# LLNL/saamge

Measured on AMD Instinct MI355X. Metric: AMG setup+solve DoF/s (3D Poisson, PCG to 1e-8), higher is better.
Workload: dtype f64; 1 GPU; 3D Poisson 256^3 Q1 hexes, 3-level SAAMGE, theta=0.003, nu_relax=3, 8x8x4-element AEs, 8x8x4-AE coarse blocks; workload_id=poisson256, dofs=16974593, converged=True, parallelism=single GPU

## Files before the change

### saamge_amd/csrc/capi.hip

```cpp
#include <cstdlib>
#include "../../include/saamge_amd.h"

#include <string>

#include "hierarchy.h"
#include "operator.h"
#include "partition.h"
#include "spgemm.h"

using namespace saamge_amd;

struct saamge_amd_hierarchy {
    Hierarchy *H;
};

struct saamge_amd_partitioning {
    int device = 0;
    std::vector<DBuf<int>> part;
    std::vector<std::vector<int>> part_host;
    std::vector<const int *> part_ptr, part_host_ptr;
    std::vector<int> n_elem, nparts;
    std::vector<DBuf<roff_t>> xadj;
    std::vector<DBuf<int>> adj;
    std::vector<int64_t> nnz;
// ... 261 lines not shown
        set_thread_stream(hs);
    }
    delete h->H;
    delete h;
    if (had) {
        dev_pool_close_stream(hs);
        unset_thread_stream();
    }
}

struct VecIn {
    DBuf<double> buf;
    const double *p;
    VecIn(const double *src, size_t n, hipStream_t s) {
        if (is_device_ptr(src)) p = src;
        else { buf.assign(src, n, s); p = buf.p; }
    }
};
struct VecOut {
    DBuf<double> buf;
    double *p, *host = nullptr;
    size_t n;
    hipStream_t s;
    VecOut(double *dst, size_t n_, hipStream_t s_, bool load) : n(n_), s(s_) {
        if (is_device_ptr(dst)) p = dst;
        else {
            host = dst;
            if (load) buf.assign(dst, n, s); else buf.alloc(n);
            p = buf.p;
        }
    }
    void finish() {
        if (host && n) SA_HIP_CHECK(hipMemcpyAsync(host, p, 8 * n, hipMemcpyDeviceToHost, s));
        SA_HIP_CHECK(hipStreamSynchronize(s));
    }
};

int saamge_amd_vcycle_mult(saamge_amd_hierarchy *h, const double *b, double *x) {
    SA_API_BEGIN
    SA_REQUIRE(h && b && x, "null argument");
    Hierarchy &H = *h->H;
    require_device(H);
    const size_t n = (size_t)H.levels[0]->A.nrows;
    VecIn vb(b, n, H.stream);
    VecOut vx(x, n, H.stream, false);
    vcycle_apply(H, 0, vb.p, vx.p);
    vx.finish();
    SA_API_END
}

int saamge_amd_vcycle(saamge_amd_hierarchy *h, const double *b, double *x, int iterative_mode) {
    if (!iterative_mode) return saamge_amd_vcycle_mult(h, b, x);
    SA_API_BEGIN
    SA_REQUIRE(h && b && x, "null argument");
    Hierarchy &H = *h->H;
    require_device(H);
    Level &L0 = *H.levels[0];
    SA_REQUIRE(!L0.dist.on, "iterative_mode is not available on a row-partitioned hierarchy");
    const size_t n = (size_t)L0.A.nrows;
    VecIn vb(b, n, H.stream);
    VecOut vx(x, n, H.stream, true);
    spmv_residual(H.stream, L0.A, vx.p, vb.p, H.pcg_r.p);
    vcycle_apply(H, 0, H.pcg_r.p, H.pcg_z.p);
    vec_axpy(H.stream, (int)n, 1.0, H.pcg_z.p, vx.p);
    vx.finish();
    SA_API_END
}

int saamge_amd_set_coarse_solver(saamge_amd_hierarchy *h, saamge_amd_coarse_solve_fn fn, void *ctx) {
    SA_API_BEGIN
    SA_REQUIRE(h, "null argument");
    h->H->user_coarse_solve = fn;
    h->H->user_coarse_ctx = ctx;
    SA_API_END
}

int saamge_amd_set_smoother(saamge_amd_hierarchy *h, int level, saamge_amd_smoother_fn pre, saamge_amd_smoother_fn post,
                            void *ctx) {
    SA_API_BEGIN
    SA_REQUIRE(h, "null argument");
    Hierarchy &H = *h->H;
    SA_REQUIRE(level >= 0 && level < (int)H.levels.size(), "bad level");
    if (H.user_smoothers.size() < H.levels.size()) H.user_smoothers.resize(H.levels.size());
    H.user_smoothers[(size_t)level].pre = pre;
    H.user_smoothers[(size_t)level].post = post;
    H.user_smoothers[(size_t)level].ctx = ctx;
    SA_API_END
}

int saamge_amd_smoother(saamge_amd_hierarchy *h, int level, const double *b, double *x) {
    SA_API_BEGIN
    SA_REQUIRE(h && b && x, "null argument");
    Hierarchy &H = *h->H;
    require_device(H);
    SA_REQUIRE(level >= 0 && level < (int)H.levels.size(), "bad level");
    const size_t n = (size_t)H.levels[level]->A.nrows;
    VecIn vb(b, n, H.stream);
    VecOut vx(x, n, H.stream, true);
    smoother_apply(H, level, vb.p, vx.p);
    vx.finish();
    SA_API_END
}

int saamge_amd_pcg(saamge_amd_hierarchy *h, const double *b, double *x, double rel_tol,
                   double abs_tol, int max_iter, int squared_tol, int zero_guess, int *iters,
                   int *converged, double *hist) {
    SA_API_BEGIN
    SA_REQUIRE(h && b && x && iters, "null argument");
    Hierarchy &H = *h->H;
    require_device(H);
    const size_t n = (size_t)H.levels[0]->A.nrows;
    VecIn vb(b, n, H.stream);
    VecOut vx(x, n, H.stream, !zero_guess);
    int conv = 0;
    *iters = pcg_solve(H, vb.p, vx.p, rel_tol, abs_tol, max_iter, squared_tol, zero_guess, &conv, hist);
    if (converged) *converged = conv;
    vx.finish();
    SA_API_END
}

int saamge_amd_num_levels(const saamge_amd_hierarchy *h) { return h ? (int)h->H->levels.size() + 1 : 0; }

static const DCsr &level_op(const Hierarchy &H, int level, int which) {
    const int nl = (int)H.levels.size();
    SA_REQUIRE(level >= 0 && level < nl, "bad level");
    const Level &L = *H.levels[level];
    switch (which) {
        case 0: return L.A;
        case 1: return L.P;
        case 2: return L.R;
        case 3: return (level + 1 < nl) ? H.levels[level + 1]->A : L.Ac;
    }
    throw Error(1, "bad operator selector");
}

int saamge_amd_level_info(const saamge_amd_hierarchy *h, int level, long long info[16]) {
    SA_API_BEGIN
    SA_REQUIRE(h && info, "null argument");
    const Hierarchy &H = *h->H;
    for (int i = 0; i < 16; ++i) info[i] = 0;
    const Level &L = *H.levels.at(level);
    info[0] = L.A.nrows;
    info[1] = L.A.nnz;
    info[2] = L.rel.nparts;
    info[3] = L.rel.num_mises;
    info[4] = L.P.ncols;
    info[5] = L.P.nnz;
    info[6] = level_op(H, level, 3).nnz;
    long long tot = 0;
    for (int m : L.ae_m) tot += m;
    info[7] = tot;
    info[8] = H.last_coarse_iters;
    info[9] = L.ae_xoff.empty() ? 0 : L.ae_xoff.back();
    info[10] = L.mis_s_off.empty() ? 0 : L.mis_s_off.back();
    long long usz = 0;
    for (int m = 0; m < L.rel.num_mises; ++m) usz += (long long)L.mis_k[m] * L.rel.mis_to_dof.row_size(m);
    info[11] = usz;
    info[12] = L.dist.on ? 1 : 0;
    info[13] = L.dist.row0;
    info[14] = L.dist.nloc;
    info[15] = L.dist.nrecv;
    SA_API_END
}

int saamge_amd_level_format(const saamge_amd_hierarchy *h, int level, long long info[12]) {
    SA_API_BEGIN
    SA_REQUIRE(h && info, "null argument");
    const Hierarchy &H = *h->H;
    for (int i = 0; i < 12; ++i) info[i] = 0;
    const Sell &S = H.levels.at(level)->A.sell;
    for (int c = 0; c < 3; ++c) { info[c] = S.class_slices[c]; info[3 + c] = S.class_entries[c]; }
    if (S.dict.on) { info[8] = S.dict.ng; info[9] = S.dict.bs3 ? 1 : 0; info[10] = S.dict.bs3 ? S.dict.nirr : 0; }
    info[6] = S.stage.on() ? (long long)div_up(S.nslices, 4) - S.stage.nunstaged : 0;
    info[7] = (long long)S.stream_bytes;
    info[11] = H.levels.at(level)->ae_solved;
    SA_API_END
}

int saamge_amd_coarse_solver_info(const saamge_amd_hierarchy *h, long long info[8]) {
    SA_API_BEGIN
    SA_REQUIRE(h && info, "null argument");
    const Hierarchy &H = *h->H;
    for (int i = 0; i < 8; ++i) info[i] = 0;
    SA_REQUIRE(!H.levels.empty(), "no levels");
    info[0] = H.user_coarse_solve ? 0 : H.coarse_kind;
    info[1] = H.levels.back()->Ac.nrows;
    if (H.coarse_kind == 3) {
        info[2] = H.c_bt.nblk;
        info[3] = H.c_bt.max_block;
        info[4] = (long long)H.c_bt.Sinv.n;
    } else if (H.coarse_kind == 1) {
        info[4] = (long long)H.c_L.n;
    }
    SA_API_END
}

static int get_csr(const saamge_amd_hierarchy *h, int level, int which, void *rowptr, int rowptr_bits, int *col, double *val) {
    SA_API_BEGIN
    SA_REQUIRE(h, "null argument");
    const Hierarchy &H = *h->H;
    require_device(H);
    const DCsr &M = level_op(H, level, which);
    hipStream_t s = H.stream;
    if (rowptr && rowptr_bits == 64)
        SA_HIP_CHECK(hipMemcpyAsync(rowptr, M.rowptr.p, sizeof(roff_t) * ((size_t)M.nrows + 1), hipMemcpyDeviceToHost, s));
    else if (rowptr)
        export_rowptr32((int *)rowptr, M.rowptr, (size_t)M.nrows + 1, s);
    if (col && M.nnz) SA_HIP_CHECK(hipMemcpyAsync(col, M.col.p, 4 * (size_t)M.nnz, hipMemcpyDeviceToHost, s));
    if (val && M.nnz) SA_HIP_CHECK(hipMemcpyAsync(val, M.val.p, 8 * (size_t)M.nnz, hipMemcpyDeviceToHost, s));
    SA_HIP_CHECK(hipStreamSynchronize(s));
    SA_API_END
}
int saamge_amd_get_csr(const saamge_amd_hierarchy *h, int level, int which, int *rowptr, int *col, double *val) {
    return get_csr(h, level, which, rowptr, 32, col, val);
}
int saamge_amd_get_csr64(const saamge_amd_hierarchy *h, int level, int which, long long *rowptr, int *col, double *val) {
    return get_csr(h, level, which, rowptr, 64, col, val);
}

int saamge_amd_get_table(const saamge_amd_hierarchy *h, int level, int which, int *nrows,
                         long long *nconn, int *I, int *J) {
    SA_API_BEGIN
    SA_REQUIRE(h, "null argument");
    require_device(*h->H);
    {
        Level &Lw = *h->H->levels.at(level);
        fetch_relations_ae_host(Lw.rel, Lw.drel, h->H->stream);
    }
    const Relations &r = h->H->levels.at(level)->rel;
    const Table *T = nullptr;
    switch (which) {
        case 0: T = &r.AE_to_dof; break;
        case 1: T = &r.dof_to_AE; break;
        case 2: T = &r.mis_to_dof; break;
        case 3: T = &r.mis_to_AE; break;
        case 4: T = &r.AE_to_mis; break;
        case 5: {
            if (r.elem_to_dof.I.empty()) {
                Level &L = *h->H->levels.at(level);
                Relations &rw = L.rel;
                rw.elem_to_dof.I = L.drel.e2d_I.to_host(h->H->stream);
                rw.elem_to_dof.J = L.drel.e2d_J.to_host(h->H->stream);
                rw.elem_to_dof.ncols = rw.ND;
            }
            T = &r.elem_to_dof;
            break;
        }
        default: throw Error(1, "bad table selector");
    }
    if (nrows) *nrows = T->nrows();
    if (nconn) *nconn = (long long)T->J.size();
    if (I) std::copy(T->I.begin(), T->I.end(), I);
    if (J) std::copy(T->J.begin(), T->J.end(), J);
    SA_API_END
}

int saamge_amd_get_mis(const saamge_amd_hierarchy *h, int level, int *mises, int *mis_k,
                       int *mis_ncols, signed char *agg_flags) {
    SA_API_BEGIN
    SA_REQUIRE(h, "null argument");
    require_device(*h->H);
    {
        Level &Lw = *h->H->levels.at(level);
        fetch_relations_ae_host(Lw.rel, Lw.drel, h->H->stream);
    }
    const Level &L = *h->H->levels.at(level);
    if (mises) std::copy(L.rel.mises.begin(), L.rel.mises.end(), mises);
    if (mis_k) std::copy(L.mis_k.begin(), L.mis_k.end(), mis_k);
    if (mis_ncols) std::copy(L.mis_ncols.begin(), L.mis_ncols.end(), mis_ncols);
    if (agg_flags) std::copy(L.rel.agg_flags.begin(), L.rel.agg_flags.end(), agg_flags);
    SA_API_END
}

int saamge_amd_get_ae_eigens(const saamge_amd_hierarchy *h, int level, int *ae_m, double *evals,
                             double *evecs, double *ae_D) {
    SA_API_BEGIN
    SA_REQUIRE(h, "null argument");
    const Hierarchy &H = *h->H;
    const Level &L = *H.levels.at(level);
    hipStream_t s = H.stream;
    if (ae_m) std::copy(L.ae_m.begin(), L.ae_m.end(), ae_m);
    if (evals || evecs || ae_D) SA_REQUIRE(H.params.keep_debug, "hierarchy was built without keep_debug");
    if (evals && L.evals.n) SA_HIP_CHECK(hipMemcpyAsync(evals, L.evals.p, 8 * L.evals.n, hipMemcpyDeviceToHost, s));
    if (evecs && L.evecs.n) SA_HIP_CHECK(hipMemcpyAsync(evecs, L.evecs.p, 8 * L.evecs.n, hipMemcpyDeviceToHost, s));
    if (ae_D && L.ae_D.n) SA_HIP_CHECK(hipMemcpyAsync(ae_D, L.ae_D.p, 8 * L.ae_D.n, hipMemcpyDeviceToHost, s));
    SA_HIP_CHECK(hipStreamSynchronize(s));
    SA_API_END
}

int saamge_amd_get_mis_svd(const saamge_amd_hierarchy *h, int level, long long *sig_off,
                           double *sig, double *U) {
    SA_API_BEGIN
    SA_REQUIRE(h, "null argument");
    const Hierarchy &H = *h->H;
    const Level &L = *H.levels.at(level);
    hipStream_t s = H.stream;
    const int nm = L.rel.num_mises;
    if (sig_off) for (int m = 0; m <= nm; ++m) sig_off[m] = L.mis_s_off[m];
    if (sig) {
        SA_REQUIRE(H.params.keep_debug, "hierarchy was built without keep_debug");
        if (L.mis_s_off[nm]) SA_HIP_CHECK(hipMemcpyAsync(sig, L.mis_sig.p, 8 * (size_t)L.mis_s_off[nm], hipMemcpyDeviceToHost, s));
    }
    if (U) {
        auto all = L.mis_U.to_host(s);
        size_t o = 0;
        for (int m = 0; m < nm; ++m) {
            const size_t cnt = (size_t)L.mis_k[m] * L.rel.mis_to_dof.row_size(m);
            std::copy(all.begin() + L.mis_u_off[m], all.begin() + L.mis_u_off[m] + cnt, U + o);
            o += cnt;
        }
    }
    SA_HIP_CHECK(hipStreamSynchronize(s));
    SA_API_END
}

static int spmv_entry(int nrows, int ncols, const void *rowptr, int rowptr_bits, const int *col, const double *val,
                      const double *x, double *y) {
    SA_API_BEGIN
    SA_REQUIRE(rowptr && col && val && x && y && nrows >= 0, "bad argument");
    const Options opt = g_default_options;
    validate_options(opt);
    hipStream_t s = 0;
    set_thread_stream(s);
    DCsr A;
    A.nrows = nrows;
    A.ncols = ncols;
    import_rowptr(A.rowptr, rowptr, rowptr_bits, (size_t)nrows + 1, s);
    roff_t nnz = 0;
    SA_HIP_CHECK(hipMemcpyAsync(&nnz, A.rowptr.p + nrows, sizeof(roff_t), hipMemcpyDeviceToHost, s));
    SA_HIP_CHECK(hipStreamSynchronize(s));
    A.nnz = nnz;
    import_array(A.col, col, (size_t)A.nnz, s);
    import_array(A.val, val, (size_t)A.nnz, s);
    A.lanes_per_row = pick_lanes_per_row(A.nnz, nrows > 0 ? nrows : 1);
    if (nrows == ncols && opt.spmv_sell) build_sell(s, A, opt);
    VecIn vx(x, (size_t)ncols, s);
    VecOut vy(y, (size_t)nrows, s, false);
    spmv(s, A, vx.p, vy.p);
    vy.finish();
    SA_API_END
}
int saamge_amd_spmv(int nrows, int ncols, const int *rowptr, const int *col, const double *val,
                    const double *x, double *y) {
    return spmv_entry(nrows, ncols, rowptr, 32, col, val, x, y);
}
int saamge_amd_spmv64(int nrows, int ncols, const long long *rowptr, const int *col, const double *val,
                      const double *x, double *y) {
    return spmv_entry(nrows, ncols, rowptr, 64, col, val, x, y);
}

static void import_host_csr(DCsr &M, const char *name, int nrows, int ncols, const int *rowptr, const int *col,
                            const double *val, hipStream_t s) {
    const std::string who(name);
    SA_REQUIRE(nrows >= 0 && ncols >= 0 && rowptr, who + ": bad dimensions or no row offsets");
    SA_REQUIRE(rowptr[0] == 0, who + ": the row offsets must start at 0");
    for (int i = 0; i < nrows; ++i) SA_REQUIRE(rowptr[i + 1] >= rowptr[i], who + ": the row offsets must ascend");
    const size_t nnz = (size_t)rowptr[nrows];
    SA_REQUIRE(nnz == 0 || (col && val), who + ": entries without their arrays");
    for (size_t k = 0; k < nnz; ++k) SA_REQUIRE(col[k] >= 0 && col[k] < ncols, who + ": a column index out of range");
    M.nrows = nrows;
    M.ncols = ncols;
    M.nnz = (int64_t)nnz;
    import_rowptr(M.rowptr, rowptr, 32, (size_t)nrows + 1, s);
    M.col.assign(col, nnz, s);
    M.val.assign(val, nnz, s);
    SA_HIP_CHECK(hipStreamSynchronize(s));
    M.lanes_per_row = pick_lanes_per_row(M.nnz, nrows > 0 ? nrows : 1);
}
static void export_host_csr(const DCsr &M, int *rowptr, long long *nnz, int *col, double *val, hipStream_t s) {
    if (rowptr) export_rowptr32(rowptr, M.rowptr, (size_t)M.nrows + 1, s);
    if (nnz) *nnz = (long long)M.nnz;
    if (col && val && M.nnz) {
        SA_HIP_CHECK(hipMemcpyAsync(col, M.col.p, 4 * (size_t)M.nnz, hipMemcpyDeviceToHost, s));
        SA_HIP_CHECK(hipMemcpyAsync(val, M.val.p, 8 * (size_t)M.nnz, hipMemcpyDeviceToHost, s));
    }
    SA_HIP_CHECK(hipStreamSynchronize(s));
}

int saamge_amd_spgemm(int nrows, int ninner, int ncols, const int *Arow, const int *Acol, const double *Aval,
                      const int *Brow, const int *Bcol, const double *Bval, const int *Erow, const int *Ecol,
                      const double *Eval, const double *d, double alpha, double beta, int *Crow, long long *Cnnz,
                      int *Ccol, double *Cval, int *route) {
    if (route) *route = SPGEMM_ROUTE_NONE;
    SA_API_BEGIN
    hipStream_t s = 0;
    set_thread_stream(s);
    DCsr A, B, E, Cm;
    import_host_csr(A, "A", nrows, ninner, Arow, Acol, Aval, s);
    import_host_csr(B, "B", ninner, ncols, Brow, Bcol, Bval, s);
    const bool alias = Erow && Erow == Brow && Ecol == Bcol && Eval == Bval && nrows == ninner;
    if (Erow && !alias) import_host_csr(E, "E", nrows, ncols, Erow, Ecol, Eval, s);
    DBuf<double> dd;
    if (d) dd.assign(d, (size_t)nrows, s);
    spgemm(s, A, B, Erow ? (alias ? &B : &E) : nullptr, d ? dd.p : nullptr, alpha, beta, Cm);
    if (route) *route = spgemm_last_route();
    export_host_csr(Cm, Crow, Cnnz, Ccol, Cval, s);
    SA_API_END
}

int saamge_amd_csr_transpose(int nrows, int ncols, const int *rowptr, const int *col, const double *val, int *Rrow,
                             long long *Rnnz, int *Rcol, double *Rval) {
    SA_API_BEGIN
    hipStream_t s = 0;
    set_thread_stream(s);
    DCsr P, R;
    import_host_csr(P, "P", nrows, ncols, rowptr, col, val, s);
    csr_transpose(s, P, R);
    export_host_csr(R, Rrow, Rnnz, Rcol, Rval, s);
    SA_API_END
}

int saamge_amd_csr_threshold(int nrows, int ncols, const int *rowptr, const int *col, const double *val, double tol,
                             int *Crow, long long *Cnnz, int *Ccol, double *Cval) {
    SA_API_BEGIN
    hipStream_t s = 0;
    set_thread_stream(s);
    DCsr A, Cm;
    import_host_csr(A, "A", nrows, ncols, rowptr, col, val, s);
    csr_threshold(s, A, tol, Cm);
    export_host_csr(Cm, Crow, Cnnz, Ccol, Cval, s);
    SA_API_END
}

__global__ void apply_dscale_kernel(int count, const int *ns, const int64_t *moff, const int64_t *voff,
                                    double *W, const double *D, double *dis) {
    const int b = blockIdx.x;
    const int n = ns[b];
    double *Wm = W + moff[b];
    const double *Dm = D + voff[b];
    for (int i = threadIdx.x; i < n; i += blockDim.x) dis[voff[b] + i] = 1.0 / sqrt(Dm[i]);
    __syncthreads();
    for (size_t idx = threadIdx.x; idx < (size_t)n * n; idx += blockDim.x) {
        const int r = (int)(idx % n), c = (int)(idx / n);
        Wm[idx] = dis[voff[b] + r] * Wm[idx] * dis[voff[b] + c];
    }
}

int saamge_amd_lower_eigens_batched(int count, const int *n, const double *A, const double *D,
                                    double vl, double vu, int *m, double *evals, double *evecs) {
    SA_API_BEGIN
    SA_REQUIRE(count >= 0 && n && A && D && m && evals && evecs, "bad argument");
    const Options opt = g_default_options;
    validate_options(opt);
    hipStream_t s = 0;
    set_thread_stream(s);
    std::vector<int> sizes(n, n + count);
    EigBatch b;
    eig_batch_alloc(b, sizes, opt, s);
    b.set_window(vu);
    b.dense_only = opt.eig_dense_only != 0;
// ... 437 lines not shown
```

### saamge_amd/csrc/common.h

```cpp
#pragma once
#include <hip/hip_runtime.h>

#include <cstdint>
#include <cstdio>
#include <cstring>
#include <type_traits>
#include <stdexcept>
#include <string>
#include <vector>

namespace saamge_amd {

struct Error : std::runtime_error {
    int code;
    Error(int c, const std::string &m) : std::runtime_error(m), code(c) {}
};

#define SA_HIP_CHECK(expr)                                                              \
    do {                                                                                \
        hipError_t e_ = (expr);                                                         \
        if (e_ != hipSuccess)                                                           \
            throw ::saamge_amd::Error(2, std::string(__FILE__) + ":" +                  \
                                             std::to_string(__LINE__) + " " + #expr +   \
                                             " -> " + hipGetErrorString(e_));           \
    } while (0)

#define SA_REQUIRE(cond, msg)                                                           \
    do {                                                                                \
        if (!(cond))                                                                    \
            throw ::saamge_amd::Error(1, std::string(__FILE__) + ":" +                  \
                                             std::to_string(__LINE__) + " " + (msg));   \
    } while (0)

inline int current_device() {
    int d = 0;
    SA_HIP_CHECK(hipGetDevice(&d));
    return d;
}
inline void adopt_device(int dev) { SA_HIP_CHECK(hipSetDevice(dev)); }
hipStream_t side_stream(int slot);

void *pinned_alloc(size_t bytes);
void pinned_free(void *p, size_t bytes);
void pinned_pool_release();

template <class T>
struct PinnedAlloc {
    typedef T value_type;
    PinnedAlloc() {}
    template <class U>
    PinnedAlloc(const PinnedAlloc<U> &) {}
    T *allocate(size_t n) { return (T *)pinned_alloc(n * sizeof(T)); }
    void deallocate(T *p, size_t n) { pinned_free((void *)p, n * sizeof(T)); }
    template <class U>
    bool operator==(const PinnedAlloc<U> &) const { return true; }
    template <class U>
    bool operator!=(const PinnedAlloc<U> &) const { return false; }
};
template <class T>
using hvec = std::vector<T, PinnedAlloc<T>>;

inline bool is_device_ptr(const void *p) {
    if (!p) return false;
    hipPointerAttribute_t a;
    hipError_t e = hipPointerGetAttributes(&a, p);
    if (e != hipSuccess) {
        (void)hipGetLastError();
        return false;
    }
    return a.type == hipMemoryTypeDevice || a.type == hipMemoryTypeManaged;
}

void host_heap_policy(int mb);
bool env_timing();
bool env_timing_host();
bool env_serial();

void set_thread_stream(hipStream_t s);
void unset_thread_stream();
hipStream_t thread_stream();
bool thread_stream_is_set();
void *dev_alloc(size_t bytes);
void dev_free(void *p) noexcept;
void dev_pool_release();
size_t dev_pool_idle_bytes();
void dev_memory_stats(size_t *live, size_t *peak, bool reset_peak);
void dev_pool_counts(long *n_malloc, long *n_free, size_t *malloc_bytes, bool reset);
struct ThreadStreamScope {
    hipStream_t prev;
    bool had;
    explicit ThreadStreamScope(hipStream_t s) : prev(thread_stream()), had(thread_stream_is_set()) { set_thread_stream(s); }
    ~ThreadStreamScope() { if (had) set_thread_stream(prev); else unset_thread_stream(); }
};
void dev_pool_close_stream(hipStream_t s);

template <class T>
struct DBuf {
    T *p = nullptr;
    size_t n = 0;
    bool owned = true;
    DBuf() {}
    explicit DBuf(size_t n_) { alloc(n_); }
    DBuf(const DBuf &) = delete;
    DBuf &operator=(const DBuf &) = delete;
    DBuf(DBuf &&o) noexcept : p(o.p), n(o.n), owned(o.owned) { o.p = nullptr; o.n = 0; }
    DBuf &operator=(DBuf &&o) noexcept {
        if (this != &o) {
            release();
            p = o.p; n = o.n; owned = o.owned;
            o.p = nullptr; o.n = 0;
        }
        return *this;
    }
    ~DBuf() { release(); }
    void release() {
        if (p && owned) dev_free(p);
        p = nullptr; n = 0; owned = true;
    }
    void alloc(size_t n_) {
        release();
        n = n_;
        if (n) p = (T *)dev_alloc(n * sizeof(T));
    }
    void zero(hipStream_t s = 0) {
        if (n) SA_HIP_CHECK(hipMemsetAsync(p, 0, n * sizeof(T), s));
    }
    void assign(const T *src, size_t n_, hipStream_t s = 0) {
        alloc(n_);
        if (!n) return;
        SA_HIP_CHECK(hipMemcpyAsync(p, src, n * sizeof(T), hipMemcpyDefault, s));
    }
    template <class V>
    void from_host(const V &v, hipStream_t s = 0) {
        alloc(v.size());
        if (!n) return;
        const size_t bytes = n * sizeof(T);
        const bool pinned = std::is_same<typename V::allocator_type, PinnedAlloc<typename V::value_type>>::value;
        if (!pinned && bytes >= (256u << 10)) {
            void *stage = pinned_alloc(bytes);
            std::memcpy(stage, v.data(), bytes);
            const hipError_t e = hipMemcpyAsync(p, stage, bytes, hipMemcpyHostToDevice, s);
            const hipError_t e2 = hipStreamSynchronize(s);
            pinned_free(stage, bytes);
            SA_HIP_CHECK(e);
            SA_HIP_CHECK(e2);
            return;
        }
        SA_HIP_CHECK(hipMemcpyAsync(p, v.data(), bytes, hipMemcpyHostToDevice, s));
        SA_HIP_CHECK(hipStreamSynchronize(s));
    }
    hvec<T> to_host(hipStream_t s = 0) const {
        hvec<T> v(n);
        if (n) {
            SA_HIP_CHECK(hipMemcpyAsync(v.data(), p, n * sizeof(T), hipMemcpyDeviceToHost, s));
            SA_HIP_CHECK(hipStreamSynchronize(s));
        }
        return v;
    }
    void view(T *ptr, size_t n_) {
        release();
        p = ptr; n = n_; owned = false;
    }
};

template <class T>
inline void import_array(DBuf<T> &dst, const T *src, size_t n, hipStream_t s) {
    if (is_device_ptr(src))
        dst.view(const_cast<T *>(src), n);
    else
        dst.assign(src, n, s);
}

template <class T>
inline hvec<T> fetch_host(const T *src, size_t n, hipStream_t s) {
    hvec<T> v(n);
    if (n) {
        SA_HIP_CHECK(hipMemcpyAsync(v.data(), src, n * sizeof(T), hipMemcpyDefault, s));
        SA_HIP_CHECK(hipStreamSynchronize(s));
    }
    return v;
}
template <class T>
inline T read_one(const T *p, hipStream_t s) {
    T v;
    SA_HIP_CHECK(hipMemcpyAsync(&v, p, sizeof(T), hipMemcpyDeviceToHost, s));
    SA_HIP_CHECK(hipStreamSynchronize(s));
    return v;
}

typedef int64_t roff_t;

}
#include "sell.h"
namespace saamge_amd {
struct DCsr {
    int nrows = 0, ncols = 0;
    int64_t nnz = 0;
    DBuf<roff_t> rowptr;
    DBuf<int> col;
    DBuf<double> val;
    int lanes_per_row = 8;
    mutable int max_row = -1;
    Sell sell;
};

void exclusive_scan_int(hipStream_t s, int n, const int *in, int *out);
void exclusive_scan_int_async(hipStream_t s, int n, const int *in, int *out, int *tile_sums);
void exclusive_scan_off(hipStream_t s, int n, const int *in, roff_t *out);

void import_rowptr(DBuf<roff_t> &dst, const void *src, int bits, size_t n, hipStream_t s);
void export_rowptr32(int *dst_host, const DBuf<roff_t> &src, size_t n, hipStream_t s);

inline int pick_lanes_per_row(int64_t nnz, int nrows) {
    double avg = nrows ? double(nnz) / nrows : 1.0;
    int l = 1;
    while (l < 64 && l * 2 <= avg * 0.75 + 1.0) l *= 2;
    return l;
}

inline int div_up(int64_t a, int64_t b) { return int((a + b - 1) / b); }
__host__ __device__ inline unsigned hash_home(unsigned key, unsigned size) {
    return (key * 2654435761u) >> (__builtin_clz(size) + 1);
}

struct KernelStat {
    std::string name;
    double ms = 0.0;
    int64_t launches = 0;
    double bytes = 0.0;
    double flops = 0.0;
    double fmt_bytes = 0.0;
};

struct Profiler {
    bool enabled = false;
    std::vector<KernelStat> stats;
    hipEvent_t e0 = nullptr, e1 = nullptr;
    int level_tag = 0;
    KernelStat &get(const std::string &name) {
        for (auto &s : stats)
            if (s.name == name) return s;
        stats.push_back(KernelStat());
        stats.back().name = name;
        return stats.back();
    }
    void begin(hipStream_t s) {
        if (!enabled) return;
        if (!e0) {
            SA_HIP_CHECK(hipEventCreate(&e0));
            SA_HIP_CHECK(hipEventCreate(&e1));
        }
        SA_HIP_CHECK(hipEventRecord(e0, s));
    }
    void end(hipStream_t s, const char *name, double bytes, double flops, double fmt_bytes = 0.0) {
        if (!enabled) return;
        SA_HIP_CHECK(hipEventRecord(e1, s));
        SA_HIP_CHECK(hipEventSynchronize(e1));
        float ms = 0.f;
        SA_HIP_CHECK(hipEventElapsedTime(&ms, e0, e1));
        KernelStat &k = level_tag > 0 ? get(std::string(name) + "@L" + std::to_string(level_tag)) : get(name);
        k.ms += ms;
        k.launches += 1;
        k.bytes += bytes;
        k.flops += flops;
        k.fmt_bytes += fmt_bytes > 0.0 ? fmt_bytes : bytes;
    }
};

Profiler &profiler();

}
```

### saamge_amd/csrc/hierarchy.h

```cpp
#pragma once
#include <exception>
#include <memory>
#include <thread>

#include "assemble.h"
#include "blocktri.h"
#include "common.h"
#include "eig.h"
#include "mis.h"
#include "options.h"
#include "sparse.h"
#include "topology.h"

namespace saamge_amd {

constexpr int MAX_LEVELS = 8;

struct Params {
    int num_coarsenings = 1;
    double theta[MAX_LEVELS];
    int nu_relax[MAX_LEVELS];
    int nu_pro[MAX_LEVELS];
    int avoid_ess_bdr_dofs = 1;
    int testmesh = 0;
    int coarse_solver = 0;
    double coarse_rtol = 1e-14;
    int coarse_max_iter = 2000;
    size_t workspace_bytes = (size_t)32 << 30;
    int keep_debug = 0;
    int rank = 0, world = 1;
    int (*allgather)(void *ctx, void *buf_dev, const long long *byte_off) = nullptr;
    void *allgather_ctx = nullptr;
    int (*allreduce_sum)(void *ctx, double *buf_dev, long long count) = nullptr;
    int (*alltoallv)(void *ctx, const void *send_dev, const long long *send_byte_off, void *recv_dev,
                     const long long *recv_byte_off) = nullptr;
    long long dist_min_local_rows = 262144;
    int comm_stream_ordered = 0;
    int correct_nullspace = 0;
    const double *extra_modes = nullptr;
    int num_extra_modes = 0;
    double smooth_drop_tol = 0.0;
    int do_aggregates = 0;
    int algebraic = 0;
    int eigensolver = 0;
    double eig_tol = 1e-12;
    Options opt;
};

struct NextPrep {
    bool ready = false;
    Table e2d;
    std::vector<int> colpos_ptr, colpos;
    DBuf<int> d_colpos_ptr, d_colpos;
    bool on_device = false;
};

struct Level {
    DCsr A;
    DCsr P, R, Ac;
    DCsr Ptent;
    DBuf<double> dinv_neg;
    std::vector<double> roots;
    double theta = 0.0;
    int nu_relax = 3;
    Relations rel;
    bool rel_prebuilt = false;
    NextPrep next_prep;
    DevRelations drel;
    DevElmats elmat;
    std::vector<int> ae_begin;
    std::vector<int> ae_m;
    std::vector<int> ae_class;
    std::vector<int> ae_evclass;
    long long ae_solved = 0;
    std::vector<int64_t> ae_xoff, ae_eoff;
    DBuf<double> evals, evecs;
    DBuf<double> ae_D;
    std::vector<int> mis_k;
    std::vector<int> mis_coloff;
    std::vector<int> mis_ncols;
    std::vector<int64_t> mis_u_off, mis_s_off;
    DBuf<double> mis_U, mis_sig;
    DBuf<int> d_mis_k, d_mis_coloff;
    DBuf<int64_t> d_mis_u_off;
    DBuf<double> x, b, r, t0, t1;
    DBuf<double> extra;
    DBuf<double> cvec_next;
    struct Dist {
        bool on = false;
        int row0 = 0, nloc = 0;
        std::vector<int> row_off;
        std::vector<long long> send_off, recv_off;
        std::vector<long long> own_off;
        DBuf<int> send_idx, recv_idx;
        DBuf<double> send_buf, recv_buf;
        DBuf<double> rs_buf;
        std::vector<long long> rs_off;
        int nsend = 0, nrecv = 0;
        int int_row0 = 0, int_nrows = 0;
    } dist;
};

struct KernelTiming { double setup_ms = 0, solve_ms = 0; };

struct ParCsrIn {
    long long global_rows = 0;
    const long long *row_starts = nullptr;
    int nrows = 0;
    const int *diag_i = nullptr, *diag_j = nullptr;
    const double *diag_a = nullptr;
    const int *offd_i = nullptr, *offd_j = nullptr;
    const double *offd_a = nullptr;
    int num_cols_offd = 0;
    const long long *col_map_offd = nullptr;
};
struct DistIn {
    DBuf<roff_t> rowptr;
    DBuf<int> col, e2d;
    DBuf<double> val;
    DBuf<signed char> bdr;
    std::vector<DBuf<int>> parts;
    std::vector<int> nparts;
    int elem0 = 0, NE_loc = 0;
    std::vector<std::vector<long long>> ae_begin;
};

struct Hierarchy {
    Params params;
    hipStream_t stream = 0;
    int device = 0;
    std::vector<std::unique_ptr<Level>> levels;
    int coarse_kind = 2;
    BlockTri c_bt;
    DBuf<double> c_dinv, c_r, c_z, c_d, c_q, c_t0, c_t1, c_b, c_x;
    DBuf<double> c_L, c_work;
    std::vector<double> c_roots;
    DBuf<double> pcg_r, pcg_z, pcg_d, pcg_q, scal, partials;
    int last_coarse_iters = 0;
    int (*user_coarse_solve)(void *ctx, int n, const double *rc_host, double *xc_host) = nullptr;
    void *user_coarse_ctx = nullptr;
    struct UserSmoother {
        int (*pre)(void *ctx, int level, int n, const double *b_host, double *x_host) = nullptr;
        int (*post)(void *ctx, int level, int n, const double *b_host, double *x_host) = nullptr;
        void *ctx = nullptr;
    };
    std::vector<UserSmoother> user_smoothers;
    DBuf<int> own_e2d;
    DBuf<int> e2d_ptr;
    std::vector<hvec<int>> coarse_parts;
    std::vector<int> nparts_in;
    std::unique_ptr<DistIn> dist_in;
    std::thread galerkin_thread;
    std::exception_ptr galerkin_err;
    int galerkin_lev = -1;
    hipEvent_t ev_fork = nullptr, ev_join = nullptr;
    ~Hierarchy() {
        if (galerkin_thread.joinable()) galerkin_thread.join();
        if (ev_fork) (void)hipEventDestroy(ev_fork);
        if (ev_join) (void)hipEventDestroy(ev_join);
    }
};

Hierarchy *hierarchy_create(int n, const void *Arow, int rowptr_bits, const int *Acol, const double *Aval, int NE,
                            int nde, const int *elem_ptr, const int *elem_to_dof, const double *elmat,
                            const signed char *bdr, const int *const *partitions,
                            const int *nparts, const Params &p, hipStream_t stream, std::unique_ptr<DistIn> din = nullptr);
Hierarchy *hierarchy_create_dist(const ParCsrIn &A, int NE_loc, int nde, const int *elem_to_dof, const double *elmat,
                                 const signed char *bdr_own, const int *const *partitions, const int *nparts_loc,
                                 const Params &p, hipStream_t stream);

void hierarchy_update_operators(Hierarchy &h, const double *new_val);

void vcycle_apply(Hierarchy &h, int level, const double *b, double *x);
void smoother_apply(Hierarchy &h, int level, const double *b, double *x);
int pcg_solve(Hierarchy &h, const double *b, double *x, double rel_tol, double abs_tol,
              int max_iter, int squared_tol, int zero_guess, int *converged, double *hist);

}
```

### saamge_amd/csrc/hierarchy.hip

```cpp
#include "hierarchy.h"
#include "dist.h"
#include "dense.h"
#include "spgemm.h"

#include <algorithm>
#include <cmath>
#include <chrono>
#include <cstdlib>
#include <functional>
#include <thread>

namespace saamge_amd {

static std::vector<double> sas_poly_roots(int nu) {
    SA_REQUIRE(nu > 0, "nu_relax must be positive");
    std::vector<double> r;
    const double denom = (double)(2 * nu + 1);
    for (int i = 0; i <= 2 * nu; ++i) {
        const double v = std::cos(((double)i * M_PI) / denom);
        r.push_back(v * v);
    }
    for (int i = 1; i <= nu; ++i) {
        const double v = std::sin(((double)i * M_PI) / denom);
        r.push_back(v * v);
    }
    return r;
}

struct PhaseTimer {
    bool on, host;
    hipStream_t s;
    std::chrono::steady_clock::time_point t0;
    explicit PhaseTimer(hipStream_t st) : on(env_timing() || env_timing_host()), host(env_timing_host()), s(st) {
        t0 = std::chrono::steady_clock::now();
    }
    void lap(const char *what, int lev) {
        if (!on) return;
        if (!host) (void)hipStreamSynchronize(s);
        auto t1 = std::chrono::steady_clock::now();
        std::fprintf(stderr, "TIMING: level %d %-28s %9.3f ms\n", lev, what,
                     std::chrono::duration<double, std::milli>(t1 - t0).count());
        t0 = std::chrono::steady_clock::now();
    }
};

static DBuf<double> &scratch_pool(int slot) {
    static DBuf<double> *pools = new DBuf<double>[4];
    return pools[slot];
}
static double *scratch_get(int slot, size_t need) {
    DBuf<double> &p = scratch_pool(slot);
    if (p.n < need) p.alloc(need + need / 8 + 64);
    return p.p;
}

static void finish_csr(DCsr &A) { A.lanes_per_row = pick_lanes_per_row(A.nnz, A.nrows > 0 ? A.nrows : 1); }

__global__ void iota_int_kernel(long n, int *p) {
    const long i = (long)blockIdx.x * 256 + threadIdx.x;
    if (i < n) p[i] = (int)i;
}

__global__ void iota64_kernel(long n, int64_t scale, int64_t *p) {
    const long i = (long)blockIdx.x * 256 + threadIdx.x;
    if (i < n) p[i] = i * scale;
}

constexpr int MAX_ELEM_DOFS = 32767;
__global__ __launch_bounds__(256) void elem_ptr_check_kernel(long NE, const int *__restrict__ ptr, int *__restrict__ info) {
    const long e = (long)blockIdx.x * 256 + threadIdx.x;
    if (e == 0 && ptr[0] != 0) atomicOr(&info[0], 1);
    if (e >= NE) return;
    const int nd = ptr[e + 1] - ptr[e];
    if (nd <= 0) atomicOr(&info[0], 2);
    else if (nd > MAX_ELEM_DOFS) atomicOr(&info[0], 4);
    else { atomicMax(&info[1], MAX_ELEM_DOFS - nd); atomicMax(&info[2], nd); }
}
__global__ __launch_bounds__(256) void dof_range_kernel(long nconn, int ND, const int *__restrict__ J, int *__restrict__ err) {
    const long k = (long)blockIdx.x * 256 + threadIdx.x;
    if (k < nconn && (J[k] < 0 || J[k] >= ND)) atomicOr(err, 8);
}
__global__ __launch_bounds__(256) void elem_sq_kernel(long NE, const int *__restrict__ ptr, int *__restrict__ sq) {
    const long e = (long)blockIdx.x * 256 + threadIdx.x;
    if (e < NE) { const int nd = ptr[e + 1] - ptr[e]; sq[e] = nd * nd; }
}

static int check_elem_ptr(int NE, const int *elem_ptr, const int *elem_to_dof, int ND, int &max_nd, hipStream_t s) {
    int bits = 0, mn = 0, mx = 0;
    long nconn = 0;
    if (!is_device_ptr(elem_ptr)) {
        bits |= elem_ptr[0] != 0 ? 1 : 0;
        mn = MAX_ELEM_DOFS;
        for (int e = 0; e < NE && !bits; ++e) {
            const int nd = elem_ptr[e + 1] - elem_ptr[e];
            if (nd <= 0) bits |= 2;
            else if (nd > MAX_ELEM_DOFS) bits |= 4;
            else { mn = std::min(mn, nd); mx = std::max(mx, nd); }
        }
        if (!bits) nconn = elem_ptr[NE];
    } else {
        DBuf<int> info(3);
        info.zero(s);
        hipLaunchKernelGGL(elem_ptr_check_kernel, dim3(div_up((long)NE, 256)), dim3(256), 0, s, (long)NE, elem_ptr, info.p);
        SA_HIP_CHECK(hipGetLastError());
        const auto h = info.to_host(s);
        bits = h[0]; mn = MAX_ELEM_DOFS - h[1]; mx = h[2];
        if (!bits) {
            int last = 0;
            SA_HIP_CHECK(hipMemcpyAsync(&last, elem_ptr + NE, sizeof(int), hipMemcpyDeviceToHost, s));
            SA_HIP_CHECK(hipStreamSynchronize(s));
            nconn = last;
        }
    }
    SA_REQUIRE(!(bits & 1), "elem_ptr[0] must be 0");
    SA_REQUIRE(!(bits & 2), "elem_ptr: an element without dofs or decreasing offsets");
    SA_REQUIRE(!(bits & 4), "elem_ptr: an element with more than 32767 dofs");
    if (!is_device_ptr(elem_to_dof)) {
        for (long k = 0; k < nconn; ++k)
            SA_REQUIRE(elem_to_dof[k] >= 0 && elem_to_dof[k] < ND, "elem_to_dof entry out of range");
    } else {
        DBuf<int> err(1);
        err.zero(s);
        hipLaunchKernelGGL(dof_range_kernel, dim3(div_up(nconn, 256)), dim3(256), 0, s, nconn, ND, elem_to_dof, err.p);
        SA_HIP_CHECK(hipGetLastError());
        SA_REQUIRE(!err.to_host(s)[0], "elem_to_dof entry out of range");
    }
    max_nd = mx;
    return mn == mx ? mx : 0;
}

__global__ void gather_kernel(long n, const int *__restrict__ idx, const double *__restrict__ src, double *__restrict__ dst) {
    const long i = (long)blockIdx.x * blockDim.x + threadIdx.x;
    if (i < n) dst[i] = src[idx[i]];
}
__global__ void fill_kernel(long n, double *p, double v) {
    const long i = (long)blockIdx.x * 256 + threadIdx.x;
    if (i < n) p[i] = v;
}

static void level_galerkin(Hierarchy &H, int lev, bool first, hipStream_t s) {
    Level &L = *H.levels[lev];
    const Params &P = H.params;
    const Relations &rel = L.rel;
    const int world = P.world > 1 ? P.world : 1;
    if (P.nu_pro[lev] == 0) {
        std::vector<long long> nnz_off;
        rap_mis(s, L.drel, rel, L.A, L.mis_k, L.mis_coloff, L.d_mis_k.p, L.d_mis_coloff.p,
                L.d_mis_u_off.p, L.mis_U.p, L.Ac, P.rank, world, world > 1 ? &nnz_off : nullptr);
        if (world > 1 && L.Ac.nnz > 0) {
            std::vector<long long> off((size_t)world + 1);
            for (int r = 0; r <= world; ++r) off[r] = 4ll * nnz_off[r];
            SA_REQUIRE(P.allgather(P.allgather_ctx, L.Ac.col.p, off.data()) == 0, "all-gather (Ac columns) failed");
            for (int r = 0; r <= world; ++r) off[r] = 8ll * nnz_off[r];
            SA_REQUIRE(P.allgather(P.allgather_ctx, L.Ac.val.p, off.data()) == 0, "all-gather (Ac values) failed");
        }
    } else {
        const int nu = P.nu_pro[lev];
        if (first) L.Ptent = std::move(L.P);
        DCsr tmp[2];
        const DCsr *cur = &L.Ptent;
        for (int k = 1; k <= nu; ++k) {
            const double sn = std::sin((double)k * M_PI / (double)(2 * nu + 1));
            DCsr &dst = tmp[k & 1];
            dst = DCsr();
            spgemm(s, L.A, *cur, cur, L.dinv_neg.p, 1.0 / (sn * sn), 1.0, dst);
            cur = &dst;
        }
        if (P.smooth_drop_tol != 0.0)
            csr_threshold(s, tmp[nu & 1], P.smooth_drop_tol, L.P);
        else
            L.P = std::move(tmp[nu & 1]);
        csr_transpose(s, L.P, L.R);
        DCsr AP;
        spgemm(s, L.A, L.P, nullptr, nullptr, 1.0, 0.0, AP);
        spgemm(s, L.R, AP, nullptr, nullptr, 1.0, 0.0, L.Ac);
    }
}

static void level_galerkin(Hierarchy &H, int lev, bool first) { level_galerkin(H, lev, first, H.stream); }

static void join_galerkin(Hierarchy &H) {
    if (H.galerkin_lev < 0) return;
    if (H.galerkin_thread.joinable()) H.galerkin_thread.join();
    const int lev = H.galerkin_lev;
    H.galerkin_lev = -1;
    if (H.galerkin_err) {
        std::exception_ptr e = H.galerkin_err;
        H.galerkin_err = nullptr;
        std::rethrow_exception(e);
    }
    H.levels[lev + 1]->A = std::move(H.levels[lev]->Ac);
}

struct DeviceInputs {
    const int *e2d = nullptr, *part = nullptr;
    const int *e2d_I = nullptr;
    const signed char *bdr = nullptr;
    int NE = 0, nde = 0;
};

static void prepare_next_host(const Level &L, const roff_t *p_rowptr_dev, const double *p_val_dev, int p_nrows,
                              int64_t p_nnz, hipStream_t s, NextPrep &out);

static void build_level(Hierarchy &H, int lev, Table &&e2d, const hvec<int> &part, int nparts,
                        const signed char *bdr_host, const DeviceInputs *din = nullptr) {
    Level &L = *H.levels[lev];
    hipStream_t s = H.stream;
    const Params &P = H.params;
    L.theta = P.theta[lev];
    L.nu_relax = P.nu_relax[lev];
    SA_REQUIRE(P.nu_pro[lev] >= 0 && P.nu_pro[lev] <= 8, "bad prolongator smoothing degree");
    PhaseTimer tm(s);
    std::thread op_thread;
    std::exception_ptr op_err;
    struct OpJoiner { std::thread &t; ~OpJoiner() { if (t.joinable()) t.join(); } } op_joiner{op_thread};
    const bool op_early = lev == 0 && din && !env_serial() && !profiler().enabled && H.galerkin_lev < 0 && (P.opt.overlap & 8);
    if (op_early) {
        hipStream_t os = side_stream(6);
        const int dev0 = current_device();
        SA_HIP_CHECK(hipStreamSynchronize(s));
        op_thread = std::thread([&L, &P, &op_err, os, dev0]() {
            try {
                adopt_device(dev0);
                set_thread_stream(os);
                build_sell(os, L.A, P.opt);
                L.dinv_neg.alloc((size_t)L.A.nrows);
                DBuf<double> tmp((size_t)L.A.nrows);
                build_dinv_neg(os, L.A, tmp.p, L.dinv_neg.p);
                build_dinv_codes(os, L.A, L.dinv_neg.p, P.opt);
                SA_HIP_CHECK(hipStreamSynchronize(os));
            } catch (...) { op_err = std::current_exception(); }
        });
    }
    bool on_device = false;
    if (din) {
        on_device = build_relations_ae_device(L.rel, L.drel, din->e2d, din->NE, din->nde, din->e2d_I, din->part, nparts,
                                              L.A.nrows, din->bdr, s);
        tm.lap("device topology (AE tables)", lev);
    }
    if (!on_device) {
        hvec<int> part_h;
        hvec<signed char> bdr_h;
        if (din) {
            if (din->e2d_I) {
                e2d.I = fetch_host(din->e2d_I, (size_t)din->NE + 1, s);
            } else {
                e2d.I.resize((size_t)din->NE + 1);
                for (int e = 0; e <= din->NE; ++e) e2d.I[e] = e * din->nde;
            }
            e2d.J = fetch_host(din->e2d, (size_t)e2d.I[din->NE], s);
            e2d.ncols = L.A.nrows;
            part_h = fetch_host(din->part, (size_t)din->NE, s);
            if (din->bdr) bdr_h = fetch_host(din->bdr, (size_t)L.A.nrows, s);
        }
        if (!L.rel_prebuilt)
            build_relations_ae(L.rel, std::move(e2d), din ? part_h : part, nparts, L.A.nrows,
                               din ? (din->bdr ? bdr_h.data() : nullptr) : bdr_host);
        tm.lap(L.rel_prebuilt ? "host topology (built beside the element matrices)" : "host topology (AE tables)", lev);
        upload_relations_ae(L.drel, L.rel, s);
        tm.lap("upload topology", lev);
    }
    HostCsr aggA;
    const bool aggregates = P.do_aggregates && lev == P.num_coarsenings - 1;
    if (aggregates) {
        join_galerkin(H);
        aggA.nrows = L.A.nrows;
        aggA.rowptr.resize((size_t)L.A.nrows + 1);
        aggA.col.resize((size_t)L.A.nnz);
        aggA.val.resize((size_t)L.A.nnz);
        SA_HIP_CHECK(hipMemcpyAsync(aggA.rowptr.data(), L.A.rowptr.p, sizeof(roff_t) * ((size_t)L.A.nrows + 1), hipMemcpyDeviceToHost, s));
        SA_HIP_CHECK(hipMemcpyAsync(aggA.col.data(), L.A.col.p, sizeof(int) * (size_t)L.A.nnz, hipMemcpyDeviceToHost, s));
        SA_HIP_CHECK(hipMemcpyAsync(aggA.val.data(), L.A.val.p, sizeof(double) * (size_t)L.A.nnz, hipMemcpyDeviceToHost, s));
        SA_HIP_CHECK(hipStreamSynchronize(s));
    }
    hipStream_t mis_stream = side_stream(0);
    const int dev = current_device();
    std::exception_ptr mis_err;
    const bool serial = env_serial();
    auto mis_work = [&]() {
        try {
            adopt_device(dev);
            set_thread_stream(mis_stream);
            constexpr bool host_mis = false;
            PhaseTimer tmis(mis_stream);
            bool on_dev = false;
            if (!aggregates && !host_mis) on_dev = build_relations_mis_device(L.rel, L.drel, mis_stream);
            if (on_dev) tmis.lap("    device MIS tables", lev);
            if (!on_dev) {
                fetch_relations_ae_host(L.rel, L.drel, mis_stream);
                build_relations_mis(L.rel, aggregates ? &aggA : nullptr);
                upload_relations_mis(L.drel, L.rel, mis_stream);
            }
            SA_HIP_CHECK(hipStreamSynchronize(mis_stream));
        } catch (...) { mis_err = std::current_exception(); }
    };
    std::thread mis_thread;
    if (serial) {
        mis_work();
        set_thread_stream(s);
    } else {
// ... 300 lines not shown
        solve_cls[slot].clear();
        if (dedupe && dedupe_level && !batch.dense_only) {
            DdSource src = classes.src;
            bool found = classes.early;
            if (!found && !classes.searched && batch.has_bw) {
                src = eig_dedupe_source(batch);
                found = eig_dedupe_find(qa, src, cnt, batch.max_n, classes.cls, P.opt.debug);
            }
            if (!found && lvl_classes.empty()) dedupe_level = false;
            if (found) {
                const DdClasses &cl = classes.cls;
                const int nl = (int)cl.reps.size();
                std::vector<int> l2g((size_t)nl, -1);
                std::vector<int> list, qidx, cand;
                std::vector<const unsigned long long *> blobs;
                std::vector<long> bwords;
                for (int q = 0; q < nl; ++q) {
                    auto it = lvl_by_hash.find(DdKey{cl.rep_hash[2 * (size_t)q], cl.rep_hash[2 * (size_t)q + 1]});
                    if (it == lvl_by_hash.end()) continue;
                    for (int id : it->second)
                        if (lvl_classes[id].kind == src.kind) {
                            list.push_back(cl.reps[q]); qidx.push_back(q); cand.push_back(id);
                            blobs.push_back(lvl_classes[id].blob.p); bwords.push_back(lvl_classes[id].words);
                        }
                }
                std::vector<char> same;
                eig_dedupe_compare(qa, src, batch.max_n, list, blobs, bwords, same);
                for (size_t t = 0; t < list.size(); ++t)
                    if (same[t] && l2g[qidx[t]] < 0) l2g[qidx[t]] = cand[t];
                std::vector<int> newq, newlist;
                for (int q = 0; q < nl; ++q)
                    if (l2g[q] < 0) { newq.push_back(q); newlist.push_back(cl.reps[q]); }
                const std::vector<long> nwords = eig_dedupe_words(qa, src, batch.h_n, newlist);
                std::vector<DBuf<unsigned long long>> nblobs;
                eig_dedupe_pack(qa, src, batch.max_n, newlist, nwords, nblobs);
                std::vector<int> alias(newq.size(), -1);
                {
                    std::unordered_map<DdKey, int, DdKeyHash> firstc;
                    std::vector<int> clist, cwho;
                    std::vector<const unsigned long long *> cblobs;
                    std::vector<long> cwords;
                    for (size_t t = 0; t < newq.size(); ++t) {
                        auto it = firstc.emplace(DdKey{cl.rep_hash[2 * (size_t)newq[t]], cl.rep_hash[2 * (size_t)newq[t] + 1]}, (int)t);
                        if (it.second) continue;
                        clist.push_back(newlist[t]); cwho.push_back((int)t);
                        cblobs.push_back(nblobs[it.first->second].p); cwords.push_back(nwords[it.first->second]);
                    }
                    std::vector<char> csame;
                    eig_dedupe_compare(qa, src, batch.max_n, clist, cblobs, cwords, csame);
                    for (size_t u = 0; u < clist.size(); ++u)
                        if (csame[u]) alias[cwho[u]] = firstc[DdKey{cl.rep_hash[2 * (size_t)newq[cwho[u]]], cl.rep_hash[2 * (size_t)newq[cwho[u]] + 1]}];
                }
                std::vector<int> solve_list;
                std::vector<int> id_of(newq.size(), -1);
                for (size_t t = 0; t < newq.size(); ++t) {
                    if (alias[t] >= 0) { id_of[t] = id_of[alias[t]]; l2g[newq[t]] = id_of[t]; continue; }
                    solve_list.push_back(newlist[t]);
                    const int id = (int)lvl_classes.size();
                    id_of[t] = id;
                    lvl_classes.emplace_back();
                    SolvedClass &sc = lvl_classes.back();
                    sc.n = batch.h_n[newlist[t]];
                    sc.kind = src.kind;
                    sc.words = nwords[t];
                    sc.blob = std::move(nblobs[t]);
                    lvl_by_hash[DdKey{cl.rep_hash[2 * (size_t)newq[t]], cl.rep_hash[2 * (size_t)newq[t] + 1]}].push_back(id);
                    l2g[newq[t]] = id;
                    solve_cls[slot].push_back(id);
                }
                cls_of[slot].resize((size_t)cnt);
                for (int i = 0; i < cnt; ++i) cls_of[slot][i] = l2g[cl.rep_of[i]];
                assembled[slot] = std::move(batch);
                eig_batch_compact(qa, batch, assembled[slot], solve_list);
            }
        }
        if (batch.count) eig_tridiagonalize(qa, batch, 1);
        L.ae_solved += batch.count;
        pend_ae0[slot] = ae0;
        pend_cnt[slot] = cnt;
        pend_row0[slot] = row0;
        if (prev >= 0) { join_iterate(); post(prev); }
        start_iterate(slot);
        prev = slot;
        row0 += rows_chunk;
        ae0 += cnt;
    }
    if (prev >= 0) { join_iterate(); post(prev); }
    tm.lap("local eigenproblems", lev);
    if (operator_pending) {
        operator_data();
        tm.lap("operator (deferred Galerkin product) + SELL + D", lev);
    }
    if (world > 1) {
        DBuf<int> d_m;
        d_m.from_host(L.ae_m, s);
        std::vector<long long> off((size_t)world + 1);
        for (int r = 0; r <= world; ++r) off[r] = 4ll * ae_begin[r];
        SA_REQUIRE(P.allgather(P.allgather_ctx, d_m.p, off.data()) == 0, "all-gather (counts) failed");
        auto t_ = d_m.to_host(s);
        L.ae_m.assign(t_.begin(), t_.end());
    }
    const bool extra = (P.testmesh && lev == 0);
    L.ae_xoff.assign((size_t)nparts + 1, 0);
    L.ae_eoff.assign((size_t)nparts + 1, 0);
    std::vector<int> m_tot = L.ae_m;
    if (extra) m_tot[0] += 1;
    for (int p = 0; p < nparts; ++p) {
        L.ae_xoff[p + 1] = L.ae_xoff[p] + (int64_t)m_tot[p] * sizes[p];
        L.ae_eoff[p + 1] = L.ae_eoff[p] + L.ae_m[p];
    }
    L.evals.alloc((size_t)L.ae_eoff[nparts]);
    L.evecs.alloc((size_t)L.ae_xoff[nparts]);
    for (Chunk &c : chunks) {
        if (c.evals.n)
            SA_HIP_CHECK(hipMemcpyAsync(L.evals.p + L.ae_eoff[c.ae0], c.evals.p, 8 * c.evals.n,
                                        hipMemcpyDeviceToDevice, s));
        if (extra && c.ae0 == 0) {
            const int64_t first = (int64_t)L.ae_m[0] * sizes[0];
            SA_HIP_CHECK(hipMemcpyAsync(L.evecs.p, c.evecs.p, 8 * first, hipMemcpyDeviceToDevice, s));
            hipLaunchKernelGGL(fill_kernel, dim3(div_up(sizes[0], 256)), dim3(256), 0, s, (long)sizes[0],
                               L.evecs.p + first, 1.0);
            if (c.evecs.n > (size_t)first)
                SA_HIP_CHECK(hipMemcpyAsync(L.evecs.p + L.ae_xoff[1], c.evecs.p + first,
                                            8 * (c.evecs.n - first), hipMemcpyDeviceToDevice, s));
        } else if (c.evecs.n) {
            SA_HIP_CHECK(hipMemcpyAsync(L.evecs.p + L.ae_xoff[c.ae0], c.evecs.p, 8 * c.evecs.n,
                                        hipMemcpyDeviceToDevice, s));
        }
    }
    SA_HIP_CHECK(hipStreamSynchronize(s));
    chunks.clear();
    L.ae_m = m_tot;
    if (world > 1) {
        std::vector<long long> off((size_t)world + 1);
        for (int r = 0; r <= world; ++r) off[r] = 8ll * L.ae_xoff[ae_begin[r]];
        SA_REQUIRE(P.allgather(P.allgather_ctx, L.evecs.p, off.data()) == 0, "all-gather (eigenvectors) failed");
        if (P.keep_debug) {
            for (int r = 0; r <= world; ++r) off[r] = 8ll * L.ae_eoff[ae_begin[r]];
            SA_REQUIRE(P.allgather(P.allgather_ctx, L.evals.p, off.data()) == 0, "all-gather (eigenvalues) failed");
            int64_t rows = 0;
            std::vector<int64_t> rowoff((size_t)nparts + 1, 0);
            for (int p = 0; p < nparts; ++p) rowoff[p + 1] = rowoff[p] + sizes[p];
            (void)rows;
            for (int r = 0; r <= world; ++r) off[r] = 8ll * rowoff[ae_begin[r]];
            SA_REQUIRE(P.allgather(P.allgather_ctx, L.ae_D.p, off.data()) == 0, "all-gather (D) failed");
        }
        tm.lap("all-gather eigenvectors", lev);
    }

    if (mis_thread.joinable()) mis_thread.join();
    if (mis_err) std::rethrow_exception(mis_err);
    tm.lap("MIS tables (join)", lev);
    const int nm = rel.num_mises;
    std::vector<int64_t> g_off((size_t)nm + 1, 0);
    L.mis_u_off.assign((size_t)nm + 1, 0);
    L.mis_s_off.assign((size_t)nm + 1, 0);
    int max_ctot = 0;
    const int nextra = (lev == 0 && P.extra_modes) ? P.num_extra_modes : 0;
    if (nextra) import_array(L.extra, P.extra_modes, (size_t)nextra * L.A.nrows, s);
    for (int m = 0; m < nm; ++m) {
        int ctot = nextra;
        for (int q = rel.mis_to_AE.I[m]; q < rel.mis_to_AE.I[m + 1]; ++q) ctot += L.ae_m[rel.mis_to_AE.J[q]];
        const int r = rel.mis_to_dof.row_size(m);
        g_off[m + 1] = g_off[m] + (int64_t)r * ctot;
        L.mis_u_off[m + 1] = L.mis_u_off[m] + (int64_t)r * std::max(1, std::min(r, ctot));
        L.mis_s_off[m + 1] = L.mis_s_off[m] + ctot;
        max_ctot = std::max(max_ctot, ctot);
    }
    L.mis_U.alloc((size_t)L.mis_u_off[nm]);
    L.mis_sig.alloc((size_t)L.mis_s_off[nm] + 1);
    L.mis_sig.zero(s);
    L.d_mis_k.alloc((size_t)nm);
    {
        double *gather = scratch_get(1, (size_t)g_off[nm] + 1);
        DBuf<int64_t> d_goff, d_soff, d_xoff;
        DBuf<int> d_aem, d_ncols((size_t)nm);
        d_goff.from_host(g_off, s);
        d_soff.from_host(L.mis_s_off, s);
        L.d_mis_u_off.from_host(L.mis_u_off, s);
        d_xoff.from_host(L.ae_xoff, s);
        d_aem.from_host(L.ae_m, s);
        MisSvdIO io;
        io.ae_m = d_aem.p;
        io.ae_xoff = d_xoff.p;
        io.evecs = L.evecs.p;
        io.g_off = d_goff.p;
        io.gather = gather;
        io.u_off = L.d_mis_u_off.p;
        io.s_off = d_soff.p;
        io.U = L.mis_U.p;
        io.sig = L.mis_sig.p;
        io.k = L.d_mis_k.p;
        io.ncols = d_ncols.p;
        io.avoid_ess = P.avoid_ess_bdr_dofs;
        io.extra = nextra ? L.extra.p : nullptr;
        io.nextra = nextra;
        io.ND = L.A.nrows;
        io.debug = P.opt.debug;
        if (world > 1) {
            std::vector<int> mb((size_t)world + 1, nm);
            double total = 0.0;
            auto cost = [&](int m) {
                const double r = rel.mis_to_dof.row_size(m), c = (double)(L.mis_s_off[m + 1] - L.mis_s_off[m]);
                return r * std::min(r, c) * std::max(r, c) + 64.0;
            };
            for (int m = 0; m < nm; ++m) total += cost(m);
            double run = 0.0;
            int rk = 0;
            mb[0] = 0;
            for (int m = 0; m < nm && rk + 1 < world; ++m) {
                run += cost(m);
                while (rk + 1 < world && run >= total * (rk + 1) / world) mb[++rk] = m + 1;
            }
            mb[world] = nm;
            L.d_mis_k.zero(s);
            d_ncols.zero(s);
            mis_svd(s, L.drel, mb[P.rank + 1] - mb[P.rank], max_ctot, io, mb[P.rank]);
            std::vector<long long> off((size_t)world + 1);
            for (int r = 0; r <= world; ++r) off[r] = 8ll * L.mis_u_off[mb[r]];
            SA_REQUIRE(P.allgather(P.allgather_ctx, L.mis_U.p, off.data()) == 0, "all-gather (MIS bases) failed");
            for (int r = 0; r <= world; ++r) off[r] = 8ll * L.mis_s_off[mb[r]];
            SA_REQUIRE(P.allgather(P.allgather_ctx, L.mis_sig.p, off.data()) == 0, "all-gather (singular values) failed");
            for (int r = 0; r <= world; ++r) off[r] = 4ll * mb[r];
            SA_REQUIRE(P.allgather(P.allgather_ctx, L.d_mis_k.p, off.data()) == 0, "all-gather (MIS counts) failed");
            SA_REQUIRE(P.allgather(P.allgather_ctx, d_ncols.p, off.data()) == 0, "all-gather (MIS columns) failed");
        } else {
            DBuf<int> d_ev;
            bool any = false;
            for (int v_ : L.ae_evclass) any = any || v_ >= 0;
            if (any && P.opt.eig_dedupe != 0 && !(P.testmesh && lev == 0)) d_ev.from_host(L.ae_evclass, s);
            mis_svd(s, L.drel, nm, max_ctot, io, 0, d_ev.n ? d_ev.p : nullptr);
        }
        { auto t_ = L.d_mis_k.to_host(s); L.mis_k.assign(t_.begin(), t_.end()); }
        { auto t_ = d_ncols.to_host(s); L.mis_ncols.assign(t_.begin(), t_.end()); }
    }
    tm.lap("MIS gather + SVD", lev);
    L.mis_coloff.assign((size_t)nm + 1, 0);
    for (int m = 0; m < nm; ++m) L.mis_coloff[m + 1] = L.mis_coloff[m] + L.mis_k[m];
    L.d_mis_coloff.from_host(L.mis_coloff, s);
    build_P_R(s, L.drel, rel, L.mis_k, L.mis_u_off, L.d_mis_k.p, L.d_mis_coloff.p, L.d_mis_u_off.p,
              L.mis_U.p, L.P, L.R);
    if (lev + 1 < P.num_coarsenings) {
        L.cvec_next.alloc((size_t)L.R.nrows);
        const double *cv = nullptr;
        DBuf<double> ones;
        if (lev > 0 && H.levels[lev - 1]->cvec_next.n == (size_t)L.A.nrows) cv = H.levels[lev - 1]->cvec_next.p;
        else {
            ones.alloc((size_t)L.A.nrows);
            hipLaunchKernelGGL(fill_kernel, dim3(div_up((long)L.A.nrows, 256)), dim3(256), 0, s, (long)L.A.nrows, ones.p, 1.0);
            cv = ones.p;
        }
        spmv(s, L.R, cv, L.cvec_next.p);
        SA_HIP_CHECK(hipStreamSynchronize(s));
    }
    std::exception_ptr prep_err;
    std::thread prep_thread;
    struct PrepJoiner { std::thread &t; ~PrepJoiner() { if (t.joinable()) t.join(); } } prep_joiner{prep_thread};
    constexpr bool host_e2d = false;
    if (lev + 1 < P.num_coarsenings && P.nu_pro[lev] == 0 && !host_e2d) {
        NextPrep &np = L.next_prep;
        np.on_device = coarse_e2d_device(s, L.drel, rel, L.d_mis_k.p, L.d_mis_coloff.p, L.mis_coloff.back(),
                                         L.P.rowptr.p, L.P.val.p, np.d_colpos_ptr, np.d_colpos, np.e2d);
        np.ready = np.on_device;
    }
    if (lev + 1 < P.num_coarsenings && P.nu_pro[lev] == 0 && !L.next_prep.ready) {
        hipStream_t side = side_stream(1);
        SA_HIP_CHECK(hipStreamSynchronize(s));
        const roff_t *prp = L.P.rowptr.p;
        const double *pvl = L.P.val.p;
        const int pnr = L.P.nrows;
        const int64_t pnz = L.P.nnz;
        hipStream_t sd = side;
        prep_thread = std::thread([&L, &prep_err, prp, pvl, pnr, pnz, sd, dev]() {
            try {
                adopt_device(dev);
                set_thread_stream(sd);
                prepare_next_host(L, prp, pvl, pnr, pnz, sd, L.next_prep);
                SA_HIP_CHECK(hipStreamSynchronize(sd));
            } catch (...) { prep_err = std::current_exception(); }
        });
    }
    const bool no_overlap = !(P.opt.overlap & 4) || env_serial();
    const bool defer = lev + 1 < P.num_coarsenings && P.nu_pro[lev] == 0 && world == 1 && !no_overlap &&
                       !profiler().enabled;
    if (defer) {
        SA_HIP_CHECK(hipStreamSynchronize(s));
        hipStream_t gs = side_stream(2);
        H.galerkin_lev = lev;
        H.galerkin_thread = std::thread([&H, lev, gs, dev]() {
            try {
                adopt_device(dev);
                set_thread_stream(gs);
                level_galerkin(H, lev, true, gs);
                SA_HIP_CHECK(hipStreamSynchronize(gs));
            } catch (...) { H.galerkin_err = std::current_exception(); }
        });
    } else {
        level_galerkin(H, lev, true);
    }
    if (prep_thread.joinable()) prep_thread.join();
    if (prep_err) std::rethrow_exception(prep_err);
    tm.lap(defer ? "P, R (RAP deferred)" : "P, R, RAP", lev);
    if (!P.keep_debug) {
        L.evals.release();
        L.evecs.release();
        L.mis_sig.release();
    }
    const size_t n = (size_t)L.A.nrows;
    L.x.alloc(n); L.b.alloc(n); L.r.alloc(n); L.t0.alloc(n);
}

static void prepare_next_host(const Level &L, const roff_t *p_rowptr_dev, const double *p_val_dev, int p_nrows,
                              int64_t p_nnz, hipStream_t s, NextPrep &out) {
    fetch_relations_ae_host(const_cast<Relations &>(L.rel), L.drel, s);
    const Relations &rel = L.rel;
    const int nparts = rel.nparts;
    Table &e2d = out.e2d;
    e2d.ncols = L.mis_coloff.back();
    e2d.I.assign((size_t)nparts + 1, 0);
    hvec<roff_t> p_rowptr((size_t)p_nrows + 1);
    hvec<double> p_val((size_t)p_nnz + 1);
    SA_HIP_CHECK(hipMemcpyAsync(p_rowptr.data(), p_rowptr_dev, sizeof(roff_t) * ((size_t)p_nrows + 1), hipMemcpyDeviceToHost, s));
    if (p_nnz) SA_HIP_CHECK(hipMemcpyAsync(p_val.data(), p_val_dev, sizeof(double) * (size_t)p_nnz, hipMemcpyDeviceToHost, s));
    SA_HIP_CHECK(hipStreamSynchronize(s));
    std::vector<int> &colpos_ptr = out.colpos_ptr;
    colpos_ptr.assign(rel.AE_to_mis.J.size() + 1, 0);
    for (int e = 0; e < nparts; ++e)
        for (int t = rel.AE_to_mis.I[e]; t < rel.AE_to_mis.I[e + 1]; ++t)
            colpos_ptr[(size_t)t + 1] = colpos_ptr[t] + L.mis_k[rel.AE_to_mis.J[t]];
    std::vector<int> &colpos = out.colpos;
    colpos.assign((size_t)colpos_ptr.back(), -1);
    {
        int T = (int)std::thread::hardware_concurrency();
        if (T < 1) T = 1;
        if (T > 16) T = 16;
        if (nparts < 64) T = 1;
        auto walk = [&](int e, std::vector<int> &stamp, int *dst, bool fill) -> int {
            int run = 0;
            const int *misrow = rel.AE_to_mis.row(e);
            const int nmis = rel.AE_to_mis.row_size(e);
            for (int k = rel.AE_to_dof.I[e]; k < rel.AE_to_dof.I[e + 1]; ++k) {
                const int dof = rel.AE_to_dof.J[k];
                const int m = rel.mises[dof];
                const int km = L.mis_k[m];
                if (km == 0) continue;
                const int t = rel.AE_to_mis.I[e] + (int)(std::lower_bound(misrow, misrow + nmis, m) - misrow);
                for (int v = 0; v < km; ++v) {
                    const int cd = L.mis_coloff[m] + v;
                    if (stamp[cd] == e) continue;
                    if (p_val[(size_t)p_rowptr[dof] + v] == 0.0) continue;
                    stamp[cd] = e;
                    if (fill) {
                        colpos[(size_t)colpos_ptr[t] + v] = run;
                        dst[run] = cd;
                    }
                    ++run;
                }
            }
            return run;
        };
        const int dev = current_device();
        for (int pass = 0; pass < 2; ++pass) {
            std::vector<std::thread> th;
            for (int t = 0; t < T; ++t)
                th.emplace_back([&, t, pass]() {
                    (void)hipSetDevice(dev);
                    std::vector<int> stamp((size_t)e2d.ncols, -1);
                    const int eb = (int)((int64_t)nparts * t / T), ee = (int)((int64_t)nparts * (t + 1) / T);
                    for (int e = eb; e < ee; ++e) {
                        if (pass == 0) e2d.I[e + 1] = walk(e, stamp, nullptr, false);
                        else walk(e, stamp, e2d.J.data() + e2d.I[e], true);
                    }
                });
            for (auto &x : th) x.join();
            if (pass == 0) {
                for (int e = 0; e < nparts; ++e) e2d.I[e + 1] += e2d.I[e];
                e2d.J.resize((size_t)e2d.I[nparts]);
            }
        }
    }
    out.ready = true;
}

static Table prepare_next_level(Hierarchy &H, int lev) {
    Level &L = *H.levels[lev];
    hipStream_t s = H.stream;
    const Relations &rel = L.rel;
    const int nparts = rel.nparts;
    if (!L.next_prep.ready) {
        const DCsr &PT = L.Ptent.nrows ? L.Ptent : L.P;
        NextPrep &np = L.next_prep;
        constexpr bool host_e2d = false;
        if (!host_e2d)
            np.on_device = coarse_e2d_device(s, L.drel, rel, L.d_mis_k.p, L.d_mis_coloff.p, L.mis_coloff.back(),
                                             PT.rowptr.p, PT.val.p, np.d_colpos_ptr, np.d_colpos, np.e2d);
        if (!np.on_device) prepare_next_host(L, PT.rowptr.p, PT.val.p, PT.nrows, PT.nnz, s, L.next_prep);
    }
    Table e2d = std::move(L.next_prep.e2d);
    DBuf<int> d_colpos_ptr, d_colpos;
    if (L.next_prep.on_device) {
        d_colpos_ptr = std::move(L.next_prep.d_colpos_ptr);
        d_colpos = std::move(L.next_prep.d_colpos);
    } else {
        for (int v : L.next_prep.colpos) SA_REQUIRE(v >= 0, "coarse dof with an all-zero prolongator column in an AE");
        d_colpos_ptr.from_host(L.next_prep.colpos_ptr, s);
        d_colpos.from_host(L.next_prep.colpos, s);
    }
    L.next_prep = NextPrep();
    Level &N = *H.levels[lev + 1];
    std::vector<int64_t> out_off((size_t)nparts + 1, 0);
    for (int e = 0; e < nparts; ++e) {
        const int64_t ke = e2d.row_size(e);
        out_off[e + 1] = out_off[e] + ke * ke;
    }
    N.elmat.off.from_host(out_off, s);
    N.elmat.val.alloc((size_t)out_off[nparts] + 1);
    std::exception_ptr topo_err;
    std::thread topo_thread;
    struct TopoJoiner { std::thread &t; ~TopoJoiner() { if (t.joinable()) t.join(); } } topo_joiner{topo_thread};
    if (lev + 1 < H.params.num_coarsenings && lev + 1 < (int)H.coarse_parts.size() && !H.coarse_parts[(size_t)lev + 1].empty() &&
        !env_serial()) {
        const int dev = current_device();
        const int nd_next = L.mis_coloff.back(), np_next = H.nparts_in[(size_t)lev + 1];
        Table *e2d_copy = new Table(e2d);
        const hvec<int> *part_next = &H.coarse_parts[(size_t)lev + 1];
        topo_thread = std::thread([&N, &topo_err, e2d_copy, part_next, nd_next, np_next, dev]() {
            std::unique_ptr<Table> own(e2d_copy);
            try {
                adopt_device(dev);
                build_relations_ae(N.rel, std::move(*own), *part_next, np_next, nd_next, nullptr);
                N.rel_prebuilt = true;
            } catch (...) { topo_err = std::current_exception(); }
        });
    }
    std::vector<int> sizes((size_t)nparts);
    for (int p = 0; p < nparts; ++p) sizes[p] = rel.AE_to_dof.row_size(p);
    const int world = H.params.world > 1 ? H.params.world : 1;
    const int ae_lo = world > 1 ? L.ae_begin[H.params.rank] : 0;
    const int ae_hi = world > 1 ? L.ae_begin[H.params.rank + 1] : nparts;
    DBuf<int> d_ae_class;
    for (int ae0 = ae_lo; ae0 < ae_hi;) {
        size_t bytes = 0;
        int cnt = 0;
        while (ae0 + cnt < ae_hi) {
            const size_t n = (size_t)sizes[ae0 + cnt];
            const size_t add = 8 * (n * n + n * (EIG_NB + 8) + n * (size_t)e2d.row_size(ae0 + cnt));
            if (cnt > 0 && bytes + add > H.params.workspace_bytes) break;
            bytes += add;
            ++cnt;
        }
        EigBatch batch;
        eig_batch_alloc(batch, std::vector<int>(sizes.begin() + ae0, sizes.begin() + ae0 + cnt), H.params.opt, s);
        std::vector<int64_t> soff((size_t)cnt + 1, 0);
        for (int i = 0; i < cnt; ++i) soff[i + 1] = soff[i] + (int64_t)sizes[ae0 + i] * e2d.row_size(ae0 + i);
        DBuf<int64_t> d_soff;
        d_soff.from_host(soff, s);
        double *scratch = scratch_get(0, (size_t)soff[cnt] + 1);
        int RW = 0;
        const double *rv = nullptr;
        const short *rc = nullptr;
        constexpr bool dense_only = false;
        const RowsSpan span{(int64_t)rel.AE_to_dof.I[ae0] - (int64_t)rel.AE_to_dof.I[ae_lo], (int64_t)rel.AE_to_dof.I[ae_hi] - (int64_t)rel.AE_to_dof.I[ae_lo]};
        if (lev == 0 && !dense_only && ae_sparse_rows(s, L.drel, L.A, L.elmat, ae0, batch, RW, rv, rc, &span)) {
            int kmax = 0;
            for (int km : L.mis_k) kmax = std::max(kmax, km);
            bool have_classes = H.params.opt.eig_dedupe != 0 && (int)L.ae_class.size() == nparts;
            for (int i = ae0; have_classes && i < ae0 + cnt; ++i) have_classes = L.ae_class[i] >= 0;
            if (have_classes && !d_ae_class.n) d_ae_class.from_host(L.ae_class, s);
            coarse_elmats_sparse(s, L.drel, ae0, batch, RW, rv, rc, L.d_mis_k.p, L.d_mis_u_off.p, L.mis_U.p,
                                 d_colpos_ptr.p, d_colpos.p, N.elmat.off.p, N.elmat.val.p, scratch, d_soff.p, kmax,
                                 have_classes ? d_ae_class.p : nullptr);
        } else {
            ae_build(s, L.drel, lev == 0 ? &L.A : nullptr, L.elmat, ae0, batch, false, nullptr);
            coarse_elmats(s, L.drel, ae0, batch, L.d_mis_k.p, L.d_mis_u_off.p, L.mis_U.p, d_colpos_ptr.p,
                          d_colpos.p, N.elmat.off.p, N.elmat.val.p, scratch, d_soff.p);
        }
        if (world > 1 || ae0 + cnt < ae_hi) SA_HIP_CHECK(hipStreamSynchronize(s));
        ae0 += cnt;
    }
    if (world > 1) {
        std::vector<long long> off((size_t)world + 1);
        for (int r = 0; r <= world; ++r) off[r] = 8ll * out_off[L.ae_begin[r]];
        SA_REQUIRE(H.params.allgather(H.params.allgather_ctx, N.elmat.val.p, off.data()) == 0,
                   "all-gather (coarse element matrices) failed");
    }
    if (topo_thread.joinable()) topo_thread.join();
    if (topo_err) std::rethrow_exception(topo_err);
    return e2d;
}

static const DCsr &coarsest_op(const Hierarchy &H) { return H.levels.back()->Ac; }

static void setup_coarse_solver(Hierarchy &H) {
    DCsr &Ac = H.levels.back()->Ac;
    hipStream_t s = H.stream;
    const size_t n = (size_t)Ac.nrows;
    build_sell(s, Ac, H.params.opt);
    H.coarse_kind = 2;
    H.c_dinv.alloc(n);
    H.c_r.alloc(n); H.c_z.alloc(n); H.c_d.alloc(n); H.c_q.alloc(n); H.c_t0.alloc(n); H.c_t1.alloc(n);
    if (n) {
        DBuf<double> tmp(n);
        build_dinv_neg(s, Ac, tmp.p, H.c_dinv.p);
        SA_HIP_CHECK(hipStreamSynchronize(s));
    }
    H.c_roots = sas_poly_roots(H.levels.back()->nu_relax);
    const int want = H.params.coarse_solver;
    constexpr long dense_max = 8192;
    H.c_bt = BlockTri();
    if (n && (want == 1 || (want == 0 && (long)n <= dense_max)) && n <= 16384) {
        if (dense_inverse_spd(s, Ac, H.c_L)) H.coarse_kind = 1;
        else H.c_L.release();
    } else if (n && (want == 1 || want == 3)) {
        if (blocktri_factor(s, Ac, H.c_bt)) H.coarse_kind = 3;
    }
}

static inline RowRange rows_of(const Level::Dist *D) {
    RowRange rr;
    if (D) { rr.row0 = D->row0; rr.nrows = D->nloc; }
    return rr;
}

static void smooth_from_zero(Hierarchy &H, const DCsr &A, const double *dinv,
                             const std::vector<double> &roots, const double *b, double *x, double *tmp,
                             Level::Dist *D = nullptr) {
    hipStream_t s = H.stream;
    const int deg = (int)roots.size();
    const int off = D ? D->row0 : 0, nl = D ? D->nloc : A.nrows;
    double *cur = ((deg - 1) % 2 == 0) ? x : tmp;
    double *oth = (cur == x) ? tmp : x;
    smooth_first(s, nl, dinv + off, b + off, cur + off, 1.0 / roots[0]);
    for (int i = 1; i < deg; ++i) {
        const double scale = 1.0 / roots[i];
        halo_then(H, D, cur, [&](hipStream_t q, RowRange rr) { smooth_step(q, A, dinv, b, cur, oth, scale, rr); });
        std::swap(cur, oth);
    }
}

static void smooth_inplace(Hierarchy &H, const DCsr &A, const double *dinv,
                           const std::vector<double> &roots, const double *b, double *x, double *tmp,
                           Level::Dist *D = nullptr) {
    hipStream_t s = H.stream;
    const int deg = (int)roots.size();
    const int off = D ? D->row0 : 0, nl = D ? D->nloc : A.nrows;
    double *cur = x, *oth = tmp;
    for (int i = 0; i < deg; ++i) {
        const double scale = 1.0 / roots[i];
        halo_then(H, D, cur, [&](hipStream_t q, RowRange rr) { smooth_step(q, A, dinv, b, cur, oth, scale, rr); });
        std::swap(cur, oth);
    }
    if (cur != x) vec_copy(s, nl, cur + off, x + off);
}

static double read_scalar(hipStream_t s, const double *dptr) {
    double v;
    SA_HIP_CHECK(hipMemcpyAsync(&v, dptr, sizeof(double), hipMemcpyDeviceToHost, s));
    SA_HIP_CHECK(hipStreamSynchronize(s));
    return v;
}

static int pcg_loop(Hierarchy &H, const DCsr &A, const std::function<void(const double *, double *)> &prec,
                    const double *b, double *x, double *r, double *z, double *d, double *q,
                    double rel_tol, double abs_tol, int max_iter, bool squared, bool zero_guess,
                    int *converged, double *hist, double *sc, Level::Dist *D = nullptr) {
    hipStream_t s = H.stream;
    const int off = D ? D->row0 : 0, n = D ? D->nloc : A.nrows;
    auto pdot = [&](const double *u, const double *v, double *out) {
        dot(s, n, u + off, v + off, H.partials.p, out);
        if (D) dist_allreduce(H, out, 1);
    };
    if (zero_guess) {
        vec_zero(s, n, x + off);
        vec_copy(s, n, b + off, r + off);
    } else {
        halo_then(H, D, x, [&](hipStream_t q, RowRange rq) { spmv_residual(q, A, x, b, r, rq); });
    }
    prec(r, z);
    vec_copy(s, n, z + off, d + off);
    pdot(d, r, sc + 0);
    const double nom0 = read_scalar(s, sc + 0);
    if (hist) hist[0] = nom0;
    const double r0 = squared ? std::max(nom0 * rel_tol * rel_tol, abs_tol * abs_tol)
                              : std::max(nom0 * rel_tol, abs_tol);
    if (converged) *converged = 0;
    if (nom0 <= r0) {
        if (converged) *converged = 1;
        return 0;
    }
    halo_then(H, D, d, [&](hipStream_t st, RowRange rq) { spmv(st, A, d, q, rq); });
    pdot(q, d, sc + 1);
    if (read_scalar(s, sc + 1) == 0.0) return 0;
    int i = 1;
    int final_iter = max_iter;
    for (;;) {
        pcg_update_xr(s, n, sc, x + off, r + off, d + off, q + off);
        prec(r, z);
        pdot(r, z, sc + 2);
        const double betanom = read_scalar(s, sc + 2);
        if (hist) hist[i] = betanom;
        if (betanom < r0) {
            if (converged) *converged = 1;
            final_iter = i;
            break;
        }
        if (++i > max_iter) break;
        pcg_update_d(s, n, sc, d + off, z + off);
        halo_then(H, D, d, [&](hipStream_t st, RowRange rq) { spmv(st, A, d, q, rq); });
        pdot(d, q, sc + 1);
        SA_HIP_CHECK(hipMemcpyAsync(sc + 0, sc + 2, sizeof(double), hipMemcpyDeviceToDevice, s));
    }
    return final_iter;
}

static void coarse_solve(Hierarchy &H, const double *rc, double *xc) {
    const DCsr &Ac = coarsest_op(H);
    if (Ac.nrows == 0) return;
    if (H.user_coarse_solve) {
        const size_t n = (size_t)Ac.nrows;
        hvec<double> hr(n), hx(n, 0.0);
        SA_HIP_CHECK(hipMemcpyAsync(hr.data(), rc, 8 * n, hipMemcpyDeviceToHost, H.stream));
        SA_HIP_CHECK(hipStreamSynchronize(H.stream));
        SA_REQUIRE(H.user_coarse_solve(H.user_coarse_ctx, (int)n, hr.data(), hx.data()) == 0, "user coarse solver failed");
        SA_HIP_CHECK(hipMemcpyAsync(xc, hx.data(), 8 * n, hipMemcpyHostToDevice, H.stream));
        SA_HIP_CHECK(hipStreamSynchronize(H.stream));
        H.last_coarse_iters = 0;
        return;
    }
    if (H.coarse_kind == 1) {
        const int n = Ac.nrows;
        dense_symv(H.stream, n, H.c_L.p, rc, xc, false);
        spmv_residual(H.stream, Ac, xc, rc, H.c_r.p);
        dense_symv(H.stream, n, H.c_L.p, H.c_r.p, xc, true);
        H.last_coarse_iters = 0;
        return;
    }
    if (H.coarse_kind == 3) {
        blocktri_solve(H.stream, Ac, H.c_bt, rc, xc);
        H.last_coarse_iters = 0;
        return;
    }
    auto prec = [&](const double *r, double *z) {
        smooth_from_zero(H, Ac, H.c_dinv.p, H.c_roots, r, z, H.c_t0.p);
    };
    int conv = 0;
    H.last_coarse_iters = pcg_loop(H, Ac, prec, rc, xc, H.c_r.p, H.c_z.p, H.c_d.p, H.c_q.p,
                                   H.params.coarse_rtol, 0.0, H.params.coarse_max_iter, false, true,
                                   &conv, nullptr, H.scal.p + 4);
}

static Level::Dist *dist_of(Level &L) { return L.dist.on ? &L.dist : nullptr; }

static void user_smooth(Hierarchy &H, int level, int (*fn)(void *, int, int, const double *, double *), void *ctx,
                        const double *b, double *x, bool zero_start) {
    Level &L = *H.levels[level];
    SA_REQUIRE(!L.dist.on, "a caller's smoother cannot run on a level that is row-partitioned over several ranks");
    const size_t n = (size_t)L.A.nrows;
    hvec<double> hb(n), hx(n, 0.0);
    SA_HIP_CHECK(hipMemcpyAsync(hb.data(), b, 8 * n, hipMemcpyDeviceToHost, H.stream));
    if (!zero_start) SA_HIP_CHECK(hipMemcpyAsync(hx.data(), x, 8 * n, hipMemcpyDeviceToHost, H.stream));
    SA_HIP_CHECK(hipStreamSynchronize(H.stream));
    SA_REQUIRE(fn(ctx, level, (int)n, hb.data(), hx.data()) == 0, "the caller's smoother failed");
    SA_HIP_CHECK(hipMemcpyAsync(x, hx.data(), 8 * n, hipMemcpyHostToDevice, H.stream));
    SA_HIP_CHECK(hipStreamSynchronize(H.stream));
}

static void vcycle_rec(Hierarchy &H, int level, const double *b, double *x) {
    Level &L = *H.levels[level];
    hipStream_t s = H.stream;
    Level::Dist *D = dist_of(L);
    const bool last = (level + 1 == (int)H.levels.size());
    const Hierarchy::UserSmoother us = level < (int)H.user_smoothers.size() ? H.user_smoothers[level] : Hierarchy::UserSmoother();
    if (us.pre) user_smooth(H, level, us.pre, us.ctx, b, x, true);
    else smooth_from_zero(H, L.A, L.dinv_neg.p, L.roots, b, x, L.t0.p, D);
    halo_then(H, D, x, [&](hipStream_t q, RowRange rr) { spmv_residual(q, L.A, x, b, L.r.p, rr); });
    double *rc = last ? H.c_b.p : H.levels[level + 1]->b.p;
    double *xc = last ? H.c_x.p : H.levels[level + 1]->x.p;
    spmv(s, L.R, L.r.p, rc);
    if (D) {
        constexpr bool no_rs = false;
        if (!last && !no_rs && H.levels[level + 1]->dist.on) dist_reduce_scatter_rows(H, H.levels[level + 1]->dist, rc);
        else dist_allreduce(H, rc, L.R.nrows);
    }
    if (last) {
        coarse_solve(H, rc, xc);
    } else {
        vcycle_rec(H, level + 1, rc, xc);
        Level &N = *H.levels[level + 1];
        if (N.dist.on) dist_allgather_rows(H, N.dist, xc);
    }
    spmv_add(s, L.P, xc, x, rows_of(D));
    if (us.post) user_smooth(H, level, us.post, us.ctx, b, x, false);
    else smooth_inplace(H, L.A, L.dinv_neg.p, L.roots, b, x, L.t0.p, D);
}

void smoother_apply(Hierarchy &H, int level, const double *b, double *x) {
    Level &L = *H.levels[level];
    Level::Dist *D = dist_of(L);
    smooth_inplace(H, L.A, L.dinv_neg.p, L.roots, b, x, L.t0.p, D);
    if (D) dist_allgather_rows(H, *D, x);
}

void vcycle_apply(Hierarchy &H, int level, const double *b, double *x) {
    vcycle_rec(H, level, b, x);
    Level &L = *H.levels[level];
    if (L.dist.on) dist_allgather_rows(H, L.dist, x);
}

int pcg_solve(Hierarchy &H, const double *b, double *x, double rel_tol, double abs_tol,
              int max_iter, int squared_tol, int zero_guess, int *converged, double *hist) {
    Level &L0 = *H.levels[0];
    Level::Dist *D = dist_of(L0);
    auto prec = [&](const double *r, double *z) { vcycle_rec(H, 0, r, z); };
    PhaseTimer tm(H.stream);
    struct Lap { PhaseTimer &t; ~Lap() { t.lap("TOTAL pcg_solve", 0); } } lap{tm};
    const int it = pcg_loop(H, L0.A, prec, b, x, H.pcg_r.p, H.pcg_z.p, H.pcg_d.p, H.pcg_q.p, rel_tol,
                            abs_tol, max_iter, squared_tol != 0, zero_guess != 0, converged, hist,
                            H.scal.p, D);
    if (D) dist_allgather_rows(H, *D, x);
    return it;
}

__global__ __launch_bounds__(64) void scaling_p_kernel(const int *__restrict__ mis2d_I, const int *__restrict__ k,
                                                       const int *__restrict__ coloff,
                                                       const int64_t *__restrict__ u_off,
                                                       const double *__restrict__ U,
                                                       const int *__restrict__ active, roff_t *__restrict__ prow,
                                                       int *__restrict__ pcol, double *__restrict__ pval) {
    extern __shared__ double xs[];
    const int m = blockIdx.x, lane = threadIdx.x;
    const int km = k[m];
    if (km == 0) return;
    const int r = mis2d_I[m + 1] - mis2d_I[m];
    const double *Um = U + u_off[m];
    double nn = 0.0;
    for (int v = 0; v < km; ++v) {
        double sum = 0.0;
        for (int i = lane; i < r; i += 64) sum += Um[(size_t)v * r + i];
#pragma unroll
        for (int o = 32; o > 0; o >>= 1) sum += __shfl_xor(sum, o, 64);
        if (lane == 0) xs[v] = sum;
        nn = fma(sum, sum, nn);
    }
    __syncthreads();
    const double inv = 1.0 / sqrt(nn);
    for (int v = lane; v < km; v += 64) {
        const int row = coloff[m] + v;
        prow[row] = row;
        pcol[row] = active[m];
        pval[row] = xs[v] * inv;
    }
}

static void add_nullspace_level(Hierarchy &H) {
    hipStream_t s = H.stream;
    Level &L = *H.levels.back();
    const int nm = L.rel.num_mises;
    const int nc = L.Ac.nrows;
    SA_REQUIRE(!H.params.testmesh, "the corrected null-space level is not available with the mltest fixture vectors");
    std::vector<int> active((size_t)nm, -1);
    int nact = 0, kmax = 1;
    for (int m = 0; m < nm; ++m)
        if (L.mis_k[m] > 0) { active[m] = nact++; kmax = std::max(kmax, L.mis_k[m]); }
    H.levels.emplace_back(new Level);
    Level &N = *H.levels.back();
    N.A = std::move(L.Ac);
    N.theta = 0.0;
    N.nu_relax = 3;
    N.roots = sas_poly_roots(3);
    build_sell(s, N.A, H.params.opt);
    N.dinv_neg.alloc((size_t)nc);
    {
        DBuf<double> tmp((size_t)nc);
        build_dinv_neg(s, N.A, tmp.p, N.dinv_neg.p);
        SA_HIP_CHECK(hipStreamSynchronize(s));
    }
    N.P.nrows = nc;
    N.P.ncols = nact;
    N.P.nnz = nc;
    N.P.rowptr.alloc((size_t)nc + 1);
    N.P.col.alloc((size_t)nc + 1);
    N.P.val.alloc((size_t)nc + 1);
    DBuf<int> d_active;
    d_active.from_host(active, s);
    hipLaunchKernelGGL(scaling_p_kernel, dim3(nm), dim3(64), sizeof(double) * (size_t)kmax, s, L.drel.mis2d_I.p,
                       L.d_mis_k.p, L.d_mis_coloff.p, L.d_mis_u_off.p, L.mis_U.p, d_active.p, N.P.rowptr.p,
                       N.P.col.p, N.P.val.p);
    SA_HIP_CHECK(hipGetLastError());
    const roff_t nc_off = nc;
    SA_HIP_CHECK(hipMemcpyAsync(N.P.rowptr.p + nc, &nc_off, sizeof(roff_t), hipMemcpyHostToDevice, s));
    SA_HIP_CHECK(hipStreamSynchronize(s));
    N.P.lanes_per_row = 1;
    csr_transpose(s, N.P, N.R);
    DCsr AP;
    spgemm(s, N.A, N.P, nullptr, nullptr, 1.0, 0.0, AP);
    spgemm(s, N.R, AP, nullptr, nullptr, 1.0, 0.0, N.Ac);
    N.rel.ND = nc;
    N.rel.nparts = nact;
    N.x.alloc((size_t)nc); N.b.alloc((size_t)nc); N.r.alloc((size_t)nc); N.t0.alloc((size_t)nc);
}

Hierarchy *hierarchy_create(int n, const void *Arow, int rowptr_bits, const int *Acol, const double *Aval, int NE,
                            int nde, const int *elem_ptr, const int *elem_to_dof, const double *elmat,
                            const signed char *bdr, const int *const *partitions,
                            const int *nparts, const Params &p, hipStream_t stream, std::unique_ptr<DistIn> dist_inputs) {
    SA_REQUIRE(p.num_coarsenings >= 1 && p.num_coarsenings < MAX_LEVELS, "bad number of coarsenings");
    ae_rows_new_build();
    DBuf<int> iota_e2d;
    if (p.algebraic) {
        NE = n;
        nde = 1;
        iota_e2d.alloc((size_t)n);
        hipLaunchKernelGGL(iota_int_kernel, dim3(div_up(n, 256)), dim3(256), 0, stream, (long)n, iota_e2d.p);
        SA_HIP_CHECK(hipGetLastError());
        elem_to_dof = iota_e2d.p;
        elmat = nullptr;
        bdr = nullptr;
    }
    int max_nd = 0;
    if (elem_ptr) {
        SA_REQUIRE(!p.algebraic && !dist_inputs && elem_to_dof && elmat, "elem_ptr needs element arrays");
        SA_REQUIRE(n > 0 && NE > 0, "empty problem");
        nde = check_elem_ptr(NE, elem_ptr, elem_to_dof, n, max_nd, stream);
        if (nde) elem_ptr = nullptr;
    }
    SA_REQUIRE(n > 0 && NE > 0 && (nde > 0 || elem_ptr), "empty problem");
    PhaseTimer tm_all(stream), tm0(stream);
    std::unique_ptr<Hierarchy> Hp(new Hierarchy);
    Hierarchy &H = *Hp;
    H.params = p;
    H.stream = stream;
    H.device = current_device();
    H.own_e2d = std::move(iota_e2d);
    H.dist_in = std::move(dist_inputs);
    hipStream_t s = stream;
    H.scal.alloc(8);
    H.partials.alloc(1024);
    for (int l = 0; l < p.num_coarsenings; ++l) H.levels.emplace_back(new Level);
    Level &L0 = *H.levels[0];
    {
        import_rowptr(L0.A.rowptr, Arow, rowptr_bits, (size_t)n + 1, s);
        roff_t nnz = 0;
        SA_HIP_CHECK(hipMemcpyAsync(&nnz, L0.A.rowptr.p + n, sizeof(roff_t), hipMemcpyDeviceToHost, s));
        SA_HIP_CHECK(hipStreamSynchronize(s));
        L0.A.nrows = L0.A.ncols = n;
        L0.A.nnz = nnz;
        import_array(L0.A.col, Acol, (size_t)nnz, s);
        import_array(L0.A.val, Aval, (size_t)nnz, s);
        finish_csr(L0.A);
    }
    {
        L0.elmat.off.alloc((size_t)NE + 1);
        if (H.dist_in) {
            L0.elmat.off.zero(s);
            hipLaunchKernelGGL(iota64_kernel, dim3(div_up((long)H.dist_in->NE_loc + 1, 256)), dim3(256), 0, s, (long)H.dist_in->NE_loc + 1,
                               (int64_t)nde * nde, L0.elmat.off.p + H.dist_in->elem0);
            SA_HIP_CHECK(hipGetLastError());
            import_array(L0.elmat.val, elmat, (size_t)H.dist_in->NE_loc * nde * nde, s);
            L0.elmat.first = H.dist_in->elem0;
        } else if (elem_ptr) {
            import_array(H.e2d_ptr, elem_ptr, (size_t)NE + 1, s);
            DBuf<int> sq((size_t)NE);
            hipLaunchKernelGGL(elem_sq_kernel, dim3(div_up((long)NE, 256)), dim3(256), 0, s, (long)NE, H.e2d_ptr.p, sq.p);
            SA_HIP_CHECK(hipGetLastError());
            exclusive_scan_off(s, NE, sq.p, L0.elmat.off.p);
            int64_t total = 0;
            SA_HIP_CHECK(hipMemcpyAsync(&total, L0.elmat.off.p + NE, sizeof(int64_t), hipMemcpyDeviceToHost, s));
            SA_HIP_CHECK(hipStreamSynchronize(s));
            import_array(L0.elmat.val, elmat, (size_t)total, s);
            L0.elmat.max_nd = max_nd;
        } else {
        hipLaunchKernelGGL(iota64_kernel, dim3(div_up((long)NE + 1, 256)), dim3(256), 0, s, (long)NE + 1,
                           (int64_t)nde * nde, L0.elmat.off.p);
        SA_HIP_CHECK(hipGetLastError());
        if (!p.algebraic) import_array(L0.elmat.val, elmat, (size_t)NE * nde * nde, s);
        }
        L0.elmat.nde = nde;
        L0.elmat.algebraic = p.algebraic;
    }
    constexpr bool host_topo = false;
    DeviceInputs din;
    const bool dev_inputs = !host_topo && is_device_ptr(elem_to_dof) && is_device_ptr(partitions[0]) &&
                            (!bdr || is_device_ptr(bdr));
    Table e2d;
    hvec<signed char> bdr_h;
    if (dev_inputs) {
        din.e2d = elem_to_dof;
        din.part = partitions[0];
        din.bdr = bdr;
        din.NE = NE;
        din.nde = nde;
        din.e2d_I = elem_ptr ? H.e2d_ptr.p : nullptr;
    } else if (elem_ptr) {
        e2d.I = fetch_host(H.e2d_ptr.p, (size_t)NE + 1, s);
        e2d.J = fetch_host(elem_to_dof, (size_t)e2d.I[NE], s);
        e2d.ncols = n;
        if (bdr) bdr_h = fetch_host(bdr, (size_t)n, s);
    } else {
        auto J = fetch_host(elem_to_dof, (size_t)NE * nde, s);
        e2d.J = std::move(J);
        e2d.I.resize((size_t)NE + 1);
        for (int e = 0; e <= NE; ++e) e2d.I[e] = e * nde;
        e2d.ncols = n;
        if (bdr) bdr_h = fetch_host(bdr, (size_t)n, s);
    }
    H.coarse_parts.resize((size_t)p.num_coarsenings);
    H.nparts_in.assign(nparts, nparts + p.num_coarsenings);
    {
        int ne = nparts[0];
        for (int lev = 1; lev < p.num_coarsenings; ++lev) {
            H.coarse_parts[(size_t)lev] = fetch_host(partitions[lev], (size_t)ne, s);
            ne = nparts[lev];
        }
    }
    tm0.lap("inputs fetched/imported", 0);
    int n_elem = NE;
    for (int lev = 0; lev < p.num_coarsenings; ++lev) {
        hvec<int> part;
        if (lev > 0) part = H.coarse_parts[(size_t)lev];
        else if (!dev_inputs) part = fetch_host(partitions[lev], (size_t)n_elem, s);
        const bool tag_levels = (H.params.opt.debug & 4) != 0;
        profiler().level_tag = tag_levels ? lev : 0;
        build_level(H, lev, std::move(e2d), part, nparts[lev], (lev == 0 && bdr && !dev_inputs) ? bdr_h.data() : nullptr,
                    (lev == 0 && dev_inputs) ? &din : nullptr);
        Level &L = *H.levels[lev];
        if (lev + 1 < p.num_coarsenings) {
            PhaseTimer tm(s);
            e2d = prepare_next_level(H, lev);
            tm.lap("next-level elements", lev);
            Level &N = *H.levels[lev + 1];
            if (H.galerkin_lev == lev) {
                N.A = DCsr();
                N.A.nrows = N.A.ncols = L.mis_coloff.back();
            } else {
                N.A = std::move(L.Ac);
            }
            n_elem = L.rel.nparts;
        }
    }
    profiler().level_tag = 0;
    join_galerkin(H);
    tm0 = PhaseTimer(s);
    if (p.correct_nullspace) {
        add_nullspace_level(H);
        tm0.lap("corrected null-space level", 0);
    }
    setup_coarse_solver(H);
    const size_t nc = (size_t)coarsest_op(H).nrows;
    H.c_b.alloc(nc);
    H.c_x.alloc(nc);
    H.pcg_r.alloc((size_t)n); H.pcg_z.alloc((size_t)n); H.pcg_d.alloc((size_t)n); H.pcg_q.alloc((size_t)n);
    SA_HIP_CHECK(hipStreamSynchronize(s));
    tm0.lap("coarse solver + vectors", 0);
    if (p.world > 1 && p.alltoallv) {
        for (int lev = 0; lev < p.num_coarsenings; ++lev)
            if (!dist_setup_level(H, lev)) break;
        tm0.lap("row-partitioned solve: halo lists", 0);
    }
    tm_all.lap("TOTAL ml_produce_data", 0);
    if (env_timing()) {
        long nm_ = 0, nf_ = 0;
        size_t mb_ = 0;
        dev_pool_counts(&nm_, &nf_, &mb_, true);
        std::fprintf(stderr, "TIMING: device pool: %ld hipMalloc (%.1f MB), %ld hipFree of cached blocks, %.1f GB idle\n", nm_, mb_ / 1048576.0, nf_,
                     dev_pool_idle_bytes() / 1073741824.0);
    }
    return Hp.release();
}

void hierarchy_update_operators(Hierarchy &H, const double *new_val) {
    hipStream_t s = H.stream;
    const int nspec = H.params.num_coarsenings;
    Level &L0 = *H.levels[0];
    if (new_val && new_val != L0.A.val.p) {
        if (is_device_ptr(new_val)) {
            L0.A.val.view(const_cast<double *>(new_val), (size_t)L0.A.nnz);
        } else {
            if (!L0.A.val.owned) L0.A.val.alloc((size_t)L0.A.nnz);
            SA_HIP_CHECK(hipMemcpyAsync(L0.A.val.p, new_val, sizeof(double) * (size_t)L0.A.nnz,
                                        hipMemcpyHostToDevice, s));
            SA_HIP_CHECK(hipStreamSynchronize(s));
        }
    }
    for (int lev = 0; lev < nspec; ++lev) {
        Level &L = *H.levels[lev];
        build_sell(s, L.A, H.params.opt);
        {
            DBuf<double> tmp((size_t)L.A.nrows);
            build_dinv_neg(s, L.A, tmp.p, L.dinv_neg.p);
            build_dinv_codes(s, L.A, L.dinv_neg.p, H.params.opt);
            SA_HIP_CHECK(hipStreamSynchronize(s));
        }
        L.Ac = DCsr();
        level_galerkin(H, lev, false);
        if (lev + 1 < (int)H.levels.size()) H.levels[lev + 1]->A = std::move(L.Ac);
    }
    if (H.params.correct_nullspace) {
        Level &N = *H.levels.back();
        build_sell(s, N.A, H.params.opt);
        DBuf<double> tmp((size_t)N.A.nrows);
        build_dinv_neg(s, N.A, tmp.p, N.dinv_neg.p);
        SA_HIP_CHECK(hipStreamSynchronize(s));
        DCsr AP;
        spgemm(s, N.A, N.P, nullptr, nullptr, 1.0, 0.0, AP);
        N.Ac = DCsr();
        spgemm(s, N.R, AP, nullptr, nullptr, 1.0, 0.0, N.Ac);
    }
    H.c_L.release();
    setup_coarse_solver(H);
    SA_HIP_CHECK(hipStreamSynchronize(s));
}

}
```

### saamge_amd/csrc/mis.h

```cpp
#pragma once
#include "common.h"
#include "topology.h"

namespace saamge_amd {

struct MisSvdIO {
    const int *ae_m = nullptr;
    const int64_t *ae_xoff = nullptr;
    const double *evecs = nullptr;
    const int64_t *g_off = nullptr;
    double *gather = nullptr;
    const int64_t *u_off = nullptr;
    const int64_t *s_off = nullptr;
    double *U = nullptr;
    double *sig = nullptr;
    int *k = nullptr;
    int *ncols = nullptr;
    int avoid_ess = 1;
    int debug = 0;
    const double *extra = nullptr;
    int nextra = 0, ND = 0;
};

void mis_svd(hipStream_t s, const DevRelations &rel, int num_mises, int max_ctot, const MisSvdIO &io, int m0 = 0,
             const int *ae_ev = nullptr);

void build_P_R(hipStream_t s, const DevRelations &rel, const Relations &hrel,
               const std::vector<int> &h_k, const std::vector<int64_t> &h_u_off, const int *d_k,
               const int *d_coloff, const int64_t *d_u_off, const double *U, DCsr &P, DCsr &R);

bool coarse_e2d_device(hipStream_t s, const DevRelations &rel, const Relations &hrel, const int *d_mis_k,
                       const int *d_mis_coloff, int ncoarse, const roff_t *p_rowptr, const double *p_val,
                       DBuf<int> &colpos_ptr, DBuf<int> &colpos, Table &e2d);

void rap_mis(hipStream_t s, const DevRelations &rel, const Relations &hrel, const DCsr &A,
             const std::vector<int> &h_k, const std::vector<int> &h_coloff, const int *d_k,
             const int *d_coloff, const int64_t *d_u_off, const double *U, DCsr &Ac, int rank = 0,
             int world = 1, std::vector<long long> *nnz_off = nullptr);

}
```

### saamge_amd/csrc/mis.hip

```cpp
#include "mis.h"
#include "assemble.h"

#include <cfloat>

namespace saamge_amd {

__device__ inline double wsum(double v) {
#pragma unroll
    for (int o = 32; o > 0; o >>= 1) v += __shfl_xor(v, o, 64);
    return v;
}

__global__ __launch_bounds__(64) void mis_svd_kernel(
    const int *__restrict__ mis2d_I, const int *__restrict__ mis2d_J,
    const int *__restrict__ mis2ae_I, const int *__restrict__ mis2ae_J,
    const int *__restrict__ ae2d_I, const int64_t *__restrict__ pair_loc_off,
    const int *__restrict__ pair_loc, const signed char *__restrict__ flags, MisSvdIO io, int m0,
    const int *__restrict__ list = nullptr) {
    extern __shared__ __align__(16) double lds[];
    const int m = list ? list[blockIdx.x] : m0 + (int)blockIdx.x;
    const int lane = threadIdx.x;
    const int r = mis2d_I[m + 1] - mis2d_I[m];
    const int *dofs = mis2d_J + mis2d_I[m];
    double *M = io.gather + io.g_off[m];
// ... 158 lines not shown
    const signed char *flags;
    MisSvdIO io;
    const int *ae_ev;
};
__device__ inline unsigned long long mi_mix(unsigned long long x) {
    x += 0x9E3779B97F4A7C15ull;
    x = (x ^ (x >> 30)) * 0xBF58476D1CE4E5B9ull;
    x = (x ^ (x >> 27)) * 0x94D049BB133111EBull;
    return x ^ (x >> 31);
}
template <bool PAIR, class F>
__device__ inline bool mis_walk(const MisIn &v, int m, int m2, int lane, F &&f) {
    const int r = v.mis2d_I[m + 1] - v.mis2d_I[m], qb = v.mis2ae_I[m], nq = v.mis2ae_I[m + 1] - qb;
    const int ctot = (int)(v.io.s_off[m + 1] - v.io.s_off[m]);
    const int *dofs = v.mis2d_J + v.mis2d_I[m];
    const int qb2 = PAIR ? v.mis2ae_I[m2] : 0;
    const int *dofs2 = PAIR ? v.mis2d_J + v.mis2d_I[m2] : nullptr;
    if (PAIR && (r != v.mis2d_I[m2 + 1] - v.mis2d_I[m2] || nq != v.mis2ae_I[m2 + 1] - qb2 ||
                 ctot != (int)(v.io.s_off[m2 + 1] - v.io.s_off[m2]))) return false;
    bool ok = true;
    if (!PAIR && lane == 0) { f(((unsigned long long)(unsigned)r << 32) | (unsigned)nq, 1ull); f((unsigned long long)(unsigned)ctot, 2ull); }
    if (v.io.avoid_ess || v.io.nextra) {
        for (int i = lane; i < r; i += 64) {
            const unsigned long long w = v.io.avoid_ess ? (unsigned long long)(v.flags[dofs[i]] & FLAG_ON_ESS_BORDER) : 0ull;
            if (PAIR) ok = ok && w == (v.io.avoid_ess ? (unsigned long long)(v.flags[dofs2[i]] & FLAG_ON_ESS_BORDER) : 0ull);
            else f(w, (1ull << 40) + (unsigned long long)i);
            for (int q = 0; q < v.io.nextra; ++q) {
                const unsigned long long x = (unsigned long long)__double_as_longlong(v.io.extra[(size_t)q * v.io.ND + dofs[i]]);
                if (PAIR) ok = ok && x == (unsigned long long)__double_as_longlong(v.io.extra[(size_t)q * v.io.ND + dofs2[i]]);
                else f(x, (2ull << 40) + ((unsigned long long)q << 24) + (unsigned long long)i);
            }
        }
    }
    for (int t = 0; t < nq; ++t) {
        const int ae = v.mis2ae_J[qb + t], na = v.ae2d_I[ae + 1] - v.ae2d_I[ae], ma = v.io.ae_m[ae];
        const int id = v.ae_ev[ae];
        const int *loc = v.pair_loc + v.pair_loc_off[qb + t];
        const unsigned long long tag = (unsigned long long)(t + 3) << 40;
        if (PAIR) {
            const int ae2 = v.mis2ae_J[qb2 + t];
            if (!(ae == ae2 || (id >= 0 && id == v.ae_ev[ae2])) || na != v.ae2d_I[ae2 + 1] - v.ae2d_I[ae2] || ma != v.io.ae_m[ae2]) return false;
            const int *loc2 = v.pair_loc + v.pair_loc_off[qb2 + t];
            for (int i = lane; i < r; i += 64) ok = ok && loc[i] == loc2[i];
        } else {
            if (lane == 0) {
                f(id >= 0 ? (unsigned long long)(unsigned)id : 0x8000000000000000ull + (unsigned long long)(unsigned)ae, tag);
                f(((unsigned long long)(unsigned)na << 32) | (unsigned)ma, tag + 1);
            }
            for (int i = lane; i < r; i += 64) f((unsigned long long)(unsigned)loc[i], tag + 2 + (unsigned long long)i);
        }
    }
    return ok;
}
__global__ __launch_bounds__(256) void mis_hash_kernel(MisIn v, int nm, unsigned long long *__restrict__ h) {
    const int m = blockIdx.x * 4 + (threadIdx.x >> 6), lane = threadIdx.x & 63;
    if (m >= nm) return;
    unsigned long long h1 = 0, h2 = 0;
    mis_walk<false>(v, m, 0, lane, [&](unsigned long long w, unsigned long long pos) {
        const unsigned long long k = mi_mix(w + 0x9E3779B97F4A7C15ull * (pos + 1));
        h1 += k;
        h2 += (k >> 32) * (k & 0xffffffffull);
    });
#pragma unroll
    for (int o = 32; o > 0; o >>= 1) { h1 += __shfl_xor(h1, o, 64); h2 += __shfl_xor(h2, o, 64); }
    if (lane == 0) { h[2 * (size_t)m] = h1; h[2 * (size_t)m + 1] = h2; }
}
constexpr unsigned long long MI_EMPTY = ~0ull;
__global__ __launch_bounds__(256) void mis_group_kernel(int nm, const unsigned long long *__restrict__ h, unsigned long long *__restrict__ keys,
                                                        int *__restrict__ first, unsigned mask, int *__restrict__ slot) {
    const int m = blockIdx.x * 256 + threadIdx.x;
    if (m >= nm) return;
    unsigned long long key = h[2 * (size_t)m];
    if (key == MI_EMPTY) key = 0;
    unsigned pos = (unsigned)(key ^ (key >> 32)) & mask;
    for (;;) {
        const unsigned long long cur = atomicCAS(keys + pos, MI_EMPTY, key);
        if (cur == MI_EMPTY || cur == key) break;
        pos = (pos + 1) & mask;
    }
    atomicMin(first + pos, m);
    slot[m] = (int)pos;
}
__global__ __launch_bounds__(256) void mis_rep_kernel2(int nm, const int *__restrict__ slot, const int *__restrict__ first, int *__restrict__ rep) {
    const int m = blockIdx.x * 256 + threadIdx.x;
    if (m < nm) rep[m] = first[slot[m]];
}
__global__ __launch_bounds__(256) void mis_verify_kernel(MisIn v, int nm, const unsigned long long *__restrict__ h, int *__restrict__ rep,
                                                         int *__restrict__ isrep) {
    const int m = blockIdx.x * 4 + (threadIdx.x >> 6), lane = threadIdx.x & 63;
    if (m >= nm) return;
    const int r0 = rep[m];
    bool same = true;
    if (r0 != m) {
        same = h[2 * (size_t)m + 1] == h[2 * (size_t)r0 + 1];
        if (same) same = mis_walk<true>(v, m, r0, lane, [](unsigned long long, unsigned long long) {});
        same = __ballot(!same) == 0ull;
    }
    if (lane == 0) {
        if (!same) rep[m] = m;
        isrep[m] = (r0 == m || !same) ? 1 : 0;
    }
}
__global__ __launch_bounds__(256) void mis_list_kernel(int nm, const int *__restrict__ isrep, const int *__restrict__ pos, int *__restrict__ list) {
    const int m = blockIdx.x * 256 + threadIdx.x;
    if (m < nm && isrep[m]) list[pos[m]] = m;
}
__global__ __launch_bounds__(256) void mis_copy_kernel(MisIn v, int nm, const int *__restrict__ rep) {
    const int m = blockIdx.x * 4 + (threadIdx.x >> 6), lane = threadIdx.x & 63;
    if (m >= nm) return;
    const int r0 = rep[m];
    if (r0 == m) return;
    const int r = v.mis2d_I[m + 1] - v.mis2d_I[m], k = v.io.k[r0], ctot = (int)(v.io.s_off[m + 1] - v.io.s_off[m]);
    if (lane == 0) { v.io.k[m] = k; v.io.ncols[m] = v.io.ncols[r0]; }
    const double *su = v.io.U + v.io.u_off[r0], *ss = v.io.sig + v.io.s_off[r0];
    double *du = v.io.U + v.io.u_off[m], *ds = v.io.sig + v.io.s_off[m];
    for (int i = lane; i < r * k; i += 64) du[i] = su[i];
    for (int i = lane; i < ctot; i += 64) ds[i] = ss[i];
}

void mis_svd(hipStream_t s, const DevRelations &rel, int num_mises, int max_ctot, const MisSvdIO &io, int m0, const int *ae_ev) {
    if (!num_mises) return;
    const size_t lds = (sizeof(double) + sizeof(int)) * (size_t)(max_ctot + 2);
    if (ae_ev && m0 == 0 && num_mises >= 4096) {
        const int nm = num_mises;
        profiler().begin(s);
        MisIn v{rel.mis2d_I.p, rel.mis2d_J.p, rel.mis2ae_I.p, rel.mis2ae_J.p, rel.ae2d_I.p, rel.pair_loc_off.p, rel.pair_loc.p, rel.flags.p, io, ae_ev};
        unsigned tsize = 1024;
        while (tsize < 4u * (unsigned)nm) tsize <<= 1;
        DBuf<unsigned long long> h(2 * (size_t)nm), keys((size_t)tsize);
        DBuf<int> first((size_t)tsize), slot((size_t)nm), rep((size_t)nm), isrep((size_t)nm), pos((size_t)nm + 1), list((size_t)nm);
        SA_HIP_CHECK(hipMemsetAsync(keys.p, 0xff, sizeof(unsigned long long) * (size_t)tsize, s));
        SA_HIP_CHECK(hipMemsetAsync(first.p, 0x7f, sizeof(int) * (size_t)tsize, s));
        hipLaunchKernelGGL(mis_hash_kernel, dim3(div_up(nm, 4)), dim3(256), 0, s, v, nm, h.p);
        hipLaunchKernelGGL(mis_group_kernel, dim3(div_up(nm, 256)), dim3(256), 0, s, nm, h.p, keys.p, first.p, tsize - 1, slot.p);
        hipLaunchKernelGGL(mis_rep_kernel2, dim3(div_up(nm, 256)), dim3(256), 0, s, nm, slot.p, first.p, rep.p);
        hipLaunchKernelGGL(mis_verify_kernel, dim3(div_up(nm, 4)), dim3(256), 0, s, v, nm, h.p, rep.p, isrep.p);
        SA_HIP_CHECK(hipGetLastError());
        exclusive_scan_int(s, nm, isrep.p, pos.p);
        hipLaunchKernelGGL(mis_list_kernel, dim3(div_up(nm, 256)), dim3(256), 0, s, nm, isrep.p, pos.p, list.p);
        SA_HIP_CHECK(hipGetLastError());
        int last[2] = {0, 0};
        SA_HIP_CHECK(hipMemcpyAsync(&last[0], pos.p + (nm - 1), sizeof(int), hipMemcpyDeviceToHost, s));
        SA_HIP_CHECK(hipMemcpyAsync(&last[1], isrep.p + (nm - 1), sizeof(int), hipMemcpyDeviceToHost, s));
        SA_HIP_CHECK(hipStreamSynchronize(s));
        const int nrep = last[0] + last[1];
        profiler().end(s, "eig_dedupe", 0.0, 0.0);
        if (io.debug & 1) std::fprintf(stderr, "MISes: %d distinct of %d\n", nrep, nm);
        profiler().begin(s);
        hipLaunchKernelGGL(mis_svd_kernel, dim3(nrep), dim3(64), lds, s, rel.mis2d_I.p,
                           rel.mis2d_J.p, rel.mis2ae_I.p, rel.mis2ae_J.p, rel.ae2d_I.p,
                           rel.pair_loc_off.p, rel.pair_loc.p, rel.flags.p, io, 0, list.p);
        hipLaunchKernelGGL(mis_copy_kernel, dim3(div_up(nm, 4)), dim3(256), 0, s, v, nm, rep.p);
        SA_HIP_CHECK(hipGetLastError());
        SA_HIP_CHECK(hipStreamSynchronize(s));
        profiler().end(s, "mis_svd", 0.0, 0.0);
        return;
    }
    profiler().begin(s);
    hipLaunchKernelGGL(mis_svd_kernel, dim3(num_mises), dim3(64), lds, s, rel.mis2d_I.p,
                       rel.mis2d_J.p, rel.mis2ae_I.p, rel.mis2ae_J.p, rel.ae2d_I.p,
                       rel.pair_loc_off.p, rel.pair_loc.p, rel.flags.p, io, m0);
    SA_HIP_CHECK(hipGetLastError());
    profiler().end(s, "mis_svd", 0.0, 0.0);
}

__global__ __launch_bounds__(256) void p_count_kernel(int ND, const int *__restrict__ mises,
                                                      const int *__restrict__ k, int *__restrict__ cnt) {
    const long i = (long)blockIdx.x * 256 + threadIdx.x;
    if (i < ND) cnt[i] = k[mises[i]];
}

__global__ __launch_bounds__(256) void r_len_kernel(int nm, const int *__restrict__ mis2d_I, const int *__restrict__ k,
                                                    const int *__restrict__ coloff, int *__restrict__ len) {
    const int m = blockIdx.x * 256 + threadIdx.x;
    if (m >= nm) return;
    const int r = mis2d_I[m + 1] - mis2d_I[m], c0 = coloff[m];
    for (int v = 0; v < k[m]; ++v) len[c0 + v] = r;
}

template <class OUT>
__global__ __launch_bounds__(256) void scan_tile_kernel(int n, const int *__restrict__ in,
                                                        OUT *__restrict__ out, OUT *__restrict__ tsum) {
    __shared__ OUT sh[256];
    const long base = (long)blockIdx.x * 1024;
    int v[4];
    OUT run = 0;
    for (int q = 0; q < 4; ++q) {
        const long i = base + threadIdx.x * 4 + q;
        v[q] = (i < n) ? in[i] : 0;
        run += v[q];
    }
    sh[threadIdx.x] = run;
    __syncthreads();
    for (int o = 1; o < 256; o <<= 1) {
        const OUT t = (threadIdx.x >= o) ? sh[threadIdx.x - o] : 0;
        __syncthreads();
        sh[threadIdx.x] += t;
        __syncthreads();
    }
    OUT excl = sh[threadIdx.x] - run;
    for (int q = 0; q < 4; ++q) {
        const long i = base + threadIdx.x * 4 + q;
        if (i < n) out[i] = excl;
        excl += v[q];
    }
    if (threadIdx.x == 255) tsum[blockIdx.x] = sh[255];
}
template <class OUT>
__global__ __launch_bounds__(256) void scan_sums_kernel(int nt, OUT *__restrict__ tsum, OUT *__restrict__ total) {
    __shared__ OUT sh[256];
    __shared__ OUT carry;
    if (threadIdx.x == 0) carry = 0;
    __syncthreads();
    for (int base = 0; base < nt; base += 256) {
        const int i = base + threadIdx.x;
        const OUT x = (i < nt) ? tsum[i] : 0;
        sh[threadIdx.x] = x;
        __syncthreads();
        for (int o = 1; o < 256; o <<= 1) {
            const OUT t = (threadIdx.x >= o) ? sh[threadIdx.x - o] : 0;
            __syncthreads();
            sh[threadIdx.x] += t;
            __syncthreads();
        }
        if (i < nt) tsum[i] = carry + sh[threadIdx.x] - x;
        __syncthreads();
        if (threadIdx.x == 255) carry += sh[255];
        __syncthreads();
    }
    if (threadIdx.x == 0) *total = carry;
}
template <class OUT>
__global__ __launch_bounds__(256) void scan_add_kernel(int n, OUT *__restrict__ out,
                                                       const OUT *__restrict__ tsum,
                                                       const OUT *__restrict__ total) {
    const long i = (long)blockIdx.x * 256 + threadIdx.x;
    if (i < n) out[i] += tsum[i >> 10];
    if (i == 0) out[n] = *total;
}

template <class OUT>
static void exclusive_scan_t(hipStream_t s, int n, const int *in, OUT *out) {
    const int nt = div_up(n, 1024);
    DBuf<OUT> tsum((size_t)nt + 1);
    hipLaunchKernelGGL(scan_tile_kernel<OUT>, dim3(nt), dim3(256), 0, s, n, in, out, tsum.p);
    hipLaunchKernelGGL(scan_sums_kernel<OUT>, dim3(1), dim3(256), 0, s, nt, tsum.p, tsum.p + nt);
    hipLaunchKernelGGL(scan_add_kernel<OUT>, dim3(div_up(n, 256)), dim3(256), 0, s, n, out, (const OUT *)tsum.p, (const OUT *)(tsum.p + nt));
    SA_HIP_CHECK(hipGetLastError());
    SA_HIP_CHECK(hipStreamSynchronize(s));
}
void exclusive_scan_int(hipStream_t s, int n, const int *in, int *out) { exclusive_scan_t<int>(s, n, in, out); }
void exclusive_scan_int_async(hipStream_t s, int n, const int *in, int *out, int *tsum) {
    const int nt = div_up(n, 1024);
    hipLaunchKernelGGL(scan_tile_kernel<int>, dim3(nt), dim3(256), 0, s, n, in, out, tsum);
    hipLaunchKernelGGL(scan_sums_kernel<int>, dim3(1), dim3(256), 0, s, nt, tsum, tsum + nt);
    hipLaunchKernelGGL(scan_add_kernel<int>, dim3(div_up(n, 256)), dim3(256), 0, s, n, out, (const int *)tsum, (const int *)(tsum + nt));
    SA_HIP_CHECK(hipGetLastError());
}
void exclusive_scan_off(hipStream_t s, int n, const int *in, roff_t *out) { exclusive_scan_t<roff_t>(s, n, in, out); }

__global__ __launch_bounds__(256) void p_fill_kernel(int ND, const int *__restrict__ mises,
                                                     const int *__restrict__ row_in_mis,
                                                     const int *__restrict__ mis2d_I,
                                                     const int *__restrict__ k,
                                                     const int *__restrict__ coloff,
                                                     const int64_t *__restrict__ u_off,
                                                     const double *__restrict__ U,
                                                     const roff_t *__restrict__ rowptr,
                                                     int *__restrict__ col, double *__restrict__ val) {
    const long i = (long)blockIdx.x * 256 + threadIdx.x;
    if (i >= ND) return;
    const int m = mises[i], km = k[m];
    const int r = mis2d_I[m + 1] - mis2d_I[m];
    const double *Um = U + u_off[m] + row_in_mis[i];
    const roff_t base = rowptr[i];
    const int c0 = coloff[m];
    for (int v = 0; v < km; ++v) {
        col[base + v] = c0 + v;
        val[base + v] = Um[(size_t)v * r];
    }
}

__global__ __launch_bounds__(256) void r_fill_kernel(int num_mises, const int *__restrict__ mis2d_I,
                                                     const int *__restrict__ mis2d_J,
                                                     const int *__restrict__ k,
                                                     const int *__restrict__ coloff,
                                                     const int64_t *__restrict__ u_off,
                                                     const double *__restrict__ U,
                                                     const roff_t *__restrict__ rowptr,
                                                     int *__restrict__ col, double *__restrict__ val) {
    const int m = blockIdx.x;
    const int km = k[m];
    if (km == 0) return;
    const int r = mis2d_I[m + 1] - mis2d_I[m];
    const int *dofs = mis2d_J + mis2d_I[m];
    const double *Um = U + u_off[m];
    for (int idx = threadIdx.x; idx < km * r; idx += 256) {
        const int v = idx / r, i = idx % r;
        const roff_t base = rowptr[coloff[m] + v];
        col[base + i] = dofs[i];
        val[base + i] = Um[(size_t)v * r + i];
    }
}

void build_P_R(hipStream_t s, const DevRelations &rel, const Relations &hrel,
               const std::vector<int> &h_k, const std::vector<int64_t> &h_u_off, const int *d_k,
               const int *d_coloff, const int64_t *d_u_off, const double *U, DCsr &P, DCsr &R) {
    (void)h_u_off;
    const int ND = hrel.ND;
    int nc = 0;
    int64_t nnz = 0;
    for (int m = 0; m < hrel.num_mises; ++m) {
        nc += h_k[m];
        nnz += (int64_t)h_k[m] * hrel.mis_to_dof.row_size(m);
    }
    P.nrows = ND; P.ncols = nc; P.nnz = nnz;
    P.rowptr.alloc((size_t)ND + 1);
    P.col.alloc((size_t)nnz);
    P.val.alloc((size_t)nnz);
    {
        DBuf<int> cnt((size_t)ND);
        hipLaunchKernelGGL(p_count_kernel, dim3(div_up(ND, 256)), dim3(256), 0, s, ND, rel.mises.p, d_k, cnt.p);
        exclusive_scan_off(s, ND, cnt.p, P.rowptr.p);
    }
    hipLaunchKernelGGL(p_fill_kernel, dim3(div_up(ND, 256)), dim3(256), 0, s, ND, rel.mises.p,
                       rel.dof_row_in_mis.p, rel.mis2d_I.p, d_k, d_coloff, d_u_off, U, P.rowptr.p,
                       P.col.p, P.val.p);
    P.lanes_per_row = pick_lanes_per_row(nnz, ND);
    R.nrows = nc; R.ncols = ND; R.nnz = nnz;
    {
        DBuf<int> len((size_t)std::max(nc, 1));
        R.rowptr.alloc((size_t)nc + 1);
        if (hrel.num_mises)
            hipLaunchKernelGGL(r_len_kernel, dim3(div_up(hrel.num_mises, 256)), dim3(256), 0, s, hrel.num_mises, rel.mis2d_I.p, d_k,
                               d_coloff, len.p);
        if (nc > 0) exclusive_scan_off(s, nc, len.p, R.rowptr.p);
        else SA_HIP_CHECK(hipMemsetAsync(R.rowptr.p, 0, sizeof(roff_t), s));
    }
    R.col.alloc((size_t)nnz);
    R.val.alloc((size_t)nnz);
    if (hrel.num_mises)
        hipLaunchKernelGGL(r_fill_kernel, dim3(hrel.num_mises), dim3(256), 0, s, hrel.num_mises,
                           rel.mis2d_I.p, rel.mis2d_J.p, d_k, d_coloff, d_u_off, U, R.rowptr.p,
                           R.col.p, R.val.p);
    SA_HIP_CHECK(hipGetLastError());
    R.lanes_per_row = pick_lanes_per_row(nnz, nc > 0 ? nc : 1);
}

__global__ __launch_bounds__(256) void ae_mis_k_kernel(long n, const int *__restrict__ ae2mis_J,
                                                       const int *__restrict__ k, int *__restrict__ out) {
    const long i = (long)blockIdx.x * 256 + threadIdx.x;
    if (i < n) out[i] = k[ae2mis_J[i]];
}

__global__ __launch_bounds__(256) void ae_ke_max_kernel(int nparts, const int *__restrict__ ae2mis_I,
                                                        const int *__restrict__ colpos_ptr, int *__restrict__ out) {
    const int e = blockIdx.x * 256 + threadIdx.x;
    int ke = 0;
    if (e < nparts) ke = colpos_ptr[ae2mis_I[e + 1]] - colpos_ptr[ae2mis_I[e]];
#pragma unroll
    for (int o = 32; o > 0; o >>= 1) ke = max(ke, __shfl_xor(ke, o, 64));
    if ((threadIdx.x & 63) == 0) atomicMax(out, ke);
}

__global__ __launch_bounds__(256) void coarse_e2d_kernel(
    const int *__restrict__ ae2d_I, const int *__restrict__ ae2d_J, const int *__restrict__ ae2mis_I,
    const int *__restrict__ ae2mis_J, const int *__restrict__ mises, const int *__restrict__ mis_k,
    const int *__restrict__ mis_coloff, const int *__restrict__ colpos_ptr, const roff_t *__restrict__ prow,
    const double *__restrict__ pval, int cap, int *__restrict__ colpos, int *__restrict__ e2d_J,
    int *__restrict__ err) {
    extern __shared__ unsigned long long ce_keys[];
    int *cd = (int *)(ce_keys + cap);
    const int e = blockIdx.x, tid = threadIdx.x;
    const int tb = ae2mis_I[e], te = ae2mis_I[e + 1];
    const int c0 = colpos_ptr[tb], KE = colpos_ptr[te] - c0;
    for (int t = tb + tid; t < te; t += 256) {
        const int m = ae2mis_J[t], km = mis_k[m], base = colpos_ptr[t] - c0, co = mis_coloff[m];
        for (int v = 0; v < km; ++v) {
            ce_keys[base + v] = ~0ull;
            cd[base + v] = co + v;
        }
    }
    __syncthreads();
    const int d0 = ae2d_I[e], d1 = ae2d_I[e + 1];
    for (int k = d0 + tid; k < d1; k += 256) {
        const int dof = ae2d_J[k], m = mises[dof], km = mis_k[m];
        if (km == 0) continue;
        int lo = tb, hi = te;
        while (lo < hi) {
            const int mid = (lo + hi) >> 1;
            if (ae2mis_J[mid] < m) lo = mid + 1; else hi = mid;
        }
        const int base = colpos_ptr[lo] - c0;
        const roff_t pr = prow[dof];
        for (int v = 0; v < km; ++v)
            if (pval[pr + v] != 0.0)
                atomicMin(&ce_keys[base + v], ((unsigned long long)(unsigned)(k - d0) << 32) | (unsigned)(base + v));
    }
    __syncthreads();
    for (int idx = tid; idx < KE; idx += 256) {
        const unsigned long long key = ce_keys[idx];
        if (key == ~0ull) {
            colpos[c0 + idx] = -1;
            atomicExch(err, 1);
            continue;
        }
        int rank = 0;
        for (int j = 0; j < KE; ++j) rank += (ce_keys[j] < key) ? 1 : 0;
        colpos[c0 + idx] = rank;
        e2d_J[c0 + rank] = cd[idx];
    }
}

bool coarse_e2d_device(hipStream_t s, const DevRelations &rel, const Relations &hrel, const int *d_mis_k,
                       const int *d_mis_coloff, int ncoarse, const roff_t *p_rowptr, const double *p_val,
                       DBuf<int> &colpos_ptr, DBuf<int> &colpos, Table &e2d) {
    const int nparts = hrel.nparts;
    const long npairs = (long)hrel.AE_to_mis.J.size();
    if (nparts == 0 || npairs == 0) return false;
    DBuf<int> kk((size_t)npairs), info(2);
    info.zero(s);
    hipLaunchKernelGGL(ae_mis_k_kernel, dim3(div_up(npairs, 256)), dim3(256), 0, s, npairs, rel.ae2mis_J.p, d_mis_k, kk.p);
    colpos_ptr.alloc((size_t)npairs + 1);
    exclusive_scan_int(s, (int)npairs, kk.p, colpos_ptr.p);
    hipLaunchKernelGGL(ae_ke_max_kernel, dim3(div_up(nparts, 256)), dim3(256), 0, s, nparts, rel.ae2mis_I.p, colpos_ptr.p, info.p);
    SA_HIP_CHECK(hipGetLastError());
    const int cap = info.to_host(s)[0];
    const size_t lds = (size_t)cap * 12 + 16;
    if (lds > 60 * 1024) return false;
    auto h_ptr = colpos_ptr.to_host(s);
    const int total = h_ptr[(size_t)npairs];
    colpos.alloc((size_t)total + 1);
    DBuf<int> d_J((size_t)total + 1);
    if (total) {
        hipLaunchKernelGGL(coarse_e2d_kernel, dim3(nparts), dim3(256), lds, s, rel.ae2d_I.p, rel.ae2d_J.p, rel.ae2mis_I.p,
                           rel.ae2mis_J.p, rel.mises.p, d_mis_k, d_mis_coloff, colpos_ptr.p, p_rowptr, p_val, cap, colpos.p,
                           d_J.p, info.p + 1);
        SA_HIP_CHECK(hipGetLastError());
    }
    SA_REQUIRE(info.to_host(s)[1] == 0, "coarse dof with an all-zero prolongator column in an AE");
    e2d.ncols = ncoarse;
    e2d.I.resize((size_t)nparts + 1);
    for (int e = 0; e <= nparts; ++e) e2d.I[e] = h_ptr[(size_t)hrel.AE_to_mis.I[e]];
    e2d.J.resize((size_t)total);
    if (total) {
        SA_HIP_CHECK(hipMemcpyAsync(e2d.J.data(), d_J.p, sizeof(int) * (size_t)total, hipMemcpyDeviceToHost, s));
        SA_HIP_CHECK(hipStreamSynchronize(s));
    }
    return true;
}

constexpr int RAP_NT = 256;
constexpr int RAP_HASH = 2048;
constexpr int RAP_SMALL_ROWS = 64;
constexpr int RAP_SUB = 64;
constexpr int RAP_ROW_CLAMP = 1 << 24;

typedef unsigned long long rap_word_t;
constexpr rap_word_t RAP_K0 = 1ull << 63;
__global__ __launch_bounds__(256) void rap_pack_kernel(int n, const int *__restrict__ mises, const int *__restrict__ row_in_mis,
                                                       const int *__restrict__ k, rap_word_t *__restrict__ pack) {
    const long i = (long)blockIdx.x * 256 + threadIdx.x;
    if (i >= n) return;
    const int m = mises[i];
    pack[i] = (rap_word_t)(unsigned)m | ((rap_word_t)(unsigned)row_in_mis[i] << 32) | (k[m] == 0 ? RAP_K0 : 0ull);
}

__device__ inline void rap_row_prefix(int nr, const int *__restrict__ dofs, const roff_t *__restrict__ Arow, int clamp,
                                      int *pre, roff_t *qs) {
    if (threadIdx.x >= 64) return;
    const int l = threadIdx.x;
    int len = 0;
    if (l < nr) {
        const int g = dofs[l];
        const roff_t q0 = Arow[g], n = Arow[g + 1] - q0;
        len = n < (roff_t)clamp ? (int)n : clamp;
        qs[l] = q0;
    }
    int inc = len;
#pragma unroll
    for (int o = 1; o < 64; o <<= 1) {
        const int t = __shfl_up(inc, o, 64);
        if (l >= o) inc += t;
    }
    if (l < nr) pre[l + 1] = inc;
    if (l == 0) pre[0] = 0;
}

__device__ inline int rap_entry_row(const int *pre, int ra, int rb, int base, int e) {
    int lo = ra, hi = rb;
    while (hi - lo > 1) {
        const int mid = (lo + hi) >> 1;
        if (pre[mid] - base <= e) lo = mid; else hi = mid;
    }
    return lo;
}

template <int NT, int CAP>
__global__ __launch_bounds__(NT) void rap_symbolic_kernel(
    const int *__restrict__ mlist, int pass, const int *__restrict__ mis2d_I, const int *__restrict__ mis2d_J,
    const roff_t *__restrict__ Arow, const int *__restrict__ Acol, const rap_word_t *__restrict__ pack,
    const int *__restrict__ k, int *__restrict__ cnt, const int *__restrict__ nbr_ptr,
    int *__restrict__ nbr, int *__restrict__ err, int *__restrict__ stage = nullptr, int stage_cap = 0,
    int maxrow = 0) {
    __shared__ int table[CAP];
    __shared__ int nfound;
    __shared__ roff_t qs[RAP_SUB];
    __shared__ int pre[RAP_SUB + 1];
    const int m1 = mlist ? mlist[blockIdx.x] : (int)blockIdx.x;
    if (k[m1] == 0) {
        if (pass == 0 && threadIdx.x == 0) cnt[m1] = 0;
        return;
    }
    const int r1 = mis2d_I[m1 + 1] - mis2d_I[m1];
    const int *dofs = mis2d_J + mis2d_I[m1];
    __shared__ int overflow;
    int HS = CAP;
    if (maxrow > 0) {
        const long bound = 2l * r1 * maxrow;
        HS = 64;
        while (HS < 256 && HS < bound) HS <<= 1;
    }
    const bool certain = maxrow > 0 && 2l * r1 * maxrow <= HS;
    for (;;) {
        for (int i = threadIdx.x; i < HS; i += NT) table[i] = -1;
        if (threadIdx.x == 0) { nfound = 0; overflow = 0; }
        __syncthreads();
        for (int s0 = 0; s0 < r1; s0 += RAP_SUB) {
            const int nr = min(RAP_SUB, r1 - s0);
            rap_row_prefix(nr, dofs + s0, Arow, RAP_ROW_CLAMP, pre, qs);
            __syncthreads();
            const int ne = pre[nr];
            for (int e = threadIdx.x; e < ne; e += NT) {
                const int row = rap_entry_row(pre, 0, nr, 0, e);
                const rap_word_t w = pack[Acol[qs[row] + (e - pre[row])]];
                if (w & RAP_K0) continue;
                const int m2 = (int)(unsigned)w;
                unsigned h = hash_home((unsigned)m2, (unsigned)HS);
                for (int probe = 0; probe < HS; ++probe) {
                    const int old = atomicCAS(&table[h], -1, m2);
                    if (old == -1) { atomicAdd(&nfound, 1); break; }
                    if (old == m2) break;
                    h = (h + 1) & (HS - 1);
                    if (probe == HS - 1) { if (HS == RAP_HASH) atomicExch(err, 1); else overflow = 1; }
                }
            }
            __syncthreads();
        }
        const bool full = !certain && (overflow || 2 * nfound > HS);
        const bool again = HS < CAP && full;
        __syncthreads();
        if (CAP < RAP_HASH && full && !again) {
            if (threadIdx.x == 0) cnt[m1] = -1;
            return;
        }
        if (!again) break;
        HS = CAP;
    }
    if (pass == 0) {
        if (threadIdx.x == 0) cnt[m1] = nfound;
        if (!stage || nfound > stage_cap) return;
    }
    __shared__ int list[CAP];
    __shared__ int nlist;
    if (threadIdx.x == 0) nlist = 0;
    __syncthreads();
    for (int i = threadIdx.x; i < HS; i += NT) {
        const int v = table[i];
        if (v >= 0) list[atomicAdd(&nlist, 1)] = v;
    }
    __syncthreads();
    const int nl = nlist;
    int *out = (pass == 0) ? stage + (size_t)m1 * stage_cap : nbr + nbr_ptr[m1];
    for (int i = threadIdx.x; i < nl; i += NT) {
        const int v = list[i];
        int rank = 0;
        for (int j = 0; j < nl; ++j) rank += (list[j] < v);
        out[rank] = v;
    }
}

__global__ __launch_bounds__(256) void rap_unstage_kernel(int nm, int cap, const int *__restrict__ stage,
                                                          const int *__restrict__ nbr_ptr, int *__restrict__ nbr) {
    const long i = (long)blockIdx.x * 256 + threadIdx.x;
    const int m = (int)(i / cap), t = (int)(i % cap);
    if (m < nm && t < nbr_ptr[m + 1] - nbr_ptr[m]) nbr[nbr_ptr[m] + t] = stage[i];
}

__device__ inline void rap_walk_row(roff_t qb, roff_t qe, const int *__restrict__ Acol, const double *__restrict__ Aval,
                                    const rap_word_t *__restrict__ pack, const double *__restrict__ U, int nn,
                                    const int *nbl, const long long *uo, const int *kk, const int *rr, const int *pos,
                                    double *Trow) {
    for (roff_t q0 = qb; q0 < qe; q0 += 4) {
        int jj4[4], lo4[4], rim4[4];
        double a4[4], u4[4];
        bool on4[4];
        rap_word_t w4[4];
#pragma unroll
        for (int t = 0; t < 4; ++t) {
            const roff_t q = min(q0 + t, qe - 1);
            jj4[t] = Acol[q];
            a4[t] = Aval[q];
// ... 53 lines not shown
        nbl[t] = m2;
        kk[t] = k[m2];
        rr[t] = mis2d_I[m2 + 1] - mis2d_I[m2];
        uo[t] = u_off[m2];
    }
    __syncthreads();
    if (tid == 0) {
        int run = 0;
        for (int t = 0; t < nn; ++t) { pos[t] = run; run += kk[t]; }
        pos[nn] = run;
    }
    __syncthreads();
    const int ncol = pos[nn];
    double *acc = lds + pos_d;
    const int rows_total = (lds_doubles - pos_d) / ncol;
    const int KC = (k1 + 1 <= rows_total) ? k1 : rows_total / 2;
    const int RC = rows_total - KC;
    double *T = acc + (size_t)KC * ncol;
    for (int idx = tid; idx < k1 * ncol; idx += NT) {
        const int v1 = idx / ncol, cc = idx % ncol;
        int lo = 0, hi = nn;
        while (hi - lo > 1) { const int mid = (lo + hi) >> 1; if (pos[mid] <= cc) lo = mid; else hi = mid; }
        ccol[crowptr[coloff[m1] + v1] + cc] = coloff[nbl[lo]] + (cc - pos[lo]);
    }
    for (int v0 = 0; v0 < k1; v0 += KC) {
        const int kc = min(KC, k1 - v0);
        __syncthreads();
        for (int i = tid; i < kc * ncol; i += NT) acc[i] = 0.0;
        for (int c0 = 0; c0 < r1; c0 += RC) {
            const int rc = min(RC, r1 - c0);
            __syncthreads();
            for (int i = tid; i < rc * ncol; i += NT) T[i] = 0.0;
            __syncthreads();
            for (int il = tid; il < rc; il += NT) {
                const int g = dofs[c0 + il];
                rap_walk_row(Arow[g], Arow[g + 1], Acol, Aval, pack, U, nn, nbl, uo, kk, rr, pos, T + (size_t)il * ncol);
            }
            __syncthreads();
            for (int idx = tid; idx < kc * ncol; idx += NT) {
                const int v1 = idx / ncol, cc = idx % ncol;
                double sum = acc[idx];
                const double *u = U1 + (size_t)(v0 + v1) * r1 + c0;
                for (int il = 0; il < rc; ++il) sum = fma(u[il], T[(size_t)il * ncol + cc], sum);
                acc[idx] = sum;
            }
        }
        __syncthreads();
        for (int idx = tid; idx < kc * ncol; idx += NT) {
            const int v1 = idx / ncol, cc = idx % ncol;
            cval[crowptr[coloff[m1] + v0 + v1] + cc] = acc[idx];
        }
    }
}

enum { RAP_SC_AGAIN = 0, RAP_SC_CNT_MAX, RAP_SC_NEED_MAX, RAP_SC_SMALL_MAX, RAP_SC_SMALL_LDS, RAP_NSC };

__global__ __launch_bounds__(256) void rap_sym_class_kernel(int nm, const int *__restrict__ mis2d_I, int *__restrict__ fa,
                                                            int *__restrict__ fb) {
    const int m = blockIdx.x * 256 + threadIdx.x;
    if (m >= nm) return;
    const int small = mis2d_I[m + 1] - mis2d_I[m] <= RAP_SMALL_ROWS;
    fa[m] = small;
    fb[m] = !small;
}

__global__ __launch_bounds__(256) void rap_cnt_stats_kernel(int nm, const int *__restrict__ cnt, int *__restrict__ fa,
                                                            unsigned long long *__restrict__ sc) {
    const int m = blockIdx.x * 256 + threadIdx.x;
    const int c = m < nm ? cnt[m] : 0;
    int neg = c < 0, mx = max(c, 0);
    if (m < nm) fa[m] = neg;
#pragma unroll
    for (int o = 32; o > 0; o >>= 1) {
        neg += __shfl_xor(neg, o, 64);
        mx = max(mx, __shfl_xor(mx, o, 64));
    }
    if ((threadIdx.x & 63) == 0) {
        if (neg) atomicAdd(&sc[RAP_SC_AGAIN], (unsigned long long)neg);
        if (mx) atomicMax(&sc[RAP_SC_CNT_MAX], (unsigned long long)mx);
    }
}

__global__ __launch_bounds__(256) void rap_size_kernel(int nm, const int *__restrict__ k, const int *__restrict__ coloff,
                                                       const int *__restrict__ mis2d_I, const int *__restrict__ nbr_ptr,
                                                       const int *__restrict__ nbr, unsigned long long cap,
                                                       int *__restrict__ rowlen, int *__restrict__ small_need,
                                                       unsigned long long *__restrict__ sc) {
    typedef unsigned long long u64;
    const int m = blockIdx.x * 256 + threadIdx.x;
    u64 need = 0, small = 0;
    if (m < nm) {
        const int km = k[m];
        int sn = 0;
        if (km > 0) {
            const int t0 = nbr_ptr[m], t1 = nbr_ptr[m + 1];
            int ncol = 0;
            for (int t = t0; t < t1; ++t) ncol += k[nbr[t]];
            for (int v = 0; v < km; ++v) rowlen[coloff[m] + v] = ncol;
            const u64 tables = (u64)(3 * (t1 - t0) + 2);
            need = tables + (u64)(km + 1) * ncol;
            if (need > cap) need = max(tables + 2ull * ncol, min(need, cap));
            small = tables + (u64)(km + 8) * ncol;
            const u64 all = tables + (u64)(km + (mis2d_I[m + 1] - mis2d_I[m])) * ncol;
            sn = (int)min(min(all, max((u64)1024, small)), (u64)(1u << 30));
        }
        small_need[m] = sn;
    }
#pragma unroll
    for (int o = 32; o > 0; o >>= 1) {
        need = max(need, (u64)__shfl_xor((long long)need, o, 64));
        small = max(small, (u64)__shfl_xor((long long)small, o, 64));
    }
    if ((threadIdx.x & 63) == 0) {
        if (need) atomicMax(&sc[RAP_SC_NEED_MAX], need);
        if (small) atomicMax(&sc[RAP_SC_SMALL_MAX], small);
    }
}

__global__ __launch_bounds__(256) void rap_num_class_kernel(int nm, int m_lo, int m_hi, const int *__restrict__ k,
                                                            const int *__restrict__ mis2d_I, const int *__restrict__ small_need,
                                                            int *__restrict__ fa, int *__restrict__ fb,
                                                            unsigned long long *__restrict__ sc) {
    const int m = blockIdx.x * 256 + threadIdx.x;
    int lds = 0;
    if (m < nm) {
        const bool on = m >= m_lo && m < m_hi && k[m] > 0;
        const bool small = on && mis2d_I[m + 1] - mis2d_I[m] <= RAP_SMALL_ROWS && small_need[m] <= 2048;
        fa[m] = small;
        fb[m] = on && !small;
        if (small) lds = small_need[m];
    }
#pragma unroll
    for (int o = 32; o > 0; o >>= 1) lds = max(lds, __shfl_xor(lds, o, 64));
    if ((threadIdx.x & 63) == 0 && lds) atomicMax(&sc[RAP_SC_SMALL_LDS], (unsigned long long)lds);
}

__global__ __launch_bounds__(256) void rap_scatter_kernel(int nm, const int *__restrict__ flag, const int *__restrict__ pos,
                                                          int *__restrict__ list) {
    const int m = blockIdx.x * 256 + threadIdx.x;
    if (m < nm && flag[m]) list[pos[m]] = m;
}

static int rap_compact(hipStream_t s, int nm, const int *flag, int *pos, DBuf<int> &list) {
    exclusive_scan_int(s, nm, flag, pos);
    int n = 0;
    SA_HIP_CHECK(hipMemcpyAsync(&n, pos + nm, sizeof(int), hipMemcpyDeviceToHost, s));
    SA_HIP_CHECK(hipStreamSynchronize(s));
    list.alloc((size_t)n);
    if (n) hipLaunchKernelGGL(rap_scatter_kernel, dim3(div_up(nm, 256)), dim3(256), 0, s, nm, flag, (const int *)pos, list.p);
    return n;
}

void rap_mis(hipStream_t s, const DevRelations &rel, const Relations &hrel, const DCsr &A,
             const std::vector<int> &h_k, const std::vector<int> &h_coloff, const int *d_k,
             const int *d_coloff, const int64_t *d_u_off, const double *U, DCsr &Ac, int rank, int world,
             std::vector<long long> *nnz_off) {
    const int nm = hrel.num_mises;
    int nc = 0;
    for (int m = 0; m < nm; ++m) nc += h_k[m];
    Ac.nrows = Ac.ncols = nc;
    Ac.nnz = 0;
    if (nm == 0 || nc == 0) {
        Ac.rowptr.from_host(std::vector<roff_t>(1, 0), s);
        return;
    }
    DBuf<int> cnt((size_t)nm), err(1);
    err.zero(s);
    if (A.max_row < 0) A.max_row = csr_max_row(s, A);
    const int maxrow = A.max_row;
    SA_REQUIRE(maxrow <= RAP_ROW_CLAMP, "RAP: a row of A is too long");
    profiler().begin(s);
    DBuf<rap_word_t> pack((size_t)A.nrows);
    hipLaunchKernelGGL(rap_pack_kernel, dim3(div_up(A.nrows, 256)), dim3(256), 0, s, A.nrows, rel.mises.p, rel.dof_row_in_mis.p, d_k, pack.p);
    constexpr int STAGE_CAP = 64;
    DBuf<int> stage((size_t)nm * STAGE_CAP);
    DBuf<int> fa((size_t)nm), fb((size_t)nm), pos((size_t)nm + 1);
    DBuf<unsigned long long> sc(RAP_NSC);
    const dim3 gm(div_up(nm, 256));
    {
        hipLaunchKernelGGL(rap_sym_class_kernel, gm, dim3(256), 0, s, nm, rel.mis2d_I.p, fa.p, fb.p);
        DBuf<int> d_sym_small, d_sym_big;
        const int n_small = rap_compact(s, nm, fa.p, pos.p, d_sym_small), n_big = rap_compact(s, nm, fb.p, pos.p, d_sym_big);
        if (n_big)
            hipLaunchKernelGGL((rap_symbolic_kernel<RAP_NT, RAP_HASH>), dim3((unsigned)n_big), dim3(RAP_NT), 0, s, d_sym_big.p, 0,
                               rel.mis2d_I.p, rel.mis2d_J.p, A.rowptr.p, A.col.p, pack.p, d_k, cnt.p, nullptr, nullptr, err.p, stage.p,
                               STAGE_CAP, maxrow);
        if (n_small)
            hipLaunchKernelGGL((rap_symbolic_kernel<64, 256>), dim3((unsigned)n_small), dim3(64), 0, s, d_sym_small.p, 0,
                               rel.mis2d_I.p, rel.mis2d_J.p, A.rowptr.p, A.col.p, pack.p, d_k, cnt.p, nullptr, nullptr, err.p, stage.p,
                               STAGE_CAP, maxrow);
        SA_HIP_CHECK(hipGetLastError());
        SA_HIP_CHECK(hipStreamSynchronize(s));
    }
    sc.zero(s);
    hipLaunchKernelGGL(rap_cnt_stats_kernel, gm, dim3(256), 0, s, nm, cnt.p, fa.p, sc.p);
    SA_HIP_CHECK(hipGetLastError());
    auto h_sc = sc.to_host(s);
    if (h_sc[RAP_SC_AGAIN]) {
        DBuf<int> d_again;
        const int n_again = rap_compact(s, nm, fa.p, pos.p, d_again);
        hipLaunchKernelGGL((rap_symbolic_kernel<RAP_NT, RAP_HASH>), dim3((unsigned)n_again), dim3(RAP_NT), 0, s, d_again.p, 0,
                           rel.mis2d_I.p, rel.mis2d_J.p, A.rowptr.p, A.col.p, pack.p, d_k, cnt.p, nullptr, nullptr, err.p, stage.p,
                           STAGE_CAP, maxrow);
        sc.zero(s);
        hipLaunchKernelGGL(rap_cnt_stats_kernel, gm, dim3(256), 0, s, nm, cnt.p, fa.p, sc.p);
        SA_HIP_CHECK(hipGetLastError());
        h_sc = sc.to_host(s);
    }
    SA_REQUIRE(err.to_host(s)[0] == 0 && h_sc[RAP_SC_AGAIN] == 0, "RAP: MIS neighbour table overflow");
    const int cnt_max = (int)h_sc[RAP_SC_CNT_MAX];
    DBuf<int> nbr_ptr((size_t)nm + 1);
    exclusive_scan_int(s, nm, cnt.p, nbr_ptr.p);
    int nbr_total = 0;
    SA_HIP_CHECK(hipMemcpyAsync(&nbr_total, nbr_ptr.p + nm, sizeof(int), hipMemcpyDeviceToHost, s));
    SA_HIP_CHECK(hipStreamSynchronize(s));
    DBuf<int> nbr((size_t)nbr_total + 1);
    if (cnt_max <= STAGE_CAP)
        hipLaunchKernelGGL(rap_unstage_kernel, dim3(div_up((long)nm * STAGE_CAP, 256)), dim3(256), 0, s, nm, STAGE_CAP, stage.p,
                           nbr_ptr.p, nbr.p);
    else
        hipLaunchKernelGGL((rap_symbolic_kernel<RAP_NT, RAP_HASH>), dim3(nm), dim3(RAP_NT), 0, s, (const int *)nullptr, 1, rel.mis2d_I.p,
                           rel.mis2d_J.p, A.rowptr.p, A.col.p, pack.p, d_k, cnt.p, nbr_ptr.p, nbr.p, err.p, (int *)nullptr, 0,
                           maxrow);
    DBuf<int> rowlen((size_t)nc), small_need((size_t)nm);
    sc.zero(s);
    hipLaunchKernelGGL(rap_size_kernel, gm, dim3(256), 0, s, nm, d_k, d_coloff, rel.mis2d_I.p, nbr_ptr.p, nbr.p,
                       (unsigned long long)(160 * 1024 / 8), rowlen.p, small_need.p, sc.p);
    SA_HIP_CHECK(hipGetLastError());
    Ac.rowptr.alloc((size_t)nc + 1);
    exclusive_scan_off(s, nc, rowlen.p, Ac.rowptr.p);
    roff_t nnz = 0;
    SA_HIP_CHECK(hipMemcpyAsync(&nnz, Ac.rowptr.p + nc, sizeof(roff_t), hipMemcpyDeviceToHost, s));
    h_sc = sc.to_host(s);
    const size_t need_max = (size_t)h_sc[RAP_SC_NEED_MAX], small_max = (size_t)h_sc[RAP_SC_SMALL_MAX];
    size_t lds_doubles = std::max((size_t)2048, small_max);
    if (need_max > 8192) lds_doubles = need_max;
    SA_REQUIRE(lds_doubles * 8 <= 160 * 1024, "RAP: MIS block too wide for LDS");
    SA_HIP_CHECK(hipFuncSetAttribute((const void *)rap_numeric_kernel<RAP_NT>, hipFuncAttributeMaxDynamicSharedMemorySize, 160 * 1024));
    SA_HIP_CHECK(hipFuncSetAttribute((const void *)rap_numeric_kernel<64>, hipFuncAttributeMaxDynamicSharedMemorySize, 160 * 1024));
    Ac.nnz = nnz;
    Ac.col.alloc((size_t)nnz);
    Ac.val.alloc((size_t)nnz);
    int m_lo = 0, m_hi = nm;
    if (world > 1 && nnz_off) {
        const auto crow = Ac.rowptr.to_host(s);
        std::vector<int> mb((size_t)world + 1, nm);
        mb[0] = 0;
        int r = 0;
        for (int m = 0; m < nm && r + 1 < world; ++m) {
            const int64_t done = crow[(size_t)h_coloff[m + 1]];
            while (r + 1 < world && done >= nnz * (r + 1) / world) mb[++r] = m + 1;
        }
        mb[world] = nm;
        nnz_off->assign((size_t)world + 1, 0);
        for (int q = 0; q <= world; ++q) (*nnz_off)[q] = crow[(size_t)h_coloff[mb[q]]];
        m_lo = mb[rank];
        m_hi = mb[rank + 1];
    }
    hipLaunchKernelGGL(rap_num_class_kernel, gm, dim3(256), 0, s, nm, m_lo, m_hi, d_k, rel.mis2d_I.p, small_need.p, fa.p, fb.p, sc.p);
    DBuf<int> d_small, d_big;
    const int n_small = rap_compact(s, nm, fa.p, pos.p, d_small), n_big = rap_compact(s, nm, fb.p, pos.p, d_big);
    const size_t small_lds = (size_t)sc.to_host(s)[RAP_SC_SMALL_LDS];
    if (n_big)
        hipLaunchKernelGGL(rap_numeric_kernel<RAP_NT>, dim3((unsigned)n_big), dim3(RAP_NT), lds_doubles * 8, s,
                           d_big.p, 0, rel.mis2d_I.p, rel.mis2d_J.p, A.rowptr.p, A.col.p, A.val.p, pack.p,
                           d_k, d_coloff, d_u_off, U, nbr_ptr.p, nbr.p, Ac.rowptr.p,
                           Ac.col.p, Ac.val.p, (int)lds_doubles);
    if (n_small) {
        const size_t sl = std::max((size_t)256, small_lds);
        hipLaunchKernelGGL(rap_numeric_kernel<64>, dim3((unsigned)n_small), dim3(64), sl * 8, s,
                           d_small.p, 0, rel.mis2d_I.p, rel.mis2d_J.p, A.rowptr.p, A.col.p, A.val.p, pack.p,
                           d_k, d_coloff, d_u_off, U, nbr_ptr.p, nbr.p, Ac.rowptr.p,
                           Ac.col.p, Ac.val.p, (int)sl);
    }
    SA_HIP_CHECK(hipGetLastError());
    SA_HIP_CHECK(hipStreamSynchronize(s));
    profiler().end(s, "rap", 12.0 * (double)(A.nnz + nnz) + 4.0 * A.nrows, 0.0);
    Ac.lanes_per_row = pick_lanes_per_row(nnz, nc);
}

}
```

Baseline: 70.04 million DoF/s.

## Compute MIS offsets and counts on device and defer coarse e2d readback

Moves the per-MIS size and offset computation (goff/u_off/s_off, column offsets, nnz, kmax) from host loops to device kernels with scans, so only a few scalars are read back and host MIS mirrors are fetched lazily when needed. The coarse element-to-dof table readback now runs asynchronously on a side stream behind an event, and its error check is deferred until the table is consumed. This cuts host-device synchronisations and host serial loops during setup, in exchange for more kernel launches, lazy-mirror mutex logic, and delayed error reporting.

```diff
diff --git a/saamge_amd/csrc/capi.hip b/saamge_amd/csrc/capi.hip
--- a/saamge_amd/csrc/capi.hip
+++ b/saamge_amd/csrc/capi.hip
@@ -437,10 +437,8 @@
     info[7] = tot;
     info[8] = H.last_coarse_iters;
     info[9] = L.ae_xoff.empty() ? 0 : L.ae_xoff.back();
-    info[10] = L.mis_s_off.empty() ? 0 : L.mis_s_off.back();
-    long long usz = 0;
-    for (int m = 0; m < L.rel.num_mises; ++m) usz += (long long)L.mis_k[m] * L.rel.mis_to_dof.row_size(m);
-    info[11] = usz;
+    info[10] = L.mis_s_total;
+    info[11] = L.mis_nnz;
     info[12] = L.dist.on ? 1 : 0;
     info[13] = L.dist.row0;
     info[14] = L.dist.nloc;
@@ -550,6 +548,7 @@
         fetch_relations_ae_host(Lw.rel, Lw.drel, h->H->stream);
     }
     const Level &L = *h->H->levels.at(level);
+    L.mis_mirrors(h->H->stream);
     if (mises) std::copy(L.rel.mises.begin(), L.rel.mises.end(), mises);
     if (mis_k) std::copy(L.mis_k.begin(), L.mis_k.end(), mis_k);
     if (mis_ncols) std::copy(L.mis_ncols.begin(), L.mis_ncols.end(), mis_ncols);
@@ -581,6 +580,7 @@
     const Level &L = *H.levels.at(level);
     hipStream_t s = H.stream;
     const int nm = L.rel.num_mises;
+    L.mis_mirrors(s);
     if (sig_off) for (int m = 0; m <= nm; ++m) sig_off[m] = L.mis_s_off[m];
     if (sig) {
         SA_REQUIRE(H.params.keep_debug, "hierarchy was built without keep_debug");
diff --git a/saamge_amd/csrc/common.h b/saamge_amd/csrc/common.h
--- a/saamge_amd/csrc/common.h
+++ b/saamge_amd/csrc/common.h
@@ -4,6 +4,7 @@
 #include <cstdint>
 #include <cstdio>
 #include <cstring>
+#include <mutex>
 #include <type_traits>
 #include <stdexcept>
 #include <string>
@@ -163,6 +164,52 @@
     }
 };
 
+struct PendingCopy {
+    mutable std::mutex mu;
+    mutable hipEvent_t ev = nullptr;
+    PendingCopy() {}
+    PendingCopy(PendingCopy &&o) noexcept : ev(o.ev) { o.ev = nullptr; }
+    PendingCopy &operator=(PendingCopy &&o) noexcept {
+        if (this != &o) { drop(); ev = o.ev; o.ev = nullptr; }
+        return *this;
+    }
+    ~PendingCopy() { drop(); }
+    bool pending() const { std::lock_guard<std::mutex> lk(mu); return ev != nullptr; }
+    void record(hipStream_t s) {
+        wait();
+        std::lock_guard<std::mutex> lk(mu);
+        SA_HIP_CHECK(hipEventCreateWithFlags(&ev, hipEventDisableTiming));
+        SA_HIP_CHECK(hipEventRecord(ev, s));
+    }
+    void wait() const {
+        std::lock_guard<std::mutex> lk(mu);
+        if (!ev) return;
+        const hipError_t e = hipEventSynchronize(ev);
+        (void)hipEventDestroy(ev);
+        ev = nullptr;
+        SA_HIP_CHECK(e);
+    }
+private:
+    void drop() noexcept {
+        if (!ev) return;
+        (void)hipEventSynchronize(ev);
+        (void)hipEventDestroy(ev);
+        ev = nullptr;
+    }
+};
+
+inline hipStream_t readback_stream_behind(hipStream_t s) {
+    hipStream_t rs = side_stream(8);
+    hipEvent_t ready = nullptr;
+    SA_HIP_CHECK(hipEventCreateWithFlags(&ready, hipEventDisableTiming));
+    const hipError_t e1 = hipEventRecord(ready, s);
+    const hipError_t e2 = e1 == hipSuccess ? hipStreamWaitEvent(rs, ready, 0) : e1;
+    (void)hipEventDestroy(ready);
+    SA_HIP_CHECK(e1);
+    SA_HIP_CHECK(e2);
+    return rs;
+}
+
 template <class T>
 inline void import_array(DBuf<T> &dst, const T *src, size_t n, hipStream_t s) {
     if (is_device_ptr(src))
diff --git a/saamge_amd/csrc/hierarchy.h b/saamge_amd/csrc/hierarchy.h
--- a/saamge_amd/csrc/hierarchy.h
+++ b/saamge_amd/csrc/hierarchy.h
@@ -1,6 +1,7 @@
 #pragma once
 #include <exception>
 #include <memory>
+#include <mutex>
 #include <thread>
 
 #include "assemble.h"
@@ -53,6 +54,7 @@
     std::vector<int> colpos_ptr, colpos;
     DBuf<int> d_colpos_ptr, d_colpos;
     bool on_device = false;
+    CoarseE2dPending pending;
 };
 
 struct Level {
@@ -76,13 +78,19 @@
     std::vector<int64_t> ae_xoff, ae_eoff;
     DBuf<double> evals, evecs;
     DBuf<double> ae_D;
-    std::vector<int> mis_k;
-    std::vector<int> mis_coloff;
-    std::vector<int> mis_ncols;
-    std::vector<int64_t> mis_u_off, mis_s_off;
+    mutable hvec<int> mis_k;
+    mutable hvec<int> mis_coloff;
+    mutable hvec<int> mis_ncols;
+    mutable hvec<int64_t> mis_u_off, mis_s_off;
+    mutable std::mutex mis_mx;
+    mutable bool mis_host = false;
+    bool mis_off_host = false;
+    void mis_mirrors(hipStream_t s) const;
+    int mis_nc = 0, mis_kmax = 0;
+    int64_t mis_nnz = 0, mis_s_total = 0;
     DBuf<double> mis_U, mis_sig;
-    DBuf<int> d_mis_k, d_mis_coloff;
-    DBuf<int64_t> d_mis_u_off;
+    DBuf<int> d_mis_k, d_mis_coloff, d_mis_ncols;
+    DBuf<int64_t> d_mis_u_off, d_mis_s_off;
     DBuf<double> x, b, r, t0, t1;
     DBuf<double> extra;
     DBuf<double> cvec_next;
diff --git a/saamge_amd/csrc/hierarchy.hip b/saamge_amd/csrc/hierarchy.hip
--- a/saamge_amd/csrc/hierarchy.hip
+++ b/saamge_amd/csrc/hierarchy.hip
@@ -138,6 +138,24 @@
     if (i < n) p[i] = v;
 }
 
+void Level::mis_mirrors(hipStream_t s) const {
+    std::lock_guard<std::mutex> lk(mis_mx);
+    if (mis_host) return;
+    auto fetch = [&](auto &h, const auto &d) {
+        h.resize(d.n);
+        if (d.n) SA_HIP_CHECK(hipMemcpyAsync(h.data(), d.p, d.n * sizeof(h[0]), hipMemcpyDeviceToHost, s));
+    };
+    fetch(mis_k, d_mis_k);
+    fetch(mis_ncols, d_mis_ncols);
+    fetch(mis_coloff, d_mis_coloff);
+    if (!mis_off_host) {
+        fetch(mis_u_off, d_mis_u_off);
+        fetch(mis_s_off, d_mis_s_off);
+    }
+    SA_HIP_CHECK(hipStreamSynchronize(s));
+    mis_host = true;
+}
+
 static void level_galerkin(Hierarchy &H, int lev, bool first, hipStream_t s) {
     Level &L = *H.levels[lev];
     const Params &P = H.params;
@@ -145,7 +163,8 @@
     const int world = P.world > 1 ? P.world : 1;
     if (P.nu_pro[lev] == 0) {
         std::vector<long long> nnz_off;
-        rap_mis(s, L.drel, rel, L.A, L.mis_k, L.mis_coloff, L.d_mis_k.p, L.d_mis_coloff.p,
+        if (world > 1) L.mis_mirrors(s);
+        rap_mis(s, L.drel, rel, L.A, L.mis_nc, L.mis_coloff, L.d_mis_k.p, L.d_mis_coloff.p,
                 L.d_mis_u_off.p, L.mis_U.p, L.Ac, P.rank, world, world > 1 ? &nnz_off : nullptr);
         if (world > 1 && L.Ac.nnz > 0) {
             std::vector<long long> off((size_t)world + 1);
@@ -752,34 +771,44 @@
     if (mis_err) std::rethrow_exception(mis_err);
     tm.lap("MIS tables (join)", lev);
     const int nm = rel.num_mises;
-    std::vector<int64_t> g_off((size_t)nm + 1, 0);
-    L.mis_u_off.assign((size_t)nm + 1, 0);
-    L.mis_s_off.assign((size_t)nm + 1, 0);
-    int max_ctot = 0;
     const int nextra = (lev == 0 && P.extra_modes) ? P.num_extra_modes : 0;
     if (nextra) import_array(L.extra, P.extra_modes, (size_t)nextra * L.A.nrows, s);
-    for (int m = 0; m < nm; ++m) {
-        int ctot = nextra;
-        for (int q = rel.mis_to_AE.I[m]; q < rel.mis_to_AE.I[m + 1]; ++q) ctot += L.ae_m[rel.mis_to_AE.J[q]];
-        const int r = rel.mis_to_dof.row_size(m);
-        g_off[m + 1] = g_off[m] + (int64_t)r * ctot;
-        L.mis_u_off[m + 1] = L.mis_u_off[m] + (int64_t)r * std::max(1, std::min(r, ctot));
-        L.mis_s_off[m + 1] = L.mis_s_off[m] + ctot;
-        max_ctot = std::max(max_ctot, ctot);
-    }
-    L.mis_U.alloc((size_t)L.mis_u_off[nm]);
-    L.mis_sig.alloc((size_t)L.mis_s_off[nm] + 1);
+    DBuf<int64_t> d_goff((size_t)nm + 1), d_xoff;
+    DBuf<int> d_aem;
+    L.d_mis_u_off.alloc((size_t)nm + 1);
+    L.d_mis_s_off.alloc((size_t)nm + 1);
+    d_aem.from_host(L.ae_m, s);
+    d_xoff.from_host(L.ae_xoff, s);
+    MisSizes sz;
+    if (world > 1) {
+        std::vector<int64_t> g_off((size_t)nm + 1, 0);
+        L.mis_u_off.assign((size_t)nm + 1, 0);
+        L.mis_s_off.assign((size_t)nm + 1, 0);
+        for (int m = 0; m < nm; ++m) {
+            int ctot = nextra;
+            for (int q = rel.mis_to_AE.I[m]; q < rel.mis_to_AE.I[m + 1]; ++q) ctot += L.ae_m[rel.mis_to_AE.J[q]];
+            const int r = rel.mis_to_dof.row_size(m);
+            g_off[m + 1] = g_off[m] + (int64_t)r * ctot;
+            L.mis_u_off[m + 1] = L.mis_u_off[m] + (int64_t)r * std::max(1, std::min(r, ctot));
+            L.mis_s_off[m + 1] = L.mis_s_off[m] + ctot;
+            sz.max_ctot = std::max(sz.max_ctot, ctot);
+        }
+        sz.g_total = g_off[nm]; sz.u_total = L.mis_u_off[nm]; sz.s_total = L.mis_s_off[nm];
+        L.mis_off_host = true;
+        d_goff.from_host(g_off, s);
+        L.d_mis_s_off.from_host(L.mis_s_off, s);
+        L.d_mis_u_off.from_host(L.mis_u_off, s);
+    } else {
+        sz = mis_stage_offsets(s, L.drel, nm, nextra, d_aem.p, d_goff.p, L.d_mis_u_off.p, L.d_mis_s_off.p);
+    }
+    const int max_ctot = sz.max_ctot;
+    L.mis_U.alloc((size_t)sz.u_total);
+    L.mis_sig.alloc((size_t)sz.s_total + 1);
     L.mis_sig.zero(s);
     L.d_mis_k.alloc((size_t)nm);
+    L.d_mis_ncols.alloc((size_t)nm);
     {
-        double *gather = scratch_get(1, (size_t)g_off[nm] + 1);
-        DBuf<int64_t> d_goff, d_soff, d_xoff;
-        DBuf<int> d_aem, d_ncols((size_t)nm);
-        d_goff.from_host(g_off, s);
-        d_soff.from_host(L.mis_s_off, s);
-        L.d_mis_u_off.from_host(L.mis_u_off, s);
-        d_xoff.from_host(L.ae_xoff, s);
-        d_aem.from_host(L.ae_m, s);
+        double *gather = scratch_get(1, (size_t)sz.g_total + 1);
         MisSvdIO io;
         io.ae_m = d_aem.p;
         io.ae_xoff = d_xoff.p;
@@ -787,11 +816,11 @@
         io.g_off = d_goff.p;
         io.gather = gather;
         io.u_off = L.d_mis_u_off.p;
-        io.s_off = d_soff.p;
+        io.s_off = L.d_mis_s_off.p;
         io.U = L.mis_U.p;
         io.sig = L.mis_sig.p;
         io.k = L.d_mis_k.p;
-        io.ncols = d_ncols.p;
+        io.ncols = L.d_mis_ncols.p;
         io.avoid_ess = P.avoid_ess_bdr_dofs;
         io.extra = nextra ? L.extra.p : nullptr;
         io.nextra = nextra;
@@ -814,7 +843,7 @@
             }
             mb[world] = nm;
             L.d_mis_k.zero(s);
-            d_ncols.zero(s);
+            L.d_mis_ncols.zero(s);
             mis_svd(s, L.drel, mb[P.rank + 1] - mb[P.rank], max_ctot, io, mb[P.rank]);
             std::vector<long long> off((size_t)world + 1);
             for (int r = 0; r <= world; ++r) off[r] = 8ll * L.mis_u_off[mb[r]];
@@ -823,7 +852,7 @@
             SA_REQUIRE(P.allgather(P.allgather_ctx, L.mis_sig.p, off.data()) == 0, "all-gather (singular values) failed");
             for (int r = 0; r <= world; ++r) off[r] = 4ll * mb[r];
             SA_REQUIRE(P.allgather(P.allgather_ctx, L.d_mis_k.p, off.data()) == 0, "all-gather (MIS counts) failed");
-            SA_REQUIRE(P.allgather(P.allgather_ctx, d_ncols.p, off.data()) == 0, "all-gather (MIS columns) failed");
+            SA_REQUIRE(P.allgather(P.allgather_ctx, L.d_mis_ncols.p, off.data()) == 0, "all-gather (MIS columns) failed");
         } else {
             DBuf<int> d_ev;
             bool any = false;
@@ -831,15 +860,18 @@
             if (any && P.opt.eig_dedupe != 0 && !(P.testmesh && lev == 0)) d_ev.from_host(L.ae_evclass, s);
             mis_svd(s, L.drel, nm, max_ctot, io, 0, d_ev.n ? d_ev.p : nullptr);
         }
-        { auto t_ = L.d_mis_k.to_host(s); L.mis_k.assign(t_.begin(), t_.end()); }
-        { auto t_ = d_ncols.to_host(s); L.mis_ncols.assign(t_.begin(), t_.end()); }
     }
     tm.lap("MIS gather + SVD", lev);
-    L.mis_coloff.assign((size_t)nm + 1, 0);
-    for (int m = 0; m < nm; ++m) L.mis_coloff[m + 1] = L.mis_coloff[m] + L.mis_k[m];
-    L.d_mis_coloff.from_host(L.mis_coloff, s);
-    build_P_R(s, L.drel, rel, L.mis_k, L.mis_u_off, L.d_mis_k.p, L.d_mis_coloff.p, L.d_mis_u_off.p,
-              L.mis_U.p, L.P, L.R);
+    L.d_mis_coloff.alloc((size_t)nm + 1);
+    const MisCounts cnts = mis_col_offsets(s, L.drel, nm, L.d_mis_k.p, L.d_mis_coloff.p);
+    d_aem.release();
+    d_xoff.release();
+    d_goff.release();
+    L.mis_s_total = sz.s_total;
+    L.mis_nc = cnts.nc;
+    L.mis_kmax = cnts.kmax;
+    L.mis_nnz = cnts.nnz;
+    build_P_R(s, L.drel, rel, cnts.nc, cnts.nnz, L.d_mis_k.p, L.d_mis_coloff.p, L.d_mis_u_off.p, L.mis_U.p, L.P, L.R);
     if (lev + 1 < P.num_coarsenings) {
         L.cvec_next.alloc((size_t)L.R.nrows);
         const double *cv = nullptr;
@@ -859,8 +891,8 @@
     constexpr bool host_e2d = false;
     if (lev + 1 < P.num_coarsenings && P.nu_pro[lev] == 0 && !host_e2d) {
         NextPrep &np = L.next_prep;
-        np.on_device = coarse_e2d_device(s, L.drel, rel, L.d_mis_k.p, L.d_mis_coloff.p, L.mis_coloff.back(),
-                                         L.P.rowptr.p, L.P.val.p, np.d_colpos_ptr, np.d_colpos, np.e2d);
+        np.on_device = coarse_e2d_device(s, L.drel, rel, L.d_mis_k.p, L.d_mis_coloff.p, L.mis_nc,
+                                         L.P.rowptr.p, L.P.val.p, np.d_colpos_ptr, np.d_colpos, np.e2d, np.pending);
         np.ready = np.on_device;
     }
     if (lev + 1 < P.num_coarsenings && P.nu_pro[lev] == 0 && !L.next_prep.ready) {
@@ -915,8 +947,9 @@
     fetch_relations_ae_host(const_cast<Relations &>(L.rel), L.drel, s);
     const Relations &rel = L.rel;
     const int nparts = rel.nparts;
+    L.mis_mirrors(s);
     Table &e2d = out.e2d;
-    e2d.ncols = L.mis_coloff.back();
+    e2d.ncols = L.mis_nc;
     e2d.I.assign((size_t)nparts + 1, 0);
     hvec<roff_t> p_rowptr((size_t)p_nrows + 1);
     hvec<double> p_val((size_t)p_nnz + 1);
@@ -992,8 +1025,8 @@
         NextPrep &np = L.next_prep;
         constexpr bool host_e2d = false;
         if (!host_e2d)
-            np.on_device = coarse_e2d_device(s, L.drel, rel, L.d_mis_k.p, L.d_mis_coloff.p, L.mis_coloff.back(),
-                                             PT.rowptr.p, PT.val.p, np.d_colpos_ptr, np.d_colpos, np.e2d);
+            np.on_device = coarse_e2d_device(s, L.drel, rel, L.d_mis_k.p, L.d_mis_coloff.p, L.mis_nc,
+                                             PT.rowptr.p, PT.val.p, np.d_colpos_ptr, np.d_colpos, np.e2d, np.pending);
         if (!np.on_device) prepare_next_host(L, PT.rowptr.p, PT.val.p, PT.nrows, PT.nnz, s, L.next_prep);
     }
     Table e2d = std::move(L.next_prep.e2d);
@@ -1006,6 +1039,7 @@
         d_colpos_ptr.from_host(L.next_prep.colpos_ptr, s);
         d_colpos.from_host(L.next_prep.colpos, s);
     }
+    CoarseE2dPending e2d_pending = std::move(L.next_prep.pending);
     L.next_prep = NextPrep();
     Level &N = *H.levels[lev + 1];
     std::vector<int64_t> out_off((size_t)nparts + 1, 0);
@@ -1015,13 +1049,14 @@
     }
     N.elmat.off.from_host(out_off, s);
     N.elmat.val.alloc((size_t)out_off[nparts] + 1);
+    e2d_pending.wait();
     std::exception_ptr topo_err;
     std::thread topo_thread;
     struct TopoJoiner { std::thread &t; ~TopoJoiner() { if (t.joinable()) t.join(); } } topo_joiner{topo_thread};
     if (lev + 1 < H.params.num_coarsenings && lev + 1 < (int)H.coarse_parts.size() && !H.coarse_parts[(size_t)lev + 1].empty() &&
         !env_serial()) {
         const int dev = current_device();
-        const int nd_next = L.mis_coloff.back(), np_next = H.nparts_in[(size_t)lev + 1];
+        const int nd_next = L.mis_nc, np_next = H.nparts_in[(size_t)lev + 1];
         Table *e2d_copy = new Table(e2d);
         const hvec<int> *part_next = &H.coarse_parts[(size_t)lev + 1];
         topo_thread = std::thread([&N, &topo_err, e2d_copy, part_next, nd_next, np_next, dev]() {
@@ -1062,8 +1097,7 @@
         constexpr bool dense_only = false;
         const RowsSpan span{(int64_t)rel.AE_to_dof.I[ae0] - (int64_t)rel.AE_to_dof.I[ae_lo], (int64_t)rel.AE_to_dof.I[ae_hi] - (int64_t)rel.AE_to_dof.I[ae_lo]};
         if (lev == 0 && !dense_only && ae_sparse_rows(s, L.drel, L.A, L.elmat, ae0, batch, RW, rv, rc, &span)) {
-            int kmax = 0;
-            for (int km : L.mis_k) kmax = std::max(kmax, km);
+            const int kmax = L.mis_kmax;
             bool have_classes = H.params.opt.eig_dedupe != 0 && (int)L.ae_class.size() == nparts;
             for (int i = ae0; have_classes && i < ae0 + cnt; ++i) have_classes = L.ae_class[i] >= 0;
             if (have_classes && !d_ae_class.n) d_ae_class.from_host(L.ae_class, s);
@@ -1360,6 +1394,7 @@
     SA_REQUIRE(!H.params.testmesh, "the corrected null-space level is not available with the mltest fixture vectors");
     std::vector<int> active((size_t)nm, -1);
     int nact = 0, kmax = 1;
+    L.mis_mirrors(s);
     for (int m = 0; m < nm; ++m)
         if (L.mis_k[m] > 0) { active[m] = nact++; kmax = std::max(kmax, L.mis_k[m]); }
     H.levels.emplace_back(new Level);
@@ -1531,7 +1566,7 @@
             Level &N = *H.levels[lev + 1];
             if (H.galerkin_lev == lev) {
                 N.A = DCsr();
-                N.A.nrows = N.A.ncols = L.mis_coloff.back();
+                N.A.nrows = N.A.ncols = L.mis_nc;
             } else {
                 N.A = std::move(L.Ac);
             }
diff --git a/saamge_amd/csrc/mis.h b/saamge_amd/csrc/mis.h
--- a/saamge_amd/csrc/mis.h
+++ b/saamge_amd/csrc/mis.h
@@ -25,16 +25,27 @@
 void mis_svd(hipStream_t s, const DevRelations &rel, int num_mises, int max_ctot, const MisSvdIO &io, int m0 = 0,
              const int *ae_ev = nullptr);
 
-void build_P_R(hipStream_t s, const DevRelations &rel, const Relations &hrel,
-               const std::vector<int> &h_k, const std::vector<int64_t> &h_u_off, const int *d_k,
+void build_P_R(hipStream_t s, const DevRelations &rel, const Relations &hrel, int nc, int64_t nnz, const int *d_k,
                const int *d_coloff, const int64_t *d_u_off, const double *U, DCsr &P, DCsr &R);
 
+struct MisSizes { int64_t g_total = 0, u_total = 0, s_total = 0; int max_ctot = 0; };
+MisSizes mis_stage_offsets(hipStream_t s, const DevRelations &rel, int nm, int nextra, const int *ae_m, int64_t *g_off,
+                           int64_t *u_off, int64_t *s_off);
+struct MisCounts { int nc = 0; int64_t nnz = 0; int kmax = 0; };
+MisCounts mis_col_offsets(hipStream_t s, const DevRelations &rel, int nm, const int *k, int *coloff);
+
+struct CoarseE2dPending {
+    DBuf<int> d_J, d_err;
+    hvec<int> h_err;
+    PendingCopy copy;
+    void wait();
+};
 bool coarse_e2d_device(hipStream_t s, const DevRelations &rel, const Relations &hrel, const int *d_mis_k,
                        const int *d_mis_coloff, int ncoarse, const roff_t *p_rowptr, const double *p_val,
-                       DBuf<int> &colpos_ptr, DBuf<int> &colpos, Table &e2d);
+                       DBuf<int> &colpos_ptr, DBuf<int> &colpos, Table &e2d, CoarseE2dPending &pend);
 
 void rap_mis(hipStream_t s, const DevRelations &rel, const Relations &hrel, const DCsr &A,
-             const std::vector<int> &h_k, const std::vector<int> &h_coloff, const int *d_k,
+             int nc, const hvec<int> &h_coloff, const int *d_k,
              const int *d_coloff, const int64_t *d_u_off, const double *U, DCsr &Ac, int rank = 0,
              int world = 1, std::vector<long long> *nnz_off = nullptr);
 
diff --git a/saamge_amd/csrc/mis.hip b/saamge_amd/csrc/mis.hip
--- a/saamge_amd/csrc/mis.hip
+++ b/saamge_amd/csrc/mis.hip
@@ -334,7 +334,7 @@
                            rel.pair_loc_off.p, rel.pair_loc.p, rel.flags.p, io, 0, list.p);
         hipLaunchKernelGGL(mis_copy_kernel, dim3(div_up(nm, 4)), dim3(256), 0, s, v, nm, rep.p);
         SA_HIP_CHECK(hipGetLastError());
-        SA_HIP_CHECK(hipStreamSynchronize(s));
+        if (thread_stream_is_set() && thread_stream() != s) SA_HIP_CHECK(hipStreamSynchronize(s));
         profiler().end(s, "mis_svd", 0.0, 0.0);
         return;
     }
@@ -360,12 +360,12 @@
     for (int v = 0; v < k[m]; ++v) len[c0 + v] = r;
 }
 
-template <class OUT>
-__global__ __launch_bounds__(256) void scan_tile_kernel(int n, const int *__restrict__ in,
+template <class OUT, class IN = int>
+__global__ __launch_bounds__(256) void scan_tile_kernel(int n, const IN *__restrict__ in,
                                                         OUT *__restrict__ out, OUT *__restrict__ tsum) {
     __shared__ OUT sh[256];
     const long base = (long)blockIdx.x * 1024;
-    int v[4];
+    IN v[4];
     OUT run = 0;
     for (int q = 0; q < 4; ++q) {
         const long i = base + threadIdx.x * 4 + q;
@@ -440,6 +440,104 @@
     SA_HIP_CHECK(hipGetLastError());
 }
 void exclusive_scan_off(hipStream_t s, int n, const int *in, roff_t *out) { exclusive_scan_t<roff_t>(s, n, in, out); }
+template <class OUT, class IN>
+static void exclusive_scan_async_t(hipStream_t s, int n, const IN *in, OUT *out, OUT *tsum) {
+    const int nt = div_up(n, 1024);
+    hipLaunchKernelGGL((scan_tile_kernel<OUT, IN>), dim3(nt), dim3(256), 0, s, n, in, out, tsum);
+    hipLaunchKernelGGL(scan_sums_kernel<OUT>, dim3(1), dim3(256), 0, s, nt, tsum, tsum + nt);
+    hipLaunchKernelGGL(scan_add_kernel<OUT>, dim3(div_up(n, 256)), dim3(256), 0, s, n, out, (const OUT *)tsum, (const OUT *)(tsum + nt));
+    SA_HIP_CHECK(hipGetLastError());
+}
+
+__global__ __launch_bounds__(256) void mis_sizes_kernel(int nm, int nextra, const int *__restrict__ mis2ae_I,
+                                                        const int *__restrict__ mis2ae_J, const int *__restrict__ mis2d_I,
+                                                        const int *__restrict__ ae_m, int *__restrict__ ctot_out,
+                                                        int64_t *__restrict__ gsz, int64_t *__restrict__ usz,
+                                                        int *__restrict__ max_ctot) {
+    const int m = blockIdx.x * 256 + threadIdx.x;
+    int ctot = 0;
+    if (m < nm) {
+        ctot = nextra;
+        for (int q = mis2ae_I[m]; q < mis2ae_I[m + 1]; ++q) ctot += ae_m[mis2ae_J[q]];
+        const int r = mis2d_I[m + 1] - mis2d_I[m];
+        ctot_out[m] = ctot;
+        gsz[m] = (int64_t)r * ctot;
+        usz[m] = (int64_t)r * max(1, min(r, ctot));
+    }
+    int mx = ctot;
+#pragma unroll
+    for (int o = 32; o > 0; o >>= 1) mx = max(mx, __shfl_xor(mx, o, 64));
+    if ((threadIdx.x & 63) == 0) atomicMax(max_ctot, mx);
+}
+__global__ __launch_bounds__(256) void mis_counts_kernel(int nm, const int *__restrict__ mis2d_I, const int *__restrict__ k,
+                                                         unsigned long long *__restrict__ nnz, int *__restrict__ kmax) {
+    const int m = blockIdx.x * 256 + threadIdx.x;
+    unsigned long long e = 0;
+    int km = 0;
+    if (m < nm) {
+        km = k[m];
+        e = (unsigned long long)km * (unsigned long long)(mis2d_I[m + 1] - mis2d_I[m]);
+    }
+#pragma unroll
+    for (int o = 32; o > 0; o >>= 1) { e += __shfl_xor(e, o, 64); km = max(km, __shfl_xor(km, o, 64)); }
+    if ((threadIdx.x & 63) == 0) { atomicAdd(nnz, e); atomicMax(kmax, km); }
+}
+__global__ void mis_info_kernel(const int64_t *a, const int64_t *b, const int64_t *c, const int *mx, int64_t *info) {
+    info[0] = *a; info[1] = *b; info[2] = *c; info[3] = *mx;
+}
+__global__ void mis_info2_kernel(const int *nc, const unsigned long long *nnz, const int *kmax, int64_t *info) {
+    info[0] = *nc; info[1] = (int64_t)*nnz; info[2] = *kmax;
+}
+
+MisSizes mis_stage_offsets(hipStream_t s, const DevRelations &rel, int nm, int nextra, const int *ae_m, int64_t *g_off,
+                           int64_t *u_off, int64_t *s_off) {
+    MisSizes out;
+    if (!nm) {
+        SA_HIP_CHECK(hipMemsetAsync(g_off, 0, sizeof(int64_t), s));
+        SA_HIP_CHECK(hipMemsetAsync(u_off, 0, sizeof(int64_t), s));
+        SA_HIP_CHECK(hipMemsetAsync(s_off, 0, sizeof(int64_t), s));
+        return out;
+    }
+    const int nt = div_up(nm, 1024);
+    DBuf<int> ctot((size_t)nm), mx(1);
+    DBuf<int64_t> gsz((size_t)nm), usz((size_t)nm), tsum(3 * ((size_t)nt + 1)), info(4);
+    mx.zero(s);
+    hipLaunchKernelGGL(mis_sizes_kernel, dim3(div_up(nm, 256)), dim3(256), 0, s, nm, nextra, rel.mis2ae_I.p, rel.mis2ae_J.p,
+                       rel.mis2d_I.p, ae_m, ctot.p, gsz.p, usz.p, mx.p);
+    exclusive_scan_async_t<int64_t, int64_t>(s, nm, gsz.p, g_off, tsum.p);
+    exclusive_scan_async_t<int64_t, int64_t>(s, nm, usz.p, u_off, tsum.p + (nt + 1));
+    exclusive_scan_async_t<int64_t, int>(s, nm, ctot.p, s_off, tsum.p + 2 * (nt + 1));
+    hipLaunchKernelGGL(mis_info_kernel, dim3(1), dim3(1), 0, s, g_off + nm, u_off + nm, s_off + nm, mx.p, info.p);
+    SA_HIP_CHECK(hipGetLastError());
+    int64_t h[4] = {0, 0, 0, 0};
+    SA_HIP_CHECK(hipMemcpyAsync(h, info.p, sizeof(h), hipMemcpyDeviceToHost, s));
+    SA_HIP_CHECK(hipStreamSynchronize(s));
+    out.g_total = h[0]; out.u_total = h[1]; out.s_total = h[2]; out.max_ctot = (int)h[3];
+    return out;
+}
+
+MisCounts mis_col_offsets(hipStream_t s, const DevRelations &rel, int nm, const int *k, int *coloff) {
+    MisCounts out;
+    if (!nm) {
+        SA_HIP_CHECK(hipMemsetAsync(coloff, 0, sizeof(int), s));
+        return out;
+    }
+    const int nt = div_up(nm, 1024);
+    DBuf<int> tsum((size_t)nt + 1), kmax(1);
+    DBuf<unsigned long long> nnz(1);
+    DBuf<int64_t> info(3);
+    kmax.zero(s);
+    nnz.zero(s);
+    exclusive_scan_async_t<int, int>(s, nm, k, coloff, tsum.p);
+    hipLaunchKernelGGL(mis_counts_kernel, dim3(div_up(nm, 256)), dim3(256), 0, s, nm, rel.mis2d_I.p, k, nnz.p, kmax.p);
+    hipLaunchKernelGGL(mis_info2_kernel, dim3(1), dim3(1), 0, s, coloff + nm, nnz.p, kmax.p, info.p);
+    SA_HIP_CHECK(hipGetLastError());
+    int64_t h[3] = {0, 0, 0};
+    SA_HIP_CHECK(hipMemcpyAsync(h, info.p, sizeof(h), hipMemcpyDeviceToHost, s));
+    SA_HIP_CHECK(hipStreamSynchronize(s));
+    out.nc = (int)h[0]; out.nnz = h[1]; out.kmax = (int)h[2];
+    return out;
+}
 
 __global__ __launch_bounds__(256) void p_fill_kernel(int ND, const int *__restrict__ mises,
                                                      const int *__restrict__ row_in_mis,
@@ -485,17 +583,9 @@
     }
 }
 
-void build_P_R(hipStream_t s, const DevRelations &rel, const Relations &hrel,
-               const std::vector<int> &h_k, const std::vector<int64_t> &h_u_off, const int *d_k,
+void build_P_R(hipStream_t s, const DevRelations &rel, const Relations &hrel, int nc, int64_t nnz, const int *d_k,
                const int *d_coloff, const int64_t *d_u_off, const double *U, DCsr &P, DCsr &R) {
-    (void)h_u_off;
     const int ND = hrel.ND;
-    int nc = 0;
-    int64_t nnz = 0;
-    for (int m = 0; m < hrel.num_mises; ++m) {
-        nc += h_k[m];
-        nnz += (int64_t)h_k[m] * hrel.mis_to_dof.row_size(m);
-    }
     P.nrows = ND; P.ncols = nc; P.nnz = nnz;
     P.rowptr.alloc((size_t)ND + 1);
     P.col.alloc((size_t)nnz);
@@ -594,42 +684,59 @@
     }
 }
 
+__global__ __launch_bounds__(256) void ae_e2d_I_kernel(int nparts, const int *__restrict__ ae2mis_I,
+                                                       const int *__restrict__ colpos_ptr, int *__restrict__ out) {
+    const int e = blockIdx.x * 256 + threadIdx.x;
+    if (e <= nparts) out[e] = colpos_ptr[ae2mis_I[e]];
+}
+
 bool coarse_e2d_device(hipStream_t s, const DevRelations &rel, const Relations &hrel, const int *d_mis_k,
                        const int *d_mis_coloff, int ncoarse, const roff_t *p_rowptr, const double *p_val,
-                       DBuf<int> &colpos_ptr, DBuf<int> &colpos, Table &e2d) {
+                       DBuf<int> &colpos_ptr, DBuf<int> &colpos, Table &e2d, CoarseE2dPending &pend) {
     const int nparts = hrel.nparts;
     const long npairs = (long)hrel.AE_to_mis.J.size();
     if (nparts == 0 || npairs == 0) return false;
-    DBuf<int> kk((size_t)npairs), info(2);
-    info.zero(s);
+    DBuf<int> kk((size_t)npairs), head((size_t)nparts + 2), tsum((size_t)div_up(npairs, 1024) + 1);
+    SA_HIP_CHECK(hipMemsetAsync(head.p + nparts + 1, 0, sizeof(int), s));
     hipLaunchKernelGGL(ae_mis_k_kernel, dim3(div_up(npairs, 256)), dim3(256), 0, s, npairs, rel.ae2mis_J.p, d_mis_k, kk.p);
     colpos_ptr.alloc((size_t)npairs + 1);
-    exclusive_scan_int(s, (int)npairs, kk.p, colpos_ptr.p);
-    hipLaunchKernelGGL(ae_ke_max_kernel, dim3(div_up(nparts, 256)), dim3(256), 0, s, nparts, rel.ae2mis_I.p, colpos_ptr.p, info.p);
+    exclusive_scan_int_async(s, (int)npairs, kk.p, colpos_ptr.p, tsum.p);
+    hipLaunchKernelGGL(ae_ke_max_kernel, dim3(div_up(nparts, 256)), dim3(256), 0, s, nparts, rel.ae2mis_I.p, colpos_ptr.p,
+                       head.p + nparts + 1);
+    hipLaunchKernelGGL(ae_e2d_I_kernel, dim3(div_up(nparts + 1, 256)), dim3(256), 0, s, nparts, rel.ae2mis_I.p, colpos_ptr.p, head.p);
     SA_HIP_CHECK(hipGetLastError());
-    const int cap = info.to_host(s)[0];
+    hvec<int> h_head = head.to_host(s);
+    const int cap = h_head[(size_t)nparts + 1];
     const size_t lds = (size_t)cap * 12 + 16;
     if (lds > 60 * 1024) return false;
-    auto h_ptr = colpos_ptr.to_host(s);
-    const int total = h_ptr[(size_t)npairs];
+    const int total = h_head[(size_t)nparts];
     colpos.alloc((size_t)total + 1);
-    DBuf<int> d_J((size_t)total + 1);
+    pend.d_J.alloc((size_t)total + 1);
+    pend.d_err.alloc(1);
+    pend.d_err.zero(s);
+    pend.h_err.assign(1, 0);
     if (total) {
         hipLaunchKernelGGL(coarse_e2d_kernel, dim3(nparts), dim3(256), lds, s, rel.ae2d_I.p, rel.ae2d_J.p, rel.ae2mis_I.p,
                            rel.ae2mis_J.p, rel.mises.p, d_mis_k, d_mis_coloff, colpos_ptr.p, p_rowptr, p_val, cap, colpos.p,
-                           d_J.p, info.p + 1);
+                           pend.d_J.p, pend.d_err.p);
         SA_HIP_CHECK(hipGetLastError());
     }
-    SA_REQUIRE(info.to_host(s)[1] == 0, "coarse dof with an all-zero prolongator column in an AE");
     e2d.ncols = ncoarse;
-    e2d.I.resize((size_t)nparts + 1);
-    for (int e = 0; e <= nparts; ++e) e2d.I[e] = h_ptr[(size_t)hrel.AE_to_mis.I[e]];
+    h_head.resize((size_t)nparts + 1);
+    e2d.I = std::move(h_head);
     e2d.J.resize((size_t)total);
-    if (total) {
-        SA_HIP_CHECK(hipMemcpyAsync(e2d.J.data(), d_J.p, sizeof(int) * (size_t)total, hipMemcpyDeviceToHost, s));
-        SA_HIP_CHECK(hipStreamSynchronize(s));
-    }
+    hipStream_t rs = readback_stream_behind(s);
+    if (total) SA_HIP_CHECK(hipMemcpyAsync(e2d.J.data(), pend.d_J.p, sizeof(int) * (size_t)total, hipMemcpyDeviceToHost, rs));
+    SA_HIP_CHECK(hipMemcpyAsync(pend.h_err.data(), pend.d_err.p, sizeof(int), hipMemcpyDeviceToHost, rs));
+    pend.copy.record(rs);
     return true;
+}
+void CoarseE2dPending::wait() {
+    if (!copy.pending()) return;
+    copy.wait();
+    d_J.release();
+    d_err.release();
+    SA_REQUIRE(h_err.empty() || h_err[0] == 0, "coarse dof with an all-zero prolongator column in an AE");
 }
 
 constexpr int RAP_NT = 256;
@@ -989,12 +1096,10 @@
 }
 
 void rap_mis(hipStream_t s, const DevRelations &rel, const Relations &hrel, const DCsr &A,
-             const std::vector<int> &h_k, const std::vector<int> &h_coloff, const int *d_k,
+             int nc, const hvec<int> &h_coloff, const int *d_k,
              const int *d_coloff, const int64_t *d_u_off, const double *U, DCsr &Ac, int rank, int world,
              std::vector<long long> *nnz_off) {
     const int nm = hrel.num_mises;
-    int nc = 0;
-    for (int m = 0; m < nm; ++m) nc += h_k[m];
     Ac.nrows = Ac.ncols = nc;
     Ac.nnz = 0;
     if (nm == 0 || nc == 0) {
```

After: 70.72 million DoF/s (median of 5 runs). Within noise of the previous version (+1.0%).
